# ysbbin/Robust-Object-Detection

Hardware: AMD Instinct MI355X
Metric: images/sec FRCNN-R50-FPN train @1333x800 bs=2/GPU (higher is better)
Workload: dtype f32; 1 GPU; configs[1]: FRCNN R50-FPN v2 baseline train step; global_batch=2, per_gpu_batch=2, image=1333x800 (padded 1344x800), parallelism=dp1, trainable_backbone_layers=3, conv_tuner=bench_tune.json (91 shapes pinned)

## Files before the change

### include/mx_det.h

```cpp
#ifndef MX_DET_H
#define MX_DET_H
#include <stddef.h>
#include <stdint.h>
#ifdef __cplusplus
extern "C" {
#endif

#define MX_OK 0
#define MX_EINVAL -1
#define MX_EUNSUPPORTED -2
#define MX_EHIP -3

#define MX_F32 0
#define MX_BF16 1

typedef void* mx_stream_t;

int mx_version(void);
const char* mx_last_error(void);
int mx_trace_marker(int id, mx_stream_t stream);
int mx_stream_create(int device, mx_stream_t* out);

size_t mx_match_workspace(int64_t G, int64_t A);
int mx_match_assign(const float* gt, const int64_t* gt_labels, int64_t G, const float* boxes, int64_t A,
// ... 190 lines not shown
int mx_conv2d_fwd(const mx_conv_shape* s, const uint16_t* x, const uint16_t* w, const float* bias, void* y,
                  int ydtype, float* stats, mx_stream_t stream);
int mx_conv2d_dgrad(const mx_conv_shape* s, const uint16_t* dy, const uint16_t* w, uint16_t* dx,
                    mx_stream_t stream);
int mx_conv2d_fwd_ex(const mx_conv_shape* s, const uint16_t* x, const uint16_t* w, const float* bias,
                     const uint16_t* residual, int act, void* y, int ydtype, float* stats, void* ws, size_t ws_bytes,
                     mx_stream_t stream, const mx_conv_cfg* cfg);
size_t mx_conv_workspace(const mx_conv_shape* s, int pass, const mx_conv_cfg* cfg);
int mx_conv_set_variant(int variant);
int mx_conv_get_variant(void);
int mx_conv_set_wgrad_variant(int variant);
int mx_conv_get_wgrad_variant(void);
int mx_conv_pack_weight(const mx_conv_shape* s, const float* w, int64_t Cin, int64_t Kout, uint16_t* wk, uint16_t* wt,
                        int split, mx_stream_t stream);
size_t mx_conv_dgrad_weight_elems(const mx_conv_shape* s, int64_t Cpad, int64_t Kpad);
typedef struct {
  const float* w;
  uint16_t* wk;
  uint16_t* wt;
  int64_t Cin, Kout, Cpad, Kpad;
  int32_t R, S, stride_h, stride_w, pad_h, pad_w;
  int32_t flags;
} mx_pack_desc;
size_t mx_conv_pack_plan_bytes(int64_t njobs);
int mx_conv_pack_batched(const mx_pack_desc* jobs, int64_t njobs, void* plan, size_t plan_bytes, int upload,
                         mx_stream_t stream);
typedef struct {
  float* p;
  float* buf;
  int64_t n;
  int32_t first;
  int32_t pack;
} mx_sgd_param;
size_t mx_sgd_pack_plan_bytes(int64_t nparams);
int mx_sgd_pack_build(const mx_sgd_param* params, int64_t nparams, const mx_pack_desc* packs, void* host_plan,
                      size_t plan_bytes, int64_t* blocks, size_t* lds_bytes);
int mx_sgd_pack_step(const void* plan, const float* const* grads, int64_t nparams, int64_t blocks, size_t lds_bytes,
                     float lr, float momentum, float dampening, float weight_decay, int nesterov, mx_stream_t stream);
typedef struct {
  float* p;
  float* exp_avg;
  float* exp_avg_sq;
  int64_t n;
  int32_t pack;
  int32_t reserved;
} mx_adamw_param;
size_t mx_adamw_pack_plan_bytes(int64_t nparams);
int mx_adamw_pack_build(const mx_adamw_param* params, int64_t nparams, const mx_pack_desc* packs, void* host_plan,
                        size_t plan_bytes, int64_t* blocks, size_t* lds_bytes);
int mx_adamw_pack_step(const void* plan, const float* const* grads, int64_t nparams, int64_t blocks, size_t lds_bytes,
                       int64_t step, double lr, double beta1, double beta2, double eps, double weight_decay,
                       mx_stream_t stream);
int mx_conv_transpose_weight(const uint16_t* w, int64_t K, int64_t RS, int64_t C, uint16_t* wt, mx_stream_t stream);
int mx_conv2d_dgrad_t(const mx_conv_shape* s, const uint16_t* dy, const uint16_t* wt, uint16_t* dx, void* ws,
                      size_t ws_bytes, mx_stream_t stream);
int mx_conv2d_dgrad_ex(const mx_conv_shape* s, const uint16_t* dy, const uint16_t* wt, const uint16_t* residual,
                       uint16_t* dx, void* ws, size_t ws_bytes, mx_stream_t stream, const mx_conv_cfg* cfg);
int mx_conv2d_dgrad_bnb(const mx_conv_shape* s, const uint16_t* dy, const uint16_t* wt, const uint16_t* residual,
                        uint16_t* dx, const uint16_t* y, const uint16_t* z, const float* mean, const float* invstd,
                        int act, float* part, int64_t part_mb, void* ws, size_t ws_bytes, mx_stream_t stream,
                        const mx_conv_cfg* cfg);
int mx_conv2d_wgrad(const mx_conv_shape* s, const uint16_t* dy, const uint16_t* x, float* dw, mx_stream_t stream);
int mx_conv2d_wgrad_ex(const mx_conv_shape* s, const uint16_t* dy, const uint16_t* x, float* dw, int64_t Kout,
                       int64_t Cin, int layout, void* ws, size_t ws_bytes, mx_stream_t stream, const mx_conv_cfg* cfg);
int mx_conv_set_loader(int loader);
int mx_conv_set_tile(int block_rows, int block_cols);
int mx_conv_set_max_splits(int max_splits);
int mx_conv_set_stages(int stages);
int mx_conv_set_korder(int order);
int mx_conv_set_wgrad_target(int64_t blocks);
int mx_conv_last_launch(int32_t out[8]);

size_t mx_conv_workspace_x3(const mx_conv_shape* s, int pass, const mx_conv_cfg* cfg);
int mx_conv2d_fwd_x3(const mx_conv_shape* s, const float* x, const uint16_t* w, const float* bias, const float* residual,
                     int act, float* y, float* stats, void* ws, size_t ws_bytes, mx_stream_t stream,
                     const mx_conv_cfg* cfg);
int mx_conv2d_stem_x3(const mx_conv_shape* s, const float* x, const uint16_t* w, const float* bias, int act, float* y,
                      float* stats, mx_stream_t stream);
int mx_conv2d_dgrad_x3(const mx_conv_shape* s, const float* dy, const uint16_t* wt, const float* residual, float* dx,
                       const float* y, const float* z, const float* mean, const float* invstd, int act, float* part,
                       int64_t part_mb, void* ws, size_t ws_bytes, mx_stream_t stream, const mx_conv_cfg* cfg);
int mx_conv2d_wgrad_x3(const mx_conv_shape* s, const float* dy, const float* x, float* dw, int64_t Kout, int64_t Cin,
                       int layout, void* ws, size_t ws_bytes, mx_stream_t stream, const mx_conv_cfg* cfg);

int64_t mx_rpn_rows_capacity(int64_t P, int64_t NB, int level);
size_t mx_rpn_rows_workspace(int64_t P);
int mx_rpn_rows_build(const float* g, int64_t N, int64_t H, int64_t W, int64_t C, int levels, int32_t* rows0,
                      int64_t cap0, int32_t* rows1, int64_t cap1, int32_t* rows2, int64_t cap2, int32_t* counts,
                      int32_t* flag, void* ws, size_t ws_bytes, mx_stream_t stream);
int64_t mx_rpn_tiles_capacity(int64_t P, int64_t NB, int level);
int mx_rpn_tiles_build(const float* g, int64_t N, int64_t H, int64_t W, int64_t C, int levels, int32_t* tiles0,
                       int64_t cap0, int32_t* tiles1, int64_t cap1, int32_t* tiles2, int64_t cap2, int32_t* counts,
                       int32_t* flag, void* ws, size_t ws_bytes, mx_stream_t stream);
int mx_conv2d_wgrad_x3_rows(const mx_conv_shape* s, const float* dy, const float* x, float* dw, int64_t Kout,
                            int64_t Cin, int layout, const int32_t* tiles, const int32_t* ntiles, int64_t cap, void* ws,
                            size_t ws_bytes, mx_stream_t stream, const mx_conv_cfg* cfg);
int mx_rpn_lists_build(const float* g, int64_t N, int64_t H, int64_t W, int64_t C, int32_t* rows0, int64_t cap0,
                       int32_t* rows1, int64_t cap1, int32_t* rows2, int64_t cap2, int32_t* counts, int32_t* tiles0,
                       int64_t tcap0, int32_t* tiles1, int64_t tcap1, int32_t* tcounts, int32_t* flag, void* ws,
                       size_t ws_bytes, mx_stream_t stream);
int mx_conv2d_dgrad_x3_rows_supported(const mx_conv_shape* s, const mx_conv_cfg* cfg);
int mx_conv2d_dgrad_x3_rows(const mx_conv_shape* s, const float* dy, const uint16_t* wt, const float* residual, float* dx,
                            const int32_t* rows, const int32_t* nrows, int64_t cap, mx_stream_t stream,
                            const mx_conv_cfg* cfg);
int mx_act_bias_bwd_rows(const float* gy, const float* y, const float* mask, int64_t mask_period, int64_t M, int64_t K,
                         const int32_t* rows, const int32_t* nrows, int64_t cap, float* g, float* db, void* ws,
                         size_t ws_bytes, mx_stream_t stream);

int mx_maxpool_fwd(const void* x, int dtype, int64_t N, int64_t H, int64_t W, int64_t C, int k, int stride, int pad,
                   void* y, int32_t* argmax, mx_stream_t stream);
int mx_maxpool_bwd(const void* gy, int dtype, const int32_t* argmax, int64_t N, int64_t H, int64_t W, int64_t C, int k,
                   int stride, int pad, void* gx, mx_stream_t stream);
int mx_upsample_nearest_fwd(const void* x, int dtype, int64_t N, int64_t H, int64_t W, int64_t C, int64_t Ho, int64_t Wo,
                            const void* add, void* y, mx_stream_t stream);
int mx_upsample_nearest_bwd(const void* gy, int dtype, int64_t N, int64_t H, int64_t W, int64_t C, int64_t Ho, int64_t Wo,
                            void* gx, mx_stream_t stream);

int mx_bn_finalize(const float* stats, int64_t mblocks, int64_t K, int64_t count, const float* gamma,
                   const float* beta, float eps, float momentum, float* running_mean, float* running_var,
                   float* mean_out, float* invstd_out, float* scale_out, float* shift_out, mx_stream_t stream);
int mx_bn_bwd_finalize(const float* part, int64_t mb, int64_t K, int64_t M, const float* mean, const float* invstd,
                       const float* gamma, float* sums, float* coef, void* ws, size_t ws_bytes, mx_stream_t stream);
size_t mx_rpn_loss_workspace(int64_t n);
int mx_rpn_loss_fwd(const float* objectness, const float* deltas, const float* labels, const float* targets,
                    const uint8_t* pos, const uint8_t* neg, int64_t n, float beta, float* out, void* ws,
                    size_t ws_bytes, mx_stream_t stream);
int mx_rpn_loss_bwd(const float* objectness, const float* deltas, const float* labels, const float* targets,
                    const uint8_t* pos, const uint8_t* neg, int64_t n, float beta, const float* out, const float* grad,
                    float* grad_objectness, float* grad_deltas, mx_stream_t stream);
int mx_roi_loss_fwd(const float* logits, int64_t ldl, int C, const float* reg, int64_t ldr, const int64_t* labels,
                    const float* targets, int64_t R, float beta, float* out, void* ws, size_t ws_bytes,
                    mx_stream_t stream);
int mx_roi_loss_bwd(const float* logits, int64_t ldl, int C, const float* reg, int64_t ldr, const int64_t* labels,
                    const float* targets, int64_t R, float beta, const float* grad, float* grad_logits,
                    float* grad_reg, mx_stream_t stream);
size_t mx_bn_finalize_workspace(int64_t mblocks, int64_t K);
int mx_bn_finalize_ex(const float* stats, int64_t mblocks, int64_t K, int64_t count, const float* gamma,
                      const float* beta, float eps, float momentum, float* running_mean, float* running_var,
                      float* mean_out, float* invstd_out, float* scale_out, float* shift_out, void* ws,
                      size_t ws_bytes, mx_stream_t stream);
int mx_bn_finalize_adapt(const float* stats, int64_t mblocks, int64_t K, int64_t count, const float* gamma,
                         const float* beta, float eps, const float* src_mean, const float* src_var, double prior,
                         double n_images, double* state ,
                         float* mean_out, float* var_out, float* scale_out, float* shift_out, void* ws, size_t ws_bytes,
                         mx_stream_t stream);
int mx_bn_apply(const void* x, int xdtype, int64_t M, int64_t K, const float* scale, const float* shift,
                const void* residual, int act, void* y, int ydtype, mx_stream_t stream);
int mx_bn_act_maxpool(const float* z, int64_t N, int64_t H, int64_t W, int64_t C, const float* scale, const float* shift,
                      int act, int k, int stride, int pad, float* y, mx_stream_t stream);
size_t mx_bn_bwd_workspace(int64_t M, int64_t K);
int mx_bn_bwd_reduce_ex(const void* dy, const void* y, const void* x, int dtype, int64_t M, int64_t K, int act,
                        const float* mean, const float* invstd, const float* gamma, void* ws, size_t ws_bytes,
                        float* sums, float* coef, mx_stream_t stream);
int mx_bn_bwd_apply_ex(const void* dy, const void* y, const void* x, int dtype, int64_t M, int64_t K, int act,
                       const float* coef, void* dx, void* dres, mx_stream_t stream);
size_t mx_act_bias_bwd_workspace(int64_t M, int64_t K);
int mx_act_bias_bwd(const void* gy, const void* y, int dtype, int64_t M, int64_t K, int64_t K8, int act,
                    void* g, int gdtype, float* db, void* ws, size_t ws_bytes, mx_stream_t stream);
int mx_bn_bwd_reduce(const uint16_t* dy, const uint16_t* y, const uint16_t* x, int64_t M, int64_t K, int act,
                     const float* mean, const float* invstd, float* sums, mx_stream_t stream);
int mx_bn_bwd_apply(const uint16_t* dy, const uint16_t* y, const uint16_t* x, int64_t M, int64_t K, int act,
                    const float* mean, const float* invstd, const float* gamma, const float* sums,
                    uint16_t* dx, uint16_t* dres ,
                    mx_stream_t stream);

int mx_sgd_step(float* const* params, const float* const* grads, float* const* momentum_bufs,
                const int64_t* numels, const uint8_t* first, int64_t count, float lr, float momentum,
                float dampening, float weight_decay, int nesterov, mx_stream_t stream);
int mx_adamw_step(float* const* params, const float* const* grads, float* const* exp_avgs, float* const* exp_avg_sqs,
                  const int64_t* numels, const int64_t* steps, int64_t count, double lr, double beta1, double beta2,
                  double eps, double weight_decay, mx_stream_t stream);

int mx_reflect_pad_u8(const uint8_t* src, int64_t B, int64_t H, int64_t W, int64_t C, int64_t Hp, int64_t Wp,
                      uint8_t* dst, mx_stream_t stream);
int mx_up_concat(const void* up, const void* skip, int dtype, int64_t N, int64_t H, int64_t W, int64_t Cu, int64_t Cs,
                 void* out, mx_stream_t stream);
int mx_up_concat_bwd(const void* gcat, int dtype, int64_t N, int64_t H, int64_t W, int64_t Cu, int64_t Cs, void* gup,
                     void* gskip, mx_stream_t stream);
int mx_restore_finish(const uint8_t* img_padded, int64_t B, int64_t Hp, int64_t Wp, const float* residual, int64_t H,
                      int64_t W, uint8_t* out, mx_stream_t stream);
int mx_restore_finish_gated(const uint8_t* img_padded, int64_t B, int64_t Hp, int64_t Wp, const float* residual, int64_t H,
                            int64_t W, const int32_t* verdict, uint8_t* out, mx_stream_t stream);

size_t mx_ssim_workspace(int64_t N, int64_t H, int64_t W, int64_t C);
int mx_ssim_l1_fwd(const float* pred, const float* target, int64_t N, int64_t H, int64_t W, int64_t C, int window,
                   float sigma, float c1, float c2, float weight, float* out3, double* dmaps, void* ws, size_t ws_bytes,
                   mx_stream_t stream);
int mx_ssim_l1_bwd(const float* pred, const float* target, const double* dmaps, int64_t N, int64_t H, int64_t W,
                   int64_t C, int window, float sigma, const float* gout, float cs, float cl, float* grad,
                   mx_stream_t stream);

typedef struct {
  int32_t width, height, ncomp;
  int32_t h[3], v[3], tq[3];
  int32_t hmax, vmax, mcux, mcuy;
  int32_t bw[3], bh[3];
  int32_t dw[3], dh[3];
  int64_t coef_off[3], coef_total;
  int32_t restart_interval;
  int32_t scan_off;
  uint16_t qt[4][64];
  uint8_t cid[3], td[3], ta[3];
  uint8_t hbits[8][17], hval[8][256];
  uint8_t hdef[8];
} mx_jpeg_info;
int mx_jpeg_parse(const uint8_t* data, int64_t n, mx_jpeg_info* info);
int mx_jpeg_decode_coefs(const uint8_t* data, int64_t n, const mx_jpeg_info* info, int16_t* coefs_host);
size_t mx_jpeg_workspace(const mx_jpeg_info* info);
int mx_jpeg_reconstruct(const int16_t* coefs, const mx_jpeg_info* info, void* ws, size_t ws_bytes, uint8_t* out,
                        int bgr, mx_stream_t stream);

int mx_jpeg_reconstruct_window(const int16_t* coefs, const mx_jpeg_info* info, int x0, int y0, int w, int h, int hflip,
                               int bgr, uint8_t* out, int64_t out_row_bytes, mx_stream_t stream);
int mx_jpeg_window_cover(const mx_jpeg_info* info, int x0, int y0, int w, int h, int32_t cover[3][4]);

#define MX_JPEG_ST_CODE 1
#define MX_JPEG_ST_DC 2
#define MX_JPEG_ST_RUN 4
#define MX_JPEG_ST_SHORT 8
#define MX_JPEG_ST_RESTART 16
size_t mx_jpeg_entropy_decode_workspace(const mx_jpeg_info* info, int64_t nbytes);
int mx_jpeg_entropy_decode(const uint8_t* scan_dev, int64_t nbytes, const mx_jpeg_info* info, void* ws, size_t ws_bytes,
                           int16_t* coefs_dev, int32_t* status_dev, mx_stream_t stream);
int mx_jpeg_entropy_decode_set_subseq(int bits);
int mx_jpeg_decode_coefs_chunked(const uint8_t* data, int64_t n, const mx_jpeg_info* info, int subseq_bits,
                                 int16_t* coefs_host, int32_t* status);

int mx_jpeg_encode_info(int width, int height, int quality, int subsampling, mx_jpeg_info* out);
int mx_jpeg_write_header(const mx_jpeg_info* info, uint8_t* out, int64_t cap, int64_t* n);
int64_t mx_jpeg_scan_bound(const mx_jpeg_info* info);
int mx_jpeg_encode_coefs(const mx_jpeg_info* info, const int16_t* coefs_host, uint8_t* out, int64_t cap, int64_t* n);
int mx_jpeg_forward(const uint8_t* img, int bgr, const mx_jpeg_info* info, int16_t* coefs_dev, mx_stream_t stream);
size_t mx_jpeg_entropy_workspace(const mx_jpeg_info* info);
int mx_jpeg_entropy(const int16_t* coefs_dev, const mx_jpeg_info* info, void* ws, size_t ws_bytes, uint8_t* out_dev,
                    int64_t out_cap, int64_t* nbytes_dev, mx_stream_t stream);

size_t mx_corrupt_jpeg_workspace(int64_t B, int64_t H, int64_t W, int subsampling);
int mx_corrupt_jpeg_u8(const uint8_t* img, int64_t B, int64_t H, int64_t W, const int32_t* quality_host,
// ... 19 lines not shown
```

### robust-object-detection_amd/csrc/mx_bn.hip

```cpp
#include "mx_common.h"
#include "mx_rpn_rows.h"

namespace mx {

__device__ __forceinline__ float actf(float v, int act) {
  if (act == 1) return v > 0.f ? v : 0.f;
  if (act == 2) return v > 0.f ? v : 0.2f * v;
  return v;
}
__device__ __forceinline__ float actd(float y, int act) {
  if (act == 1) return y > 0.f ? 1.f : 0.f;
  if (act == 2) return y > 0.f ? 1.f : 0.2f;
  return 1.f;
}

static constexpr int CTR_BYTES = 256, MAX_CHUNKS = CTR_BYTES / 4;

template <typename T>
__device__ __forceinline__ void st_sc1(T* p, T v) { __hip_atomic_store(p, v, __ATOMIC_RELAXED, __HIP_MEMORY_SCOPE_AGENT); }
template <typename T>
__device__ __forceinline__ T ld_sc1(const T* p) { return __hip_atomic_load((T*)p, __ATOMIC_RELAXED, __HIP_MEMORY_SCOPE_AGENT); }

__device__ __forceinline__ bool arrive_last(unsigned* ctr, unsigned nblocks) {
  __shared__ int last;
// ... 305 lines not shown
        }
      }
#pragma unroll
      for (int t = 0; t < 8; ++t) s[t] += v[t];
      st8(g + r * K8 + c0, v);
    }
  }
  if (!db) return;
#pragma unroll
  for (int t = 0; t < 8; ++t) red[rl][cl * 8 + t] = s[t];
  __syncthreads();
  const int col = threadIdx.x & 63;
  const int k = blockIdx.y * 64 + col;
  if (threadIdx.x < 64) {
    float a = 0.f;
#pragma unroll 8
    for (int r = 0; r < 32; ++r) a += red[r][col];
    if (k < K) st_sc1(part + (int64_t)blockIdx.x * K + k, a);
  }
  if (!arrive_last(ctr + blockIdx.y, (unsigned)RB)) return;
  __shared__ double fin[1][64], scr[256];
  last_sums<1>((const float*)part, RB, (int64_t)K, (int64_t)blockIdx.y * 64, fin, scr);
  if (threadIdx.x < 64 && k < K) db[k] = (float)fin[0][col];
}

__global__ void __launch_bounds__(256) act_bias_bwd_rows_kernel(const float* __restrict__ gy, const float* __restrict__ y,
                                                                const float* __restrict__ mask, int64_t mask_period,
                                                                int64_t M, int K, int64_t rows_per_block,
                                                                const int32_t* __restrict__ rows,
                                                                const int32_t* __restrict__ nrows, int64_t cap,
                                                                float* __restrict__ g, float* __restrict__ db,
                                                                unsigned* __restrict__ ctr, float* __restrict__ part) {
  __shared__ float red[32][65];
  __shared__ int64_t range[2];
  const int cl = threadIdx.x & 7, rl = threadIdx.x >> 3;
  const int c0 = blockIdx.y * 64 + cl * 8;
  const int64_t RB = gridDim.x;
  const int64_t r0 = (int64_t)blockIdx.x * rows_per_block;
  const int64_t r1 = min<int64_t>(M, r0 + rows_per_block);
  if (threadIdx.x < 2) {
    const int64_t n = min<int64_t>(max<int64_t>((int64_t)*nrows, 0), cap);
    range[threadIdx.x] = rpn_rows_lower_bound(rows, n, threadIdx.x ? r1 : r0);
  }
  __syncthreads();
  float s[8] = {0, 0, 0, 0, 0, 0, 0, 0};
  if (c0 < K) {
    const int64_t j1 = range[1];
    for (int64_t j = range[0]; j < j1; ++j) {
      const int64_t r = rows[j];
      if (r < r0 || r >= r1 || (int)((r - r0) & 31) != rl) continue;
      float v[8], vg[8], vy[8];
      ld8(gy + r * K + c0, vg);
      ld8(y + r * K + c0, vy);
      if (mask) {
        const float mk = mask[r % mask_period];
#pragma unroll
        for (int t = 0; t < 8; ++t) vg[t] = vg[t] * mk;
      }
#pragma unroll
      for (int t = 0; t < 8; ++t) v[t] = vg[t] * act_grad<1>(vy[t]);
#pragma unroll
      for (int t = 0; t < 8; ++t) s[t] += v[t];
      st8(g + r * K + c0, v);
    }
  }
  if (!db) return;
#pragma unroll
  for (int t = 0; t < 8; ++t) red[rl][cl * 8 + t] = s[t];
  __syncthreads();
  const int col = threadIdx.x & 63;
  const int k = blockIdx.y * 64 + col;
  if (threadIdx.x < 64) {
    float a = 0.f;
#pragma unroll 8
    for (int r = 0; r < 32; ++r) a += red[r][col];
    if (k < K) st_sc1(part + (int64_t)blockIdx.x * K + k, a);
  }
  if (!arrive_last(ctr + blockIdx.y, (unsigned)RB)) return;
  __shared__ double fin[1][64], scr[256];
  last_sums<1>((const float*)part, RB, (int64_t)K, (int64_t)blockIdx.y * 64, fin, scr);
  if (threadIdx.x < 64 && k < K) db[k] = (float)fin[0][col];
}

template <int ACT, typename T>
__global__ void __launch_bounds__(256) bn_bwd_apply2_kernel(const T* __restrict__ dy, const T* __restrict__ y,
                                                            const T* __restrict__ x, int64_t n8, int K8,
                                                            const float* __restrict__ coef, T* __restrict__ dx,
                                                            T* __restrict__ dres) {
  const int64_t e = (int64_t)blockIdx.x * 256 + threadIdx.x;
  if (e >= n8) return;
  const int K = K8 * 8;
  const int c0 = (int)(e % K8) * 8;
  float vd[8], vx[8], vy[8] = {0, 0, 0, 0, 0, 0, 0, 0};
  ld8(dy + e * 8, vd);
  ld8(x + e * 8, vx);
  if (ACT) ld8(y + e * 8, vy);
  const float4 a0 = *(const float4*)(coef + c0), a1 = *(const float4*)(coef + c0 + 4);
  const float4 b0 = *(const float4*)(coef + K + c0), b1 = *(const float4*)(coef + K + c0 + 4);
  const float4 d0 = *(const float4*)(coef + 2 * K + c0), d1 = *(const float4*)(coef + 2 * K + c0 + 4);
  const float A[8] = {a0.x, a0.y, a0.z, a0.w, a1.x, a1.y, a1.z, a1.w};
  const float B[8] = {b0.x, b0.y, b0.z, b0.w, b1.x, b1.y, b1.z, b1.w};
  const float C[8] = {d0.x, d0.y, d0.z, d0.w, d1.x, d1.y, d1.z, d1.w};
  float o[8], og[8];
#pragma unroll
  for (int q = 0; q < 8; ++q) {
    og[q] = vd[q] * act_grad<ACT>(vy[q]);
    o[q] = A[q] * og[q] + B[q] * vx[q] + C[q];
  }
  st8(dx + e * 8, o);
  if (dres) st8(dres + e * 8, og);
}

__global__ void bn_coef_from_sums_kernel(const float* __restrict__ sums, int64_t K, int64_t M, const float* __restrict__ mean,
                                         const float* __restrict__ invstd, const float* __restrict__ gamma,
                                         float* __restrict__ coef) {
  const int64_t k = (int64_t)blockIdx.x * blockDim.x + threadIdx.x;
  if (k >= K) return;
  const float is = invstd[k], a = (gamma ? gamma[k] : 1.f) * is;
  const float invM = 1.0f / (float)M;
  const float mg = sums[k] * invM, mgx = sums[K + k] * invM;
  coef[k] = a;
  coef[K + k] = -a * is * mgx;
  coef[2 * K + k] = -a * (mg - mean[k] * is * mgx);
}

static unsigned grid_rows(int64_t M, int64_t K8) {
  int64_t want = std::min<int64_t>(cdiv(M * K8, 256), 2048);
  return (unsigned)std::max<int64_t>(want, cdiv(K8, 256));
}

struct BwdGeo {
  int64_t RB, rows_per_block, gy;
};
static BwdGeo bwd_geo(int64_t M, int64_t K) {
  BwdGeo g;
  g.gy = cdiv(K, 64);
  g.RB = std::max<int64_t>(1, std::min<int64_t>(std::min<int64_t>(128, cdiv(M, 64)), std::max<int64_t>(1, 1024 / g.gy)));
  g.rows_per_block = cdiv(M, g.RB);
  g.RB = cdiv(M, g.rows_per_block);
  return g;
}

static int64_t fin_slices(int64_t mb) { return std::max<int64_t>(1, std::min<int64_t>(64, cdiv(mb, 32))); }

__device__ __forceinline__ float smooth_l1(float u, float beta) {
  const float a = fabsf(u);
  return a < beta ? 0.5f * u * u / beta : a - 0.5f * beta;
}

__global__ void __launch_bounds__(256) rpn_loss_fwd_kernel(const float* __restrict__ x, const float4* __restrict__ d,
                                                           const float* __restrict__ y, const float4* __restrict__ t,
                                                           const uint8_t* __restrict__ pm, const uint8_t* __restrict__ nm,
                                                           int64_t n, float beta, unsigned* __restrict__ ctr,
                                                           double* __restrict__ part, float* __restrict__ out) {
  double a0 = 0.0, a1 = 0.0, a2 = 0.0;
  for (int64_t i = (int64_t)blockIdx.x * 256 + threadIdx.x; i < n; i += (int64_t)gridDim.x * 256) {
    const bool p = pm[i], s = p || nm[i];
    if (!s) continue;
    const float xi = x[i], yi = y[i] > 0.f ? 1.f : 0.f;
    const float m = fmaxf(-xi, 0.f);
    a0 += (double)((1.f - yi) * xi + m + logf(expf(-m) + expf(-xi - m)));
    a2 += 1.0;
    if (p) {
      const float4 di = d[i], ti = t[i];
      a1 += (double)(smooth_l1(di.x - ti.x, beta) + smooth_l1(di.y - ti.y, beta) + smooth_l1(di.z - ti.z, beta) +
                     smooth_l1(di.w - ti.w, beta));
    }
  }
  __shared__ double red[3][256];
  red[0][threadIdx.x] = a0;
  red[1][threadIdx.x] = a1;
  red[2][threadIdx.x] = a2;
  __syncthreads();
  for (int o = 128; o > 0; o >>= 1) {
    if (threadIdx.x < o)
      for (int w = 0; w < 3; ++w) red[w][threadIdx.x] += red[w][threadIdx.x + o];
    __syncthreads();
  }
  const int64_t RB = gridDim.x;
  if (threadIdx.x < 3) st_sc1(part + threadIdx.x * RB + blockIdx.x, red[threadIdx.x][0]);
  if (!arrive_last(ctr, (unsigned)RB)) return;
  __shared__ double fin[3][64], scr[256];
  last_sums<3>(part, RB, 1, 0, fin, scr);
  if (threadIdx.x == 0) {
    const double cnt = fin[2][0];
    out[0] = (float)(fin[0][0] / cnt);
    out[1] = (float)(fin[1][0] / cnt);
    out[2] = (float)cnt;
  }
}

__global__ void __launch_bounds__(256) rpn_loss_bwd_kernel(const float* __restrict__ x, const float4* __restrict__ d,
// ... 215 lines not shown
                           const void* residual, int act, void* y, int ydtype, mx_stream_t stream) {
  MX_CHECK_ARG(K % 8 == 0, "bn_apply: K %% 8 != 0");
  MX_CHECK_ARG((xdtype == MX_BF16 || xdtype == MX_F32) && (ydtype == MX_BF16 || ydtype == MX_F32), "bn_apply: bad dtype");
  MX_CHECK_ARG(!(xdtype == MX_BF16 && ydtype == MX_F32),
               "bn_apply: bf16 input with f32 output is not a supported combination");
  if (M == 0) return MX_OK;
  const unsigned grid = grid_rows(M, K / 8);
  hipStream_t st = (hipStream_t)stream;
  if (xdtype == MX_BF16 && ydtype == MX_BF16)
    bn_apply_kernel<uint16_t, uint16_t><<<grid, 256, 0, st>>>((const uint16_t*)x, M, K, scale, shift,
                                                             (const uint16_t*)residual, act, (uint16_t*)y);
  else if (xdtype == MX_F32 && ydtype == MX_BF16)
    bn_apply_kernel<float, uint16_t><<<grid, 256, 0, st>>>((const float*)x, M, K, scale, shift, (const uint16_t*)residual,
                                                          act, (uint16_t*)y);
  else if (xdtype == MX_F32 && ydtype == MX_F32)
    bn_apply_kernel<float, float><<<grid, 256, 0, st>>>((const float*)x, M, K, scale, shift, (const float*)residual, act,
                                                       (float*)y);
  else
    MX_CHECK_ARG(false, "bn_apply: bf16 input with f32 output is not a supported combination");
  MX_LAUNCH_CHECK();
  return MX_OK;
}

extern "C" size_t mx_bn_bwd_workspace(int64_t M, int64_t K) {
  if (M <= 0 || K <= 0 || K % 8) return 0;
  BwdGeo g = bwd_geo(M, K);
  return CTR_BYTES + sizeof(float) * 2 * (size_t)g.RB * K;
}

template <typename T>
static void bn_bwd_reduce_launch(const void* dy, const void* y, const void* x, int64_t M, int64_t K, int act,
                                 const BwdGeo& g, const float* mean, const float* invstd, const float* gamma, unsigned* ctr,
                                 float* part, float* sums, float* coef, hipStream_t st) {
  dim3 grid((unsigned)g.RB, (unsigned)g.gy);
  const T *d = (const T*)dy, *yy = (const T*)y, *xx = (const T*)x;
  if (act == 1)
    bn_bwd_reduce_kernel<1, T><<<grid, 256, 0, st>>>(d, yy, xx, M, K, g.rows_per_block, mean, invstd, gamma, ctr, part, sums, coef);
  else if (act == 2)
    bn_bwd_reduce_kernel<2, T><<<grid, 256, 0, st>>>(d, yy, xx, M, K, g.rows_per_block, mean, invstd, gamma, ctr, part, sums, coef);
  else
    bn_bwd_reduce_kernel<0, T><<<grid, 256, 0, st>>>(d, yy, xx, M, K, g.rows_per_block, mean, invstd, gamma, ctr, part, sums, coef);
}

extern "C" int mx_bn_bwd_reduce_ex(const void* dy, const void* y, const void* x, int dtype, int64_t M, int64_t K, int act,
                                   const float* mean, const float* invstd, const float* gamma, void* ws, size_t ws_bytes,
                                   float* sums, float* coef, mx_stream_t stream) {
  MX_CHECK_ARG(K % 8 == 0 && K > 0 && M > 0, "bn_bwd_reduce: K must be a positive multiple of 8, M > 0");
  MX_CHECK_ARG(act >= 0 && act <= 2, "bn_bwd_reduce: act 0/1/2");
  MX_CHECK_ARG(act == 0 || y, "bn_bwd_reduce: y required for an activation");
  BwdGeo g = bwd_geo(M, K);
  MX_CHECK_ARG(g.gy <= MAX_CHUNKS && g.RB < 65536, "bn_bwd_reduce: K > %d", MAX_CHUNKS * 64);
  const size_t need = mx_bn_bwd_workspace(M, K);
  MX_CHECK_ARG(ws && ws_bytes >= need, "bn_bwd_reduce: workspace of %zu bytes required (mx_bn_bwd_workspace)", need);
  unsigned* ctr = (unsigned*)ws;
  float* part = (float*)((char*)ws + CTR_BYTES);
  MX_DT_DISPATCH(dtype, bn_bwd_reduce_launch, dy, y, x, M, K, act, g, mean, invstd, gamma, ctr, part, sums, coef,
                 (hipStream_t)stream);
  MX_LAUNCH_CHECK();
  return MX_OK;
}

template <typename T>
static void bn_bwd_apply_launch(const void* dy, const void* y, const void* x, int64_t n8, int K8, int act, const float* coef,
                                void* dx, void* dres, hipStream_t st) {
  const unsigned blocks = (unsigned)cdiv(n8, 256);
  const T *d = (const T*)dy, *yy = (const T*)y, *xx = (const T*)x;
  if (act == 1) bn_bwd_apply2_kernel<1, T><<<blocks, 256, 0, st>>>(d, yy, xx, n8, K8, coef, (T*)dx, (T*)dres);
  else if (act == 2) bn_bwd_apply2_kernel<2, T><<<blocks, 256, 0, st>>>(d, yy, xx, n8, K8, coef, (T*)dx, (T*)dres);
  else bn_bwd_apply2_kernel<0, T><<<blocks, 256, 0, st>>>(d, yy, xx, n8, K8, coef, (T*)dx, (T*)dres);
}

extern "C" int mx_bn_bwd_apply_ex(const void* dy, const void* y, const void* x, int dtype, int64_t M, int64_t K, int act,
                                  const float* coef, void* dx, void* dres, mx_stream_t stream) {
  MX_CHECK_ARG(K % 8 == 0 && K > 0 && K < (1 << 24), "bn_bwd_apply: K must be a positive multiple of 8");
  MX_CHECK_ARG(act >= 0 && act <= 2, "bn_bwd_apply: act 0/1/2");
  MX_CHECK_ARG(act == 0 || y, "bn_bwd_apply: y required for an activation");
  if (M == 0) return MX_OK;
  const int64_t n8 = M * (K / 8);
  MX_DT_DISPATCH(dtype, bn_bwd_apply_launch, dy, y, x, n8, (int)(K / 8), act, coef, dx, dres, (hipStream_t)stream);
  MX_LAUNCH_CHECK();
  return MX_OK;
}

extern "C" int mx_bn_bwd_reduce(const uint16_t* dy, const uint16_t* y, const uint16_t* x, int64_t M, int64_t K, int act,
                                const float* mean, const float* invstd, float* sums, mx_stream_t stream) {
  MX_CHECK_ARG(K % 8 == 0 && K > 0, "bn_bwd_reduce: K must be a positive multiple of 8");
  if (M == 0) return MX_OK;
  hipStream_t st = (hipStream_t)stream;
  const size_t wsb = mx_bn_bwd_workspace(M, K);
  void* ws = nullptr;
  float* coef = nullptr;
  MX_HIP(hipMallocAsync(&ws, wsb, st));
  MX_HIP(hipMemsetAsync(ws, 0, CTR_BYTES, st));
  MX_HIP(hipMallocAsync((void**)&coef, sizeof(float) * 3 * K, st));
  int rc = mx_bn_bwd_reduce_ex(dy, y, x, MX_BF16, M, K, act, mean, invstd, nullptr, ws, wsb, sums, coef, stream);
  MX_HIP(hipFreeAsync(ws, st));
  MX_HIP(hipFreeAsync(coef, st));
  return rc;
}

extern "C" int mx_bn_bwd_apply(const uint16_t* dy, const uint16_t* y, const uint16_t* x, int64_t M, int64_t K, int act,
                               const float* mean, const float* invstd, const float* gamma, const float* sums,
                               uint16_t* dx, uint16_t* dres, mx_stream_t stream) {
  MX_CHECK_ARG(K % 8 == 0 && K > 0, "bn_bwd_apply: K %% 8 != 0");
  if (M == 0) return MX_OK;
  hipStream_t st = (hipStream_t)stream;
  float* coef = nullptr;
  MX_HIP(hipMallocAsync((void**)&coef, sizeof(float) * 3 * K, st));
  bn_coef_from_sums_kernel<<<(unsigned)cdiv(K, 256), 256, 0, st>>>(sums, K, M, mean, invstd, gamma, coef);
  int rc = MX_OK;
  if (hipGetLastError() != hipSuccess) rc = MX_EHIP;
  if (!rc) rc = mx_bn_bwd_apply_ex(dy, y, x, MX_BF16, M, K, act, coef, dx, dres, stream);
  MX_HIP(hipFreeAsync(coef, st));
  return rc;
}

static BwdGeo act_geo(int64_t M, int64_t K8) {
  BwdGeo g;
  g.gy = cdiv(K8, 64);
  g.RB = std::max<int64_t>(1, std::min<int64_t>(std::min<int64_t>(128, cdiv(M, 64)), std::max<int64_t>(1, 1024 / g.gy)));
  g.rows_per_block = cdiv(M, g.RB);
  g.RB = cdiv(M, g.rows_per_block);
  return g;
}

extern "C" size_t mx_act_bias_bwd_workspace(int64_t M, int64_t K) {
  if (M <= 0 || K <= 0) return 0;
  BwdGeo g = act_geo(M, (K + 7) / 8 * 8);
  return CTR_BYTES + sizeof(float) * (size_t)g.RB * K;
}

template <typename T, typename TG>
static void launch_act_bias(const void* gy, const void* y, int64_t M, int K, int K8, int act, const BwdGeo& g,
                            void* out_, float* db, unsigned* ctr, float* part, hipStream_t st) {
  dim3 grid((unsigned)g.RB, (unsigned)g.gy);
  TG* out = (TG*)out_;
  if (act == 1)
    act_bias_bwd_kernel<T, 1, TG><<<grid, 256, 0, st>>>((const T*)gy, (const T*)y, M, K, K8, g.rows_per_block, out, db, ctr, part);
  else if (act == 2)
    act_bias_bwd_kernel<T, 2, TG><<<grid, 256, 0, st>>>((const T*)gy, (const T*)y, M, K, K8, g.rows_per_block, out, db, ctr, part);
  else
    act_bias_bwd_kernel<T, 0, TG><<<grid, 256, 0, st>>>((const T*)gy, (const T*)y, M, K, K8, g.rows_per_block, out, db, ctr, part);
}

extern "C" int mx_act_bias_bwd(const void* gy, const void* y, int dtype, int64_t M, int64_t K, int64_t K8, int act,
                               void* g, int gdtype, float* db, void* ws, size_t ws_bytes, mx_stream_t stream) {
  MX_CHECK_ARG(M >= 0 && K > 0 && K8 >= K && K8 % 8 == 0 && K8 < (1 << 24), "act_bias_bwd: need 0 < K <= K8, K8 %% 8 == 0");
  MX_CHECK_ARG(act >= 0 && act <= 2 && (act == 0 || y), "act_bias_bwd: act 0/1/2 (y required for 1/2)");
  MX_CHECK_ARG(dtype == MX_BF16 || dtype == MX_F32, "act_bias_bwd: dtype bf16 or f32");
  MX_CHECK_ARG(gdtype == MX_BF16 || gdtype == MX_F32, "act_bias_bwd: gdtype bf16 or f32");
  if (M == 0) {
    if (db) MX_HIP(hipMemsetAsync(db, 0, sizeof(float) * K, (hipStream_t)stream));
    return MX_OK;
  }
  BwdGeo g_ = act_geo(M, K8);
  MX_CHECK_ARG(g_.gy <= MAX_CHUNKS, "act_bias_bwd: K8 > %d", MAX_CHUNKS * 64);
  unsigned* ctr = nullptr;
  float* part = nullptr;
  if (db) {
    const size_t need = mx_act_bias_bwd_workspace(M, K);
    MX_CHECK_ARG(ws && ws_bytes >= need, "act_bias_bwd: workspace of %zu bytes required (mx_act_bias_bwd_workspace)", need);
    ctr = (unsigned*)ws;
    part = (float*)((char*)ws + CTR_BYTES);
  }
  hipStream_t st = (hipStream_t)stream;
  if (dtype == MX_BF16 && gdtype == MX_BF16)
// ... 103 lines not shown
```

### robust-object-detection_amd/csrc/mx_conv.hip

```cpp
#include "mx_common.h"
#include "mx_conv_layout.h"
#include "mx_dma.h"
#include "mx_rpn_rows.h"

#include <vector>

namespace mx {

typedef __bf16 bf16x8 __attribute__((ext_vector_type(8)));
typedef short s16x4 __attribute__((ext_vector_type(4)));
typedef float f32x4 __attribute__((ext_vector_type(4)));

static constexpr int BM = 128, BK = 64, NT = 256;

struct ConvP {
  const uint16_t* src;
  const uint16_t* wt;
  int64_t M, Ncol, Kdim;
  int64_t OH, OW;
  int64_t IH, IW, IC;
  int R, S, st_h, st_w, pad_h, pad_w;
  const float* bias;
  const void* residual;
  int act;
// ... 1457 lines not shown
    for (int i = 0; i < BCH; ++i) {
      if (kin && b_row[i] < p.Ncol) {
        rbh[i] = *(const uint4*)(whi + b_row[i] * p.Kdim + k);
        rbl[i] = *(const uint4*)(wlo + b_row[i] * p.Kdim + k);
      } else {
        rbh[i] = rbl[i] = make_uint4(0, 0, 0, 0);
      }
    }
  };
  auto store = [&](int buf) {
    char* Ah = smem + buf * STAGE;
    char* Al = Ah + APL;
    char* Bh = Al + APL;
    char* Bl = Bh + BPL;
#pragma unroll
    for (int i = 0; i < ACH; ++i) {
      const int row = (tid >> 2) + RPS * i;
      const int off = row * RB + ((kc ^ tile_swz<4>(row)) << 4);
      uint4 h, l;
      split8(ra[i][0], ra[i][1], h, l);
      *(uint4*)(Ah + off) = h;
      *(uint4*)(Al + off) = l;
    }
#pragma unroll
    for (int i = 0; i < BCH; ++i) {
      const int row = (tid >> 2) + RPS * i;
      const int off = row * RB + ((kc ^ tile_swz<4>(row)) << 4);
      *(uint4*)(Bh + off) = rbh[i];
      *(uint4*)(Bl + off) = rbl[i];
    }
  };
  f32x4 acc[TI][TJ];
#pragma unroll
  for (int i = 0; i < TI; ++i)
#pragma unroll
    for (int j = 0; j < TJ; ++j) acc[i][j] = f32x4{0.f, 0.f, 0.f, 0.f};
  if (ntk > 0) {
    load();
    store(0);
  }
  __syncthreads();
  for (int64_t t = 0; t < ntk; ++t) {
    const int buf = (int)(t & 1);
    if (t + 1 < ntk) load();
    const char* Ah = smem + buf * STAGE;
    const char* Al = Ah + APL;
    const char* Bh = Al + APL;
    const char* Bl = Bh + BPL;
    const int ch = lane >> 4;
    bf16x8 ah[TI], al[TI], bh[TJ], bl[TJ];
#pragma unroll
    for (int i = 0; i < TI; ++i) {
      const int row = wm * WM + i * 16 + (lane & 15);
      const int off = row * RB + ((ch ^ tile_swz<4>(row)) << 4);
      ah[i] = *(const bf16x8*)(Ah + off);
      al[i] = *(const bf16x8*)(Al + off);
    }
#pragma unroll
    for (int j = 0; j < TJ; ++j) {
      const int row = wn * WN + j * 16 + (lane & 15);
      const int off = row * RB + ((ch ^ tile_swz<4>(row)) << 4);
      bh[j] = *(const bf16x8*)(Bh + off);
      bl[j] = *(const bf16x8*)(Bl + off);
    }
#pragma unroll
    for (int i = 0; i < TI; ++i)
#pragma unroll
      for (int j = 0; j < TJ; ++j) {
        acc[i][j] = __builtin_amdgcn_mfma_f32_16x16x32_bf16(al[i], bh[j], acc[i][j], 0, 0, 0);
        acc[i][j] = __builtin_amdgcn_mfma_f32_16x16x32_bf16(ah[i], bl[j], acc[i][j], 0, 0, 0);
        acc[i][j] = __builtin_amdgcn_mfma_f32_16x16x32_bf16(ah[i], bh[j], acc[i][j], 0, 0, 0);
      }
    if (t + 1 < ntk) store(buf ^ 1);
    __syncthreads();
  }
  conv_epilogue<BN, 2, BMT, float, 2, 2, MODE == 1>(p, acc, smem, m0, n0, mt, wm, wn, lane, tid, split);
}

__device__ __forceinline__ int x3_swz(int row) {
  const int g = (row >> 2) & 3;
  return g ^ (g >> 1);
}

template <int BN, int MODE, int STAGES, int OCC, int BMT, int WR = 2, int WC = 2, bool ROWS = false>
__global__ void __launch_bounds__(64 * WR * WC, OCC) conv_x3_buf_kernel(ConvP p) {
#if defined(__HIP_DEVICE_COMPILE__)
  extern __shared__ __attribute__((aligned(16))) char smem[];
  constexpr int RB = 64, RPI = 16;
  constexpr int NW = WC * WR;
  constexpr int AR = BMT / NW, AI = AR / RPI, BR = BN / NW, BI = BR / RPI;
  constexpr int LOADS = 2 * AI + 2 * BI;
  constexpr int AH = BMT * RB, BP = BN * RB, STAGE = 2 * AH + 2 * BP;
  constexpr int WN = BN / WC, TJ = WN / 16, WM = BMT / WR, TI = WM / 16;
  static_assert(AI >= 1 && BI >= 1 && STAGES >= 2, "tile shape");
  const int tid = threadIdx.x, lane = tid & 63, wave = tid >> 6;
  const int wm = wave / WC, wn = wave % WC;
  const int64_t ntiles_n = (p.Ncol + BN - 1) / BN;
  const int64_t gid = xcd_remap(blockIdx.x, (int64_t)gridDim.x);
  const int split = (int)(gid % p.splits);
  const int64_t bid = gid / p.splits;
  const int64_t mt = bid / ntiles_n, nt = bid % ntiles_n;
  const int64_t m0 = mt * BMT, n0 = nt * BN;
  int64_t nrows = p.M;
  if constexpr (ROWS) {
    static_assert(MODE == 1, "rows form: dgrad only");
    nrows = min<int64_t>(max<int64_t>((int64_t)*p.rows_count, 0), p.rows_cap);
    if (m0 >= nrows) return;
  }
  const int lrow = lane >> 2, pc = lane & 3;
  const int qa = pc ^ x3_swz(lrow), qb = pc ^ tile_swz<4>(lrow);
  const int IH = (int)p.IH, IW = (int)p.IW, IC = (int)p.IC, R = p.R, S = p.S;
  uint32_t a_voff[AI];
  uint64_t a_mask[AI];
#pragma unroll
  for (int i = 0; i < AI; ++i) {
    int64_t m = m0 + wave * AR + i * RPI + lrow;
    uint64_t mask = 0;
    int32_t off = 0;
    bool mok = m < nrows;
    if constexpr (ROWS) {
      m = mok ? (int64_t)p.rows[m] : -1;
      mok = (uint64_t)m < (uint64_t)p.M;
    }
    if (mok) {
      const int ow = (int)(m % p.OW);
      const int64_t t = m / p.OW;
      const int oh = (int)(t % p.OH);
      const int n = (int)(t / p.OH);
      const int h0 = MODE == 0 ? oh * p.st_h - p.pad_h : oh + p.pad_h - (R - 1);
      const int w0 = MODE == 0 ? ow * p.st_w - p.pad_w : ow + p.pad_w - (S - 1);
      off = ((n * IH + h0) * IW + w0) * IC + qa * 4;
      for (int r = 0; r < R; ++r)
        for (int q = 0; q < S; ++q) {
          const int rr = MODE == 0 ? r : R - 1 - r, qq = MODE == 0 ? q : S - 1 - q;
          if ((unsigned)(h0 + rr) < (unsigned)IH && (unsigned)(w0 + qq) < (unsigned)IW) mask |= 1ull << (r * S + q);
        }
    }
    a_voff[i] = (uint32_t)off * 4u;
    a_mask[i] = mask;
  }
  uint32_t b_voff[BI];
#pragma unroll
  for (int i = 0; i < BI; ++i) {
    const int64_t n = n0 + wave * BR + i * RPI + lrow;
    b_voff[i] = n < p.Ncol ? (uint32_t)((n * p.Kdim + qb * 8) * 2) : kOOB;
  }
  const i32x4 arsrc = dma_rsrc(p.src, (uint32_t)(p.src_elems * 4));
  const i32x4 bhrsrc = dma_rsrc(p.wt, (uint32_t)(p.wt_elems * 2));
  const i32x4 blrsrc = dma_rsrc(p.wt + p.wt_plane, (uint32_t)(p.wt_elems * 2));
  const uint32_t lds0 = lds_addr(smem);
  const int64_t nk = p.Kdim / 32;
  const int64_t kbeg = (int64_t)split * p.kt_per_split;
  const int64_t ntk = min<int64_t>(nk, kbeg + p.kt_per_split) - kbeg;
  const int korder = __builtin_amdgcn_readfirstlane(p.korder);
  KPos kp;
  kp.init(korder, (int)kbeg, R, S, IC, 32);
  constexpr int dbg = 0;
  auto issue = [&](int buf) {
    const uint32_t A = lds0 + buf * STAGE;
    const uint32_t B = A + 2 * AH;
    const int cr = kp.cr, cq = kp.cq, cc = kp.cc;
    const int rr = MODE == 0 ? cr : R - 1 - cr, qq = MODE == 0 ? cq : S - 1 - cq;
    const uint32_t a_soff = (uint32_t)(((rr * IW + qq) * IC + cc) * 4);
    const int tap = cr * S + cq;
    const uint32_t b_soff = (uint32_t)__builtin_amdgcn_readfirstlane((int)((tap * IC + cc) * 2));
    if (!(dbg & 8)) {
#pragma unroll
    for (int i = 0; i < AI; ++i) {
      const bool ok = (a_mask[i] >> tap) & 1ull;
      const uint32_t v = a_voff[i] + a_soff;
      const uint32_t dst = A + (wave * AR + i * RPI) * RB;
      lds_dma16(arsrc, dst, ok ? v : kOOB, 0u);
      lds_dma16(arsrc, dst + AH, ok ? v + 64u : kOOB, 0u);
    }
    }
    if (!(dbg & 4)) {
#pragma unroll
    for (int i = 0; i < BI; ++i) {
      const uint32_t dst = B + (wave * BR + i * RPI) * RB;
      lds_dma16(bhrsrc, dst, b_voff[i], b_soff);
      lds_dma16(blrsrc, dst + BP, b_voff[i], b_soff);
    }
    }
    kp.advance(korder, R, S, IC, 32);
  };
  f32x4 acc[TI][TJ];
#pragma unroll
  for (int i = 0; i < TI; ++i)
#pragma unroll
    for (int j = 0; j < TJ; ++j) acc[i][j] = f32x4{0.f, 0.f, 0.f, 0.f};
#pragma unroll
  for (int st = 0; st < STAGES - 1; ++st)
    if (st < ntk) issue(st);
  const int g = lane >> 4, q0 = (g & 1) * 2;
  for (int64_t t = 0; t < ntk; ++t) {
    if (t + STAGES - 2 < ntk) wait_vmcnt<LOADS * (STAGES - 2)>();
    else wait_vmcnt<0>();
    block_barrier();
    if (t + STAGES - 1 < ntk) issue((int)((t + STAGES - 1) % STAGES));
    const char* A = smem + (int)(t % STAGES) * STAGE;
    const char* Ag = A + (g >> 1) * AH;
    const char* Bh = A + 2 * AH;
    const char* Bl = Bh + BP;
    constexpr int TJB = (TJ > 4 && WC == 2) ? 1 : TJ;
    bf16x8 ah[TI], al[TI], bh[TJB], bl[TJB];
    auto loadb = [&](int j, int slot) {
      const int row = wn * WN + j * 16 + (lane & 15);
      const int off = row * RB + ((g ^ tile_swz<4>(row)) << 4);
      bh[slot] = *(const bf16x8*)(Bh + off);
      bl[slot] = *(const bf16x8*)(Bl + off);
    };
    if constexpr (TJB == TJ) {
#pragma unroll
      for (int j = 0; j < TJ; ++j) loadb(j, j);
    }
#pragma unroll
    for (int i = 0; i < TI; ++i) {
      const int row = wm * WM + i * 16 + (lane & 15);
      const int f = x3_swz(row);
      const float4 u = *(const float4*)(Ag + row * RB + ((q0 ^ f) << 4));
      const float4 w = *(const float4*)(Ag + row * RB + (((q0 + 1) ^ f) << 4));
      uint4 h, l;
      if (dbg & 2) {
        h = __builtin_bit_cast(uint4, u);
        l = __builtin_bit_cast(uint4, w);
      } else {
        split8(u, w, h, l);
      }
      ah[i] = __builtin_bit_cast(bf16x8, h);
      al[i] = __builtin_bit_cast(bf16x8, l);
    }
    if constexpr (TJB == TJ) {
#pragma unroll
      for (int i = 0; i < TI; ++i)
#pragma unroll
        for (int j = 0; j < TJ; ++j) {
          acc[i][j] = __builtin_amdgcn_mfma_f32_16x16x32_bf16(al[i], bh[j], acc[i][j], 0, 0, 0);
          acc[i][j] = __builtin_amdgcn_mfma_f32_16x16x32_bf16(ah[i], bl[j], acc[i][j], 0, 0, 0);
          acc[i][j] = __builtin_amdgcn_mfma_f32_16x16x32_bf16(ah[i], bh[j], acc[i][j], 0, 0, 0);
        }
    } else {
#pragma unroll
      for (int j = 0; j < TJ; ++j) {
        loadb(j, 0);
#pragma unroll
        for (int i = 0; i < TI; ++i) {
          acc[i][j] = __builtin_amdgcn_mfma_f32_16x16x32_bf16(al[i], bh[0], acc[i][j], 0, 0, 0);
          acc[i][j] = __builtin_amdgcn_mfma_f32_16x16x32_bf16(ah[i], bl[0], acc[i][j], 0, 0, 0);
          acc[i][j] = __builtin_amdgcn_mfma_f32_16x16x32_bf16(ah[i], bh[0], acc[i][j], 0, 0, 0);
        }
      }
    }
  }
  if (dbg & 1) {
    float sum = 0.f;
#pragma unroll
    for (int i = 0; i < TI; ++i)
#pragma unroll
      for (int j = 0; j < TJ; ++j) sum += acc[i][j][0] + acc[i][j][1] + acc[i][j][2] + acc[i][j][3];
    if (sum == 1.2345e-30f) ((float*)p.out)[0] = sum;
    return;
  }
  __syncthreads();
  conv_epilogue<BN, (WC == 1 ? 1 : WR), BMT, float, WR, WC, MODE == 1, ROWS>(p, acc, smem, m0, n0, mt, wm, wn, lane,
                                                                             tid, split, nrows);
#endif
}

#if defined(__HIP_DEVICE_COMPILE__)
template <bool ROWS>
__device__ __forceinline__ void wgrad_x3_body(const WgP& p) {
  extern __shared__ __attribute__((aligned(16))) char smem[];
  constexpr int PXT = 32, OPB = PXT * 256, STAGE = 4 * OPB;
  const int tid = threadIdx.x, lane = tid & 63, wave = tid >> 6;
  const int wm = wave >> 1, wn = wave & 1;
  const int64_t ntn = (p.Ncol + 127) / 128;
  const int64_t ntiles = ((p.K + 127) / 128) * ntn;
  const int64_t work = xcd_remap(blockIdx.x, (int64_t)gridDim.x);
  const int64_t split = work / ntiles, tile = work % ntiles;
  const int64_t mt = tile / ntn, nt = tile % ntn;
  const int64_t k0 = mt * 128, c0 = nt * 128;
  const int64_t pbeg = split * p.kchunk;
  const int64_t pend = min<int64_t>(p.P, pbeg + p.kchunk);
  if (pbeg >= pend) return;
  int li = 0, lend = 0;
  if constexpr (ROWS) {
    const int n = (int)wgrad_rows(p);
    const int tb = (int)(pbeg / PXT), te = (int)((pend + PXT - 1) / PXT);
    auto lower = [&](int v) {
      int lo = 0, hi = n;
      while (lo < hi) {
        const int mid = (lo + hi) >> 1;
        if (p.rows[mid] < v) lo = mid + 1;
        else hi = mid;
      }
      return lo;
    };
    li = lower(tb);
    lend = lower(te);
  }
  const float* __restrict__ dy = (const float*)p.dy;
  const float* __restrict__ x = (const float*)p.x;
  const int ch = tid & 15;
  const int64_t col = c0 + ch * 8;
  const bool col_ok = col < p.Ncol;
  const int tap = col_ok ? (int)(col / p.C) : 0;
  const int cc = col_ok ? (int)(col - (int64_t)tap * p.C) : 0;
  const int r = tap / p.S, s = tap - (tap / p.S) * p.S;
  const bool k_ok = (k0 + ch * 8) < p.K;
  const int OW = (int)p.OW, OH = (int)p.OH, H = (int)p.H, W = (int)p.W, C = (int)p.C;
  const __amdgpu_buffer_rsrc_t dyr = __builtin_amdgcn_make_buffer_rsrc((void*)dy, (short)0, (int)(p.P * p.K * 4), 0x00020000);
  const __amdgpu_buffer_rsrc_t xr =
      __builtin_amdgcn_make_buffer_rsrc((void*)x, (short)0, (int)(p.N * p.H * p.W * p.C * 4), 0x00020000);
  const int dw = PXT % OW, dh = (PXT / OW) % OH, dn = PXT / (OW * OH);
  const int ihb = -p.pad_h + r, iwb = -p.pad_w + s;
  int px_n[2], px_oh[2], px_ow[2], px_i[2];
#pragma unroll
  for (int i = 0; i < 2; ++i) {
    const int64_t pi = pbeg + (tid >> 4) + 16 * i;
    px_i[i] = (int)pi;
    const int64_t t = pi / OW;
    px_ow[i] = (int)(pi - t * OW);
    px_oh[i] = (int)(t % OH);
    px_n[i] = (int)(t / OH);
  }
  const int pend32 = (int)pend;
  const uint32_t dy_col = (uint32_t)(k0 + ch * 8) * 4u;
  float4 rd[2][2], rx[2][2];
  auto load = [&]() {
#pragma unroll
    for (int i = 0; i < 2; ++i) {
      if constexpr (ROWS) {
        px_i[i] = p.rows[li] * PXT + (tid >> 4) + 16 * i;
        const int t = px_i[i] / OW;
        px_ow[i] = px_i[i] - t * OW;
        px_n[i] = t / OH;
        px_oh[i] = t - px_n[i] * OH;
      }
      const bool pok = px_i[i] < pend32;
      const int pix = px_i[i];
      const uint32_t od = (pok && k_ok) ? __umul24((uint32_t)pix, (uint32_t)(p.K * 4)) + dy_col : kOOB;
      const int ih = __mul24(px_oh[i], p.st_h) + ihb, iw = __mul24(px_ow[i], p.st_w) + iwb;
      const bool xok = pok && col_ok && (unsigned)ih < (unsigned)H && (unsigned)iw < (unsigned)W;
      const uint32_t ox = xok ? (uint32_t)__mul24(__mul24(px_n[i], H) + ih, W) + (uint32_t)iw : 0u;
      const uint32_t oxb = xok ? __umul24(ox, (uint32_t)(C * 4)) + (uint32_t)cc * 4u : kOOB;
      rd[i][0] = __builtin_bit_cast(float4, __builtin_amdgcn_raw_buffer_load_b128(dyr, od, 0, 0));
      rd[i][1] = __builtin_bit_cast(float4, __builtin_amdgcn_raw_buffer_load_b128(dyr, od + 16u, 0, 0));
      rx[i][0] = __builtin_bit_cast(float4, __builtin_amdgcn_raw_buffer_load_b128(xr, oxb, 0, 0));
      rx[i][1] = __builtin_bit_cast(float4, __builtin_amdgcn_raw_buffer_load_b128(xr, oxb + 16u, 0, 0));
      px_i[i] += PXT;
      if constexpr (ROWS) continue;
      int ow = px_ow[i] + dw;
      const int c1 = ow >= OW ? 1 : 0;
      ow -= c1 * OW;
      int oh = px_oh[i] + dh + c1;
      const int c2 = oh >= OH ? 1 : 0;
      oh -= c2 * OH;
      px_ow[i] = ow;
      px_oh[i] = oh;
      px_n[i] += dn + c2;
    }
    if constexpr (ROWS) ++li;
  };
  auto store = [&](int buf) {
    char* Dh = smem + buf * STAGE;
#pragma unroll
    for (int i = 0; i < 2; ++i) {
      const int row = (tid >> 4) + 16 * i;
      const int off = row * 256 + (swz_w(row, ch) << 4);
      uint4 h, l;
      split8(rd[i][0], rd[i][1], h, l);
      *(uint4*)(Dh + off) = h;
      *(uint4*)(Dh + OPB + off) = l;
      split8(rx[i][0], rx[i][1], h, l);
      *(uint4*)(Dh + 2 * OPB + off) = h;
      *(uint4*)(Dh + 3 * OPB + off) = l;
    }
  };
  auto tr_read = [&](const char* T, int prow0, int colbase) -> s16x4 {
    const int g = lane >> 4, q = (lane & 15) >> 2, pp = lane & 3;
    const int row = prow0 + 8 * g + q;
    const int colx = colbase + 4 * pp;
    const int chunk = colx >> 3, within = (colx & 7) * 2;
    return __builtin_amdgcn_ds_read_tr16_b64_v4i16((LDS_AS s16x4*)(T + row * 256 + (swz_w(row, chunk) << 4) + within));
  };
  auto frag = [&](const char* T, int colbase) -> bf16x8 {
    const s16x4 lo = tr_read(T, 0, colbase), hi = tr_read(T, 4, colbase);
    return __builtin_bit_cast(bf16x8, __builtin_shufflevector(lo, hi, 0, 1, 2, 3, 4, 5, 6, 7));
  };
  f32x4 acc[4][4];
#pragma unroll
  for (int i = 0; i < 4; ++i)
#pragma unroll
    for (int j = 0; j < 4; ++j) acc[i][j] = f32x4{0.f, 0.f, 0.f, 0.f};
  const int64_t nk = ROWS ? (int64_t)(lend - li) : (pend - pbeg + PXT - 1) / PXT;
  if (ROWS && nk == 0) {
    wgrad_store(p, acc, k0, c0, wm, wn, lane, split);
    return;
  }
  load();
  store(0);
  __syncthreads();
  for (int64_t it = 0; it < nk; ++it) {
    const int buf = (int)(it & 1);
    if (it + 1 < nk) load();
    const char* Dh = smem + buf * STAGE;
    bf16x8 ah[4], al[4], bh[4], bl[4];
#pragma unroll
    for (int i = 0; i < 4; ++i) {
      ah[i] = frag(Dh, wm * 64 + i * 16);
      al[i] = frag(Dh + OPB, wm * 64 + i * 16);
    }
#pragma unroll
    for (int j = 0; j < 4; ++j) {
      bh[j] = frag(Dh + 2 * OPB, wn * 64 + j * 16);
      bl[j] = frag(Dh + 3 * OPB, wn * 64 + j * 16);
    }
#pragma unroll
    for (int i = 0; i < 4; ++i)
#pragma unroll
      for (int j = 0; j < 4; ++j) {
        acc[i][j] = __builtin_amdgcn_mfma_f32_16x16x32_bf16(al[i], bh[j], acc[i][j], 0, 0, 0);
        acc[i][j] = __builtin_amdgcn_mfma_f32_16x16x32_bf16(ah[i], bl[j], acc[i][j], 0, 0, 0);
        acc[i][j] = __builtin_amdgcn_mfma_f32_16x16x32_bf16(ah[i], bh[j], acc[i][j], 0, 0, 0);
      }
    if (it + 1 < nk) store(buf ^ 1);
    __syncthreads();
  }
  wgrad_store(p, acc, k0, c0, wm, wn, lane, split);
}
#endif
__global__ void __launch_bounds__(NT, 2) conv_wgrad_x3_kernel(WgP p) {
#if defined(__HIP_DEVICE_COMPILE__)
  wgrad_x3_body<false>(p);
#endif
}
__global__ void __launch_bounds__(NT, 2) conv_wgrad_x3_rows_kernel(WgP p) {
#if defined(__HIP_DEVICE_COMPILE__)
  wgrad_x3_body<true>(p);
#endif
}

__global__ void __launch_bounds__(512, 1) conv_wgrad_x3w_kernel(WgP p) {
#if defined(__HIP_DEVICE_COMPILE__)
  extern __shared__ __attribute__((aligned(16))) char smem[];
  constexpr int PXT = 32, OPB = PXT * 256, STAGE = 6 * OPB;
  const int tid = threadIdx.x, lane = tid & 63, wave = tid >> 6;
  const int wm = wave >> 2, wn = wave & 3;
  const int64_t ntn = (p.Ncol + 255) / 256;
  const int64_t ntiles = ((p.K + 127) / 128) * ntn;
  const int64_t work = xcd_remap(blockIdx.x, (int64_t)gridDim.x);
  const int64_t split = work / ntiles, tile = work % ntiles;
  const int64_t mt = tile / ntn, nt = tile % ntn;
  const int64_t k0 = mt * 128, c0 = nt * 256;
  const int64_t pbeg = split * p.kchunk;
  const int64_t pend = min<int64_t>(p.P, pbeg + p.kchunk);
  if (pbeg >= pend) return;
  const float* __restrict__ dy = (const float*)p.dy;
  const float* __restrict__ x = (const float*)p.x;
  const int chd = tid & 15, rowd = tid >> 4;
  const int chx = tid & 31, rowx = tid >> 5;
  const bool k_ok = (k0 + chd * 8) < p.K;
  const int64_t col = c0 + chx * 8;
  const bool col_ok = col < p.Ncol;
  const int tap = col_ok ? (int)(col / p.C) : 0;
  const int cc = col_ok ? (int)(col - (int64_t)tap * p.C) : 0;
  const int r = tap / p.S, s = tap - (tap / p.S) * p.S;
  const int OW = (int)p.OW, OH = (int)p.OH, H = (int)p.H, W = (int)p.W, C = (int)p.C;
  const __amdgpu_buffer_rsrc_t dyr = __builtin_amdgcn_make_buffer_rsrc((void*)dy, (short)0, (int)(p.P * p.K * 4), 0x00020000);
  const __amdgpu_buffer_rsrc_t xr =
      __builtin_amdgcn_make_buffer_rsrc((void*)x, (short)0, (int)(p.N * p.H * p.W * p.C * 4), 0x00020000);
  const int dw = PXT % OW, dh = (PXT / OW) % OH, dn = PXT / (OW * OH);
  const int ihb = -p.pad_h + r, iwb = -p.pad_w + s;
  int pxd = (int)(pbeg + rowd);
  int px_n[2], px_oh[2], px_ow[2], px_i[2];
#pragma unroll
  for (int i = 0; i < 2; ++i) {
    const int64_t pi = pbeg + rowx + 16 * i;
    px_i[i] = (int)pi;
    const int64_t t = pi / OW;
    px_ow[i] = (int)(pi - t * OW);
    px_oh[i] = (int)(t % OH);
    px_n[i] = (int)(t / OH);
  }
  const int pend32 = (int)pend;
  const uint32_t dy_col = (uint32_t)(k0 + chd * 8) * 4u;
  float4 rd[2], rx[2][2];
  auto load = [&]() {
    {
      const uint32_t od = (pxd < pend32 && k_ok) ? __umul24((uint32_t)pxd, (uint32_t)(p.K * 4)) + dy_col : kOOB;
      rd[0] = __builtin_bit_cast(float4, __builtin_amdgcn_raw_buffer_load_b128(dyr, od, 0, 0));
      rd[1] = __builtin_bit_cast(float4, __builtin_amdgcn_raw_buffer_load_b128(dyr, od + 16u, 0, 0));
      pxd += PXT;
    }
#pragma unroll
    for (int i = 0; i < 2; ++i) {
      const bool pok = px_i[i] < pend32;
      const int ih = __mul24(px_oh[i], p.st_h) + ihb, iw = __mul24(px_ow[i], p.st_w) + iwb;
      const bool xok = pok && col_ok && (unsigned)ih < (unsigned)H && (unsigned)iw < (unsigned)W;
      const uint32_t ox = xok ? (uint32_t)__mul24(__mul24(px_n[i], H) + ih, W) + (uint32_t)iw : 0u;
      const uint32_t oxb = xok ? __umul24(ox, (uint32_t)(C * 4)) + (uint32_t)cc * 4u : kOOB;
      rx[i][0] = __builtin_bit_cast(float4, __builtin_amdgcn_raw_buffer_load_b128(xr, oxb, 0, 0));
      rx[i][1] = __builtin_bit_cast(float4, __builtin_amdgcn_raw_buffer_load_b128(xr, oxb + 16u, 0, 0));
      px_i[i] += PXT;
      int ow = px_ow[i] + dw;
      const int c1 = ow >= OW ? 1 : 0;
      ow -= c1 * OW;
      int oh = px_oh[i] + dh + c1;
      const int c2 = oh >= OH ? 1 : 0;
      oh -= c2 * OH;
      px_ow[i] = ow;
      px_oh[i] = oh;
      px_n[i] += dn + c2;
    }
  };
  const int xh = chx >> 4, xc = chx & 15;
  auto store = [&](int buf) {
    char* D = smem + buf * STAGE;
    uint4 h, l;
    {
      const int off = rowd * 256 + (swz_w(rowd, chd) << 4);
      split8(rd[0], rd[1], h, l);
      *(uint4*)(D + off) = h;
      *(uint4*)(D + OPB + off) = l;
    }
#pragma unroll
    for (int i = 0; i < 2; ++i) {
      const int row = rowx + 16 * i;
      const int off = row * 256 + (swz_w(row, xc) << 4);
      split8(rx[i][0], rx[i][1], h, l);
      *(uint4*)(D + (2 + xh) * OPB + off) = h;
      *(uint4*)(D + (4 + xh) * OPB + off) = l;
    }
  };
  auto tr_read = [&](const char* T, int prow0, int colbase) -> s16x4 {
    const int g = lane >> 4, q = (lane & 15) >> 2, pp = lane & 3;
    const int row = prow0 + 8 * g + q;
    const int colx = colbase + 4 * pp;
    const int chunk = colx >> 3, within = (colx & 7) * 2;
    return __builtin_amdgcn_ds_read_tr16_b64_v4i16((LDS_AS s16x4*)(T + row * 256 + (swz_w(row, chunk) << 4) + within));
  };
  auto frag = [&](const char* T, int colbase) -> bf16x8 {
    const s16x4 lo = tr_read(T, 0, colbase), hi = tr_read(T, 4, colbase);
    return __builtin_bit_cast(bf16x8, __builtin_shufflevector(lo, hi, 0, 1, 2, 3, 4, 5, 6, 7));
  };
  f32x4 acc[4][4];
#pragma unroll
  for (int i = 0; i < 4; ++i)
#pragma unroll
    for (int j = 0; j < 4; ++j) acc[i][j] = f32x4{0.f, 0.f, 0.f, 0.f};
  const int64_t nk = (pend - pbeg + PXT - 1) / PXT;
  load();
  store(0);
  __syncthreads();
  const int xplane = wn >> 1, xcol = (wn & 1) * 64;
  for (int64_t it = 0; it < nk; ++it) {
    const int buf = (int)(it & 1);
    if (it + 1 < nk) load();
    const char* D = smem + buf * STAGE;
    bf16x8 ah[4], al[4], bh[4], bl[4];
#pragma unroll
    for (int i = 0; i < 4; ++i) {
      ah[i] = frag(D, wm * 64 + i * 16);
      al[i] = frag(D + OPB, wm * 64 + i * 16);
    }
#pragma unroll
    for (int j = 0; j < 4; ++j) {
      bh[j] = frag(D + (2 + xplane) * OPB, xcol + j * 16);
      bl[j] = frag(D + (4 + xplane) * OPB, xcol + j * 16);
    }
#pragma unroll
    for (int i = 0; i < 4; ++i)
#pragma unroll
      for (int j = 0; j < 4; ++j) {
        acc[i][j] = __builtin_amdgcn_mfma_f32_16x16x32_bf16(al[i], bh[j], acc[i][j], 0, 0, 0);
        acc[i][j] = __builtin_amdgcn_mfma_f32_16x16x32_bf16(ah[i], bl[j], acc[i][j], 0, 0, 0);
        acc[i][j] = __builtin_amdgcn_mfma_f32_16x16x32_bf16(ah[i], bh[j], acc[i][j], 0, 0, 0);
      }
    if (it + 1 < nk) store(buf ^ 1);
    __syncthreads();
  }
  wgrad_store(p, acc, k0, c0, wm, wn, lane, split);
#endif
}

__device__ __forceinline__ void wgrad_store8(const WgP& p, f32x4 (&acc)[8][8], int64_t k0, int64_t c0, int wm, int wn,
                                             int lane, int64_t split) {
  float* slab = p.slab ? p.slab + split * p.K * p.Ncol : nullptr;
#pragma unroll
  for (int i = 0; i < 8; ++i)
#pragma unroll
    for (int j = 0; j < 8; ++j)
#pragma unroll
      for (int rr = 0; rr < 4; ++rr) {
        const int64_t k = k0 + wm * 128 + i * 16 + (lane >> 4) * 4 + rr;
        const int64_t cl = c0 + wn * 128 + j * 16 + (lane & 15);
        if (k >= p.K || cl >= p.Ncol) continue;
        if (slab) {
          slab[k * p.Ncol + cl] = acc[i][j][rr];
        } else {
          const int64_t o = wgrad_dst(p, k, (int)cl);
          if (o >= 0) p.dw[o] = acc[i][j][rr];
        }
      }
}

__global__ void __launch_bounds__(256, 1) conv_wgrad_x3ww_kernel(WgP p) {
#if defined(__HIP_DEVICE_COMPILE__)
  extern __shared__ __attribute__((aligned(16))) char smem[];
  constexpr int PXT = 32, SUB = PXT * 256, STAGE = 8 * SUB;
  const int tid = threadIdx.x, lane = tid & 63, wave = tid >> 6;
  const int wm = wave >> 1, wn = wave & 1;
  const int64_t ntn = (p.Ncol + 255) / 256;
  const int64_t ntiles = ((p.K + 255) / 256) * ntn;
  const int64_t work = xcd_remap(blockIdx.x, (int64_t)gridDim.x);
  const int64_t split = work / ntiles, tile = work % ntiles;
  const int64_t mt = tile / ntn, nt = tile % ntn;
  const int64_t k0 = mt * 256, c0 = nt * 256;
  const int64_t pbeg = split * p.kchunk;
  const int64_t pend = min<int64_t>(p.P, pbeg + p.kchunk);
  if (pbeg >= pend) return;
  const float* __restrict__ dy = (const float*)p.dy;
  const float* __restrict__ x = (const float*)p.x;
  const int ch = tid & 31, row0 = tid >> 5;
  const bool k_ok = (k0 + ch * 8) < p.K;
  const int64_t col = c0 + ch * 8;
  const bool col_ok = col < p.Ncol;
  const int tap = col_ok ? (int)(col / p.C) : 0;
  const int cc = col_ok ? (int)(col - (int64_t)tap * p.C) : 0;
  const int r = tap / p.S, s = tap - (tap / p.S) * p.S;
  const int OW = (int)p.OW, OH = (int)p.OH, H = (int)p.H, W = (int)p.W, C = (int)p.C;
  const __amdgpu_buffer_rsrc_t dyr = __builtin_amdgcn_make_buffer_rsrc((void*)dy, (short)0, (int)(p.P * p.K * 4), 0x00020000);
  const __amdgpu_buffer_rsrc_t xr =
      __builtin_amdgcn_make_buffer_rsrc((void*)x, (short)0, (int)(p.N * p.H * p.W * p.C * 4), 0x00020000);
  const int dw = PXT % OW, dh = (PXT / OW) % OH, dn = PXT / (OW * OH);
  const int ihb = -p.pad_h + r, iwb = -p.pad_w + s;
  int px_n[4], px_oh[4], px_ow[4], px_i[4];
#pragma unroll
  for (int i = 0; i < 4; ++i) {
    const int64_t pi = pbeg + row0 + 8 * i;
    px_i[i] = (int)pi;
    const int64_t t = pi / OW;
    px_ow[i] = (int)(pi - t * OW);
    px_oh[i] = (int)(t % OH);
    px_n[i] = (int)(t / OH);
  }
  const int pend32 = (int)pend;
  const uint32_t dy_col = (uint32_t)(k0 + ch * 8) * 4u;
  float4 rd[4][2], rx[4][2];
  auto load = [&]() {
#pragma unroll
    for (int i = 0; i < 4; ++i) {
      const bool pok = px_i[i] < pend32;
      const uint32_t od = (pok && k_ok) ? __umul24((uint32_t)px_i[i], (uint32_t)(p.K * 4)) + dy_col : kOOB;
      const int ih = __mul24(px_oh[i], p.st_h) + ihb, iw = __mul24(px_ow[i], p.st_w) + iwb;
      const bool xok = pok && col_ok && (unsigned)ih < (unsigned)H && (unsigned)iw < (unsigned)W;
      const uint32_t ox = xok ? (uint32_t)__mul24(__mul24(px_n[i], H) + ih, W) + (uint32_t)iw : 0u;
      const uint32_t oxb = xok ? __umul24(ox, (uint32_t)(C * 4)) + (uint32_t)cc * 4u : kOOB;
      rd[i][0] = __builtin_bit_cast(float4, __builtin_amdgcn_raw_buffer_load_b128(dyr, od, 0, 0));
      rd[i][1] = __builtin_bit_cast(float4, __builtin_amdgcn_raw_buffer_load_b128(dyr, od + 16u, 0, 0));
      rx[i][0] = __builtin_bit_cast(float4, __builtin_amdgcn_raw_buffer_load_b128(xr, oxb, 0, 0));
      rx[i][1] = __builtin_bit_cast(float4, __builtin_amdgcn_raw_buffer_load_b128(xr, oxb + 16u, 0, 0));
      px_i[i] += PXT;
      int ow = px_ow[i] + dw;
      const int c1 = ow >= OW ? 1 : 0;
      ow -= c1 * OW;
      int oh = px_oh[i] + dh + c1;
      const int c2 = oh >= OH ? 1 : 0;
      oh -= c2 * OH;
      px_ow[i] = ow;
      px_oh[i] = oh;
      px_n[i] += dn + c2;
    }
  };
  const int sub = ch >> 4, c16 = ch & 15;
  auto store = [&](int buf) {
    char* D = smem + buf * STAGE;
#pragma unroll
    for (int i = 0; i < 4; ++i) {
      const int row = row0 + 8 * i;
      const int off = row * 256 + (swz_w(row, c16) << 4);
      uint4 h, l;
      split8(rd[i][0], rd[i][1], h, l);
      *(uint4*)(D + (0 + sub) * SUB + off) = h;
      *(uint4*)(D + (2 + sub) * SUB + off) = l;
      split8(rx[i][0], rx[i][1], h, l);
      *(uint4*)(D + (4 + sub) * SUB + off) = h;
      *(uint4*)(D + (6 + sub) * SUB + off) = l;
    }
  };
  auto tr_read = [&](const char* T, int prow0, int colbase) -> s16x4 {
    const int g = lane >> 4, q = (lane & 15) >> 2, pp = lane & 3;
    const int row = prow0 + 8 * g + q;
    const int colx = colbase + 4 * pp;
    const int chunk = colx >> 3, within = (colx & 7) * 2;
    return __builtin_amdgcn_ds_read_tr16_b64_v4i16((LDS_AS s16x4*)(T + row * 256 + (swz_w(row, chunk) << 4) + within));
  };
  auto frag = [&](const char* T, int colbase) -> bf16x8 {
    const s16x4 lo = tr_read(T, 0, colbase), hi = tr_read(T, 4, colbase);
    return __builtin_bit_cast(bf16x8, __builtin_shufflevector(lo, hi, 0, 1, 2, 3, 4, 5, 6, 7));
  };
  f32x4 acc[8][8];
#pragma unroll
  for (int i = 0; i < 8; ++i)
#pragma unroll
    for (int j = 0; j < 8; ++j) acc[i][j] = f32x4{0.f, 0.f, 0.f, 0.f};
  const int64_t nk = (pend - pbeg + PXT - 1) / PXT;
  load();
  store(0);
  __syncthreads();
  for (int64_t it = 0; it < nk; ++it) {
    const int buf = (int)(it & 1);
    if (it + 1 < nk) load();
    const char* D = smem + buf * STAGE;
    const char* Ah = D + (0 + wm) * SUB;
    const char* Al = D + (2 + wm) * SUB;
    const char* Bh = D + (4 + wn) * SUB;
    const char* Bl = D + (6 + wn) * SUB;
    bf16x8 ah[8], al[8], bh[8], bl[8];
#pragma unroll
    for (int i = 0; i < 8; ++i) {
      ah[i] = frag(Ah, i * 16);
      al[i] = frag(Al, i * 16);
    }
#pragma unroll
    for (int j = 0; j < 8; ++j) {
      bh[j] = frag(Bh, j * 16);
      bl[j] = frag(Bl, j * 16);
    }
#pragma unroll
    for (int i = 0; i < 8; ++i)
#pragma unroll
      for (int j = 0; j < 8; ++j) {
        acc[i][j] = __builtin_amdgcn_mfma_f32_16x16x32_bf16(al[i], bh[j], acc[i][j], 0, 0, 0);
        acc[i][j] = __builtin_amdgcn_mfma_f32_16x16x32_bf16(ah[i], bl[j], acc[i][j], 0, 0, 0);
        acc[i][j] = __builtin_amdgcn_mfma_f32_16x16x32_bf16(ah[i], bh[j], acc[i][j], 0, 0, 0);
      }
    if (it + 1 < nk) store(buf ^ 1);
    __syncthreads();
  }
  wgrad_store8(p, acc, k0, c0, wm, wn, lane, split);
#endif
}

__global__ void transpose_w_kernel(const uint16_t* __restrict__ w, int64_t K, int64_t RS, int64_t C, uint16_t* __restrict__ wt) {
  int64_t i = (int64_t)blockIdx.x * blockDim.x + threadIdx.x;
  if (i >= K * RS * C) return;
  int64_t c = i % C, rs = (i / C) % RS, k = i / (C * RS);
  wt[(c * RS + rs) * K + k] = w[i];
}

__global__ void krsc_to_dgrad_kernel(const uint16_t* __restrict__ w, PackP p) {
  const int64_t i = (int64_t)blockIdx.x * blockDim.x + threadIdx.x;
  if (i >= p.K * p.R * p.S * p.C) return;
  const int64_t c = i % p.C, t = i / p.C;
  const int sx = (int)(t % p.S), r = (int)((t / p.S) % p.R);
  const int64_t k = t / ((int64_t)p.S * p.R);
  const int q = (r % p.st_h) * p.st_w + sx % p.st_w;
  p.wt[p.off[q] + ((c * p.Rc[q] + r / p.st_h) * p.Sc[q] + sx / p.st_w) * p.Kpad + k] = w[i];
}


static constexpr int STEM_T = 4, STEM_K = 64, STEM_R = 7;
struct StemP {
  const float* x;
  const uint16_t* w;
// ... 687 lines not shown
               "%s: dy / x must each stay below 2 GiB and 8M pixels (32-bit / 24-bit offset math)", name);
  return MX_OK;
}

static int wgrad_finish(const WgP& p, const WGeo& g, int64_t Kout, hipStream_t st, const char* name) {
  if (g.splits <= 1) return MX_OK;
  MX_CHECK_ARG(Kout < 65536, "%s: too many output channels for the split reduce", name);
  wgrad_reduce_kernel<<<dim3((unsigned)cdiv(p.Ncol / 4, 64), (unsigned)Kout), 256, 0, st>>>(p, (int)g.splits);
  MX_LAUNCH_CHECK();
  return MX_OK;
}

extern "C" int mx_conv2d_wgrad_ex(const mx_conv_shape* s, const uint16_t* dy, const uint16_t* x, float* dw,
                                  int64_t Kout, int64_t Cin, int layout, void* ws, size_t ws_bytes,
                                  mx_stream_t stream, const mx_conv_cfg* cfg) {
  const char* name = "conv wgrad";
  Cfg cf;
  int rc = resolve_cfg(cfg, cf);
  if (!rc) rc = wgrad_check(s, Kout, Cin, layout, name);
  if (rc) return rc;
  hipStream_t st = (hipStream_t)stream;
  WgP p{};
  WGeo g;
  rc = fill_wgrad(p, g, cf, wgrad_geo, s, dy, x, dw, Kout, Cin, layout, ws, ws_bytes, name, "mx_conv_workspace");
  if (rc) return rc;
  MX_CHECK_ARG(g.tiles < (1ll << 31) && g.splits < 65536, "conv wgrad: grid too large");
  dim3 grid((unsigned)g.tiles, (unsigned)g.splits);
  int v = cf.k.wgrad_variant >= 4 ? 3 : cf.k.wgrad_variant;
  if (v == 3 && !(p.P * p.K * 2 < (1ll << 31) && p.N * p.H * p.W * p.C * 2 < (1ll << 31) &&
                 (p.OH * p.OW >= 32 || (p.OH == 1 && p.OW == 1))))
    v = 0;
  if (v == 3) conv_wgrad_buf_kernel<<<(unsigned)(g.tiles * g.splits), NT, 3 * 2 * 32 * 256, st>>>(p);
  else if (v == 2) conv_wgrad_glds_kernel<<<grid, NT, 2 * 2 * BKG * 256, st>>>(p);
  else if (v == 1) conv_wgrad_kernel<64><<<grid, NT, 0, st>>>(p);
  else conv_wgrad_kernel<32><<<grid, NT, 0, st>>>(p);
  MX_LAUNCH_CHECK();
  g_launch_count = 0;
  record_launch(2, 128, 128, g.splits, g.tiles, v == 3, v);
  return wgrad_finish(p, g, Kout, st, name);
}

extern "C" int mx_conv2d_wgrad(const mx_conv_shape* s, const uint16_t* dy, const uint16_t* x, float* dw, mx_stream_t stream) {
  int rc = conv_check(s);
  if (rc) return rc;
  size_t wsb = mx_conv_workspace(s, 2, nullptr);
  void* ws = nullptr;
  if (wsb) MX_HIP(hipMallocAsync(&ws, wsb, (hipStream_t)stream));
  rc = mx_conv2d_wgrad_ex(s, dy, x, dw, s->K, s->C, 0, ws, wsb, stream, nullptr);
  if (ws) MX_HIP(hipFreeAsync(ws, (hipStream_t)stream));
  return rc;
}

static Geo make_geo_x3(const Cfg& cf, int64_t M, int64_t Ncol, int64_t Kdim) {
  Geo g;
  g.M = M; g.Ncol = Ncol; g.Kdim = Kdim;
  g.narrow = Ncol <= 64;
  g.bn = g.narrow ? 64 : 128;
  const int64_t cus = num_cus();
  g.bmt = 128;
  g.tiles = cdiv(M, 128) * cdiv(Ncol, g.bn);
  if (g.tiles < 2 * cus) {
    g.bmt = 64;
    g.tiles = cdiv(M, 64) * cdiv(Ncol, g.bn);
  }
  if (cf.k.tile_rows) {
    g.bmt = cf.k.tile_rows;
    g.bn = g.bmt == 256 ? 128 : std::min(cf.k.tile_cols, 128);
    g.narrow = g.bn == 64;
    g.tiles = cdiv(M, g.bmt) * cdiv(Ncol, g.bn);
  }
  g.nk = cdiv(Kdim, 32);
  g.splits = geo_splits(cf, g);
  if (g.splits > 1) g.splits = (int)cdiv(g.nk, cdiv(g.nk, (int64_t)g.splits));
  return g;
}

template <int BN, int MODE, int BMT>
static void launch_x3(const ConvP& p, int64_t blocks, hipStream_t st) {
  const size_t ring = (size_t)2 * 2 * (BMT + BN) * 64;
  const size_t epi = (size_t)(BMT / 2) * (BN + 4) * 4;
  conv_x3_kernel<BN, MODE, BMT><<<(unsigned)blocks, NT, std::max(ring, epi), st>>>(p);
}

template <int BN, int MODE, int STAGES, int OCC, int BMT, int WR = 2, int WC = 2>
static void launch_x3_buf(const ConvP& p, int64_t blocks, hipStream_t st) {
  const size_t ring = (size_t)STAGES * 2 * (BMT + BN) * 64;
  const size_t epi = (size_t)(WC == 1 ? BMT : BMT / WR) * (BN + 4) * 4;
  conv_x3_buf_kernel<BN, MODE, STAGES, OCC, BMT, WR, WC><<<(unsigned)blocks, 64 * WR * WC, std::max(ring, epi), st>>>(p);
}

template <int MODE>
static int launch_igemm_x3(const Cfg& cf, ConvP& p, const Geo& g0, void* ws, size_t ws_bytes, hipStream_t st) {
  const bool buf = cf.loader >= 1 && p.IC % 32 == 0 && p.R * p.S <= 64 && p.Kdim % 32 == 0 && p.src_elems > 0 &&
                   p.src_elems * 4 < (1ll << 31) && p.wt_elems > 0 && p.wt_plane + p.wt_elems < (1ll << 30);
  Geo g = g0;
  if (g.bmt == 256 && !buf) {
    g.bmt = 128;
    g.tiles = cdiv(g.M, 128) * cdiv(g.Ncol, g.bn);
  }
  int64_t blocks = g.tiles;
  MX_CHECK_ARG(g.Kdim < (1ll << 30) && p.IH < (1ll << 26) && p.IW < (1ll << 26) && p.IC < (1ll << 30),
               "conv: GEMM K or spatial size too large");
  MX_CHECK_ARG(p.IC % 8 == 0 && p.Kdim % 8 == 0, "conv x3: channel counts must be multiples of 8");
  const int splits = plan_splitk(p, g, cdiv(g.Kdim, 32), ws, ws_bytes, "mx_conv_workspace_x3");
  if (!splits) return MX_EINVAL;
  blocks *= splits;
  MX_CHECK_ARG(blocks < (1ll << 31), "conv: grid too large");
  if (buf) {
    const bool alt = cf.k.stages == 3;
    const bool wide = cf.k.stages == 0, wide64 = wide;
    const bool altw = cf.k.stages == 5;
    p.korder = cf.korder;
    if (cf.loader == 2) p.src_elems = 0;
    if (cf.loader == 3) p.wt_elems = 0;
    if (g.bmt == 256) {
      alt ? launch_x3_buf<128, MODE, 2, 1, 256, 4>(p, blocks, st) : launch_x3_buf<128, MODE, 3, 1, 256, 4>(p, blocks, st);
    } else if (g.bmt == 64) {
      if (g.bn == 64) {
        if (altw) launch_x3_buf<64, MODE, 3, 3, 64, 4, 1>(p, blocks, st);
        else alt ? launch_x3_buf<64, MODE, 4, 2, 64>(p, blocks, st) : launch_x3_buf<64, MODE, 3, 3, 64>(p, blocks, st);
      } else if (altw) launch_x3_buf<128, MODE, 2, 3, 64, 4, 1>(p, blocks, st);
      else if (wide64) launch_x3_buf<128, MODE, 3, 2, 64, 4, 1>(p, blocks, st);
      else alt ? launch_x3_buf<128, MODE, 2, 3, 64>(p, blocks, st) : launch_x3_buf<128, MODE, 3, 2, 64>(p, blocks, st);
    } else {
      if (g.bn == 64) alt ? launch_x3_buf<64, MODE, 2, 3, 128>(p, blocks, st) : launch_x3_buf<64, MODE, 3, 2, 128>(p, blocks, st);
      else if (altw) launch_x3_buf<128, MODE, 3, 1, 128, 4, 1>(p, blocks, st);
      else if (wide) launch_x3_buf<128, MODE, 2, 2, 128, 4, 1>(p, blocks, st);
      else alt ? launch_x3_buf<128, MODE, 3, 1, 128>(p, blocks, st) : launch_x3_buf<128, MODE, 2, 2, 128>(p, blocks, st);
    }
  } else if (g.bmt == 64) {
    if (g.bn == 64) launch_x3<64, MODE, 64>(p, blocks, st);
    else launch_x3<128, MODE, 64>(p, blocks, st);
  } else {
    if (g.bn == 64) launch_x3<64, MODE, 128>(p, blocks, st);
    else launch_x3<128, MODE, 128>(p, blocks, st);
  }
  MX_LAUNCH_CHECK();
  record_launch(MODE, g.bmt, g.bn, p.splits, g.tiles, buf, 100 + (buf ? cf.k.stages : 0));
  return launch_splitk_reduce<float>(p, g, st);
}

static size_t conv_workspace(const mx_conv_shape* s, int pass, const mx_conv_cfg* cfg,
                             Geo (*geo)(const Cfg&, int64_t, int64_t, int64_t),
                             WGeo (*wgeo)(const Cfg&, const mx_conv_shape*)) {
  Cfg cf;
  if (!s || pass < 0 || pass > 2 || resolve_cfg(cfg, cf)) return 0;
  if (pass == 2) {
    bool dense;
    const mx_conv_shape sd = wgrad_shape(s, &dense);
    return split_ws_bytes(wgeo(cf, &sd).splits, sd.K, sd.R * sd.S * sd.C);
  }
  if (pass == 0) {
    const Geo g = geo(cf, s->N * s->Ho * s->Wo, s->K, s->R * s->S * s->C);
    return split_ws_bytes(g.splits, g.M, g.Ncol);
  }
  if (s->stride_h < 1 || s->stride_h > 2 || s->stride_w < 1 || s->stride_w > 2) return 0;
  DClass cl[4];
  const int n = dgrad_launch_classes(s, cl);
  size_t mx = 0;
  for (int i = 0; i < n; ++i) {
    const Geo g = geo(cf, s->N * cl[i].Hc * cl[i].Wc, s->C, (int64_t)cl[i].Rc * cl[i].Sc * s->K);
    mx = std::max(mx, split_ws_bytes(g.splits, g.M, g.Ncol));
  }
  return mx;
}
extern "C" size_t mx_conv_workspace(const mx_conv_shape* s, int pass, const mx_conv_cfg* cfg) {
  return conv_workspace(s, pass, cfg, make_geo, wgrad_geo);
}
extern "C" size_t mx_conv_workspace_x3(const mx_conv_shape* s, int pass, const mx_conv_cfg* cfg) {
  return conv_workspace(s, pass, cfg, make_geo_x3, wgrad_geo_x3);
}

extern "C" int mx_conv2d_fwd_x3(const mx_conv_shape* s, const float* x, const uint16_t* w, const float* bias,
                                const float* residual, int act, float* y, float* stats, void* ws, size_t ws_bytes,
                                mx_stream_t stream, const mx_conv_cfg* cfg) {
  Cfg cf;
  int rc = resolve_cfg(cfg, cf);
  if (rc) return rc;
  rc = conv_check(s);
  if (rc) return rc;
  MX_CHECK_ARG(s->C % 8 == 0, "conv fwd x3: C=%lld must be a multiple of 8 (pad the input channels)", (long long)s->C);
  MX_CHECK_ARG(s->K % 8 == 0 || !residual, "conv fwd x3: residual needs K %% 8 == 0");
  MX_CHECK_ARG(x && w && y, "conv fwd x3: null operand");
  ConvP p{};
  fill_fwd(p, s, x, w);
  p.bias = bias; p.residual = residual; p.act = act; p.out = y; p.out_f32 = 1; p.stats = stats;
  p.wt_plane = p.Ncol * p.Kdim;
  g_launch_count = 0;
  return launch_igemm_x3<0>(cf, p, make_geo_x3(cf, p.M, p.Ncol, p.Kdim), ws, ws_bytes, (hipStream_t)stream);
}

extern "C" int mx_conv2d_dgrad_x3(const mx_conv_shape* s, const float* dy, const uint16_t* wt, const float* residual,
                                  float* dx, const float* y, const float* z, const float* mean, const float* invstd,
                                  int act, float* part, int64_t part_mb, void* ws, size_t ws_bytes, mx_stream_t stream,
                                  const mx_conv_cfg* cfg) {
  Cfg cf;
  int rc = resolve_cfg(cfg, cf);
  if (rc) return rc;
  rc = conv_check(s);
  if (rc) return rc;
  MX_CHECK_ARG(s->K % 8 == 0 && s->C % 8 == 0, "conv dgrad x3: K and C must be multiples of 8");
  MX_CHECK_ARG(s->stride_h <= 2 && s->stride_w <= 2, "conv dgrad x3: strides 1 and 2 are supported");
  const BnbArgs b{y, z, mean, invstd, act, part, part_mb};
  const bool bnb = part != nullptr;
  if (bnb) {
    MX_CHECK_ARG(s->stride_h == 1 && s->stride_w == 1, "conv dgrad x3 bnb: stride 1 only");
    MX_CHECK_ARG(y && z && mean && invstd && act >= 0 && act <= 2, "conv dgrad x3 bnb: bad BN arguments");
    MX_CHECK_ARG(part_mb == cdiv(s->N * s->H * s->W, 64), "conv dgrad x3 bnb: part rows must be cdiv(N*H*W, 64)");
  }
  DClass cl[4];
  const int n = dgrad_launch_classes(s, cl);
  g_launch_count = 0;
  for (int i = 0; i < n; ++i) {
    ConvP p{};
    fill_dgrad_class(p, s, cl[i], dy, wt, residual, dx, bnb ? &b : nullptr);
    p.out_f32 = 1; p.wt_plane = s->C * s->R * s->S * s->K;
    rc = launch_igemm_x3<1>(cf, p, make_geo_x3(cf, p.M, p.Ncol, p.Kdim), ws, ws_bytes, (hipStream_t)stream);
    if (rc) return rc;
  }
  return MX_OK;
}

static bool dgrad_x3_rows_pick(const Cfg& cf, const mx_conv_shape* s, Geo* out) {
  if (s->stride_h != 1 || s->stride_w != 1 || s->K % 32 || s->C % 8 || s->R * s->S > 64 || s->R * s->S < 1) return false;
  if (s->H != s->Ho || s->W != s->Wo) return false;
  const int64_t M = s->N * s->H * s->W, Kdim = s->R * s->S * s->K;
  const bool buf = cf.loader >= 1 && cf.loader != 2 && cf.loader != 3 && M * s->K * 4 < (1ll << 31) && M > 0 &&
                   2 * s->C * Kdim < (1ll << 30);
  const Geo g = make_geo_x3(cf, M, s->C, Kdim);
  if (!buf || g.splits != 1 || cf.k.stages != 0 || g.bn != 128 || (g.bmt != 128 && g.bmt != 64)) return false;
  if (out) *out = g;
  return true;
}

extern "C" int mx_conv2d_dgrad_x3_rows_supported(const mx_conv_shape* s, const mx_conv_cfg* cfg) {
  Cfg cf;
  if (!s || resolve_cfg(cfg, cf) || conv_check(s)) return 0;
  return dgrad_x3_rows_pick(cf, s, nullptr) ? 1 : 0;
}

extern "C" int mx_conv2d_dgrad_x3_rows(const mx_conv_shape* s, const float* dy, const uint16_t* wt, const float* residual,
                                       float* dx, const int32_t* rows, const int32_t* nrows, int64_t cap,
                                       mx_stream_t stream, const mx_conv_cfg* cfg) {
  Cfg cf;
  int rc = resolve_cfg(cfg, cf);
  if (rc) return rc;
  rc = conv_check(s);
  if (rc) return rc;
  MX_CHECK_ARG(dy && wt && dx && rows && nrows, "conv dgrad x3 rows: null operand");
  Geo g;
  if (!dgrad_x3_rows_pick(cf, s, &g)) {
    set_error("conv dgrad x3 rows: the dense launch of this shape and cfg has no rows form");
    return MX_EUNSUPPORTED;
  }
  DClass cl[4];
  const int n = dgrad_launch_classes(s, cl);
  MX_CHECK_ARG(n == 1 && cl[0].Hc == s->H && cl[0].Wc == s->W, "conv dgrad x3 rows: one stride-1 class expected");
  ConvP p{};
  fill_dgrad_class(p, s, cl[0], dy, wt, residual, dx, nullptr);
  p.out_f32 = 1; p.wt_plane = s->C * s->R * s->S * s->K;
  MX_CHECK_ARG(cap >= 0 && cap <= p.M, "conv dgrad x3 rows: capacity %lld outside [0, %lld]", (long long)cap, (long long)p.M);
  MX_CHECK_ARG(p.Kdim == s->R * s->S * s->K && p.M < (1ll << 31), "conv dgrad x3 rows: unexpected class geometry");
  p.rows = rows; p.rows_count = nrows; p.rows_cap = cap;
  p.splits = 1; p.kt_per_split = p.Kdim / 32; p.slab = nullptr; p.korder = cf.korder;
  g_launch_count = 0;
  if (cap == 0) return MX_OK;
  const int64_t blocks = rpn_rows_grid(cap, g.bmt) * cdiv(p.Ncol, (int64_t)g.bn);
  hipStream_t st = (hipStream_t)stream;
  if (g.bmt == 128) {
    constexpr size_t lds = std::max<size_t>((size_t)2 * 2 * (128 + 128) * 64, (size_t)128 * (128 + 4) * 4);
    conv_x3_buf_kernel<128, 1, 2, 2, 128, 4, 1, true><<<(unsigned)blocks, 256, lds, st>>>(p);
  } else {
    constexpr size_t lds = std::max<size_t>((size_t)3 * 2 * (64 + 128) * 64, (size_t)64 * (128 + 4) * 4);
    conv_x3_buf_kernel<128, 1, 3, 2, 64, 4, 1, true><<<(unsigned)blocks, 256, lds, st>>>(p);
  }
  MX_LAUNCH_CHECK();
  record_launch(1, g.bmt, g.bn, 1, blocks, true, 107);
  return MX_OK;
}

extern "C" int mx_conv2d_wgrad_x3(const mx_conv_shape* s, const float* dy, const float* x, float* dw, int64_t Kout,
                                  int64_t Cin, int layout, void* ws, size_t ws_bytes, mx_stream_t stream,
                                  const mx_conv_cfg* cfg) {
  const char* name = "conv wgrad x3";
  Cfg cf;
  int rc = resolve_cfg(cfg, cf);
  if (!rc) rc = wgrad_check(s, Kout, Cin, layout, name);
  if (rc) return rc;
  hipStream_t st = (hipStream_t)stream;
  WgP p{};
  WGeo g;
  rc = fill_wgrad(p, g, cf, wgrad_geo_x3, s, dy, x, dw, Kout, Cin, layout, ws, ws_bytes, name, "mx_conv_workspace_x3");
  if (!rc) rc = wgrad_x3_ranges(p, g, name);
  if (rc) return rc;
  const bool wide = wgrad_x3_wide(cf), ww = wgrad_x3_ww(cf);
  if (ww)
    conv_wgrad_x3ww_kernel<<<(unsigned)(g.tiles * g.splits), 256, 2 * 8 * 32 * 256, st>>>(p);
  else if (wide)
    conv_wgrad_x3w_kernel<<<(unsigned)(g.tiles * g.splits), 512, 2 * 6 * 32 * 256, st>>>(p);
  else
    conv_wgrad_x3_kernel<<<(unsigned)(g.tiles * g.splits), NT, 2 * 4 * 32 * 256, st>>>(p);
  MX_LAUNCH_CHECK();
  g_launch_count = 0;
  record_launch(2, ww ? 256 : 128, (ww || wide) ? 256 : 128, g.splits, g.tiles, true, 100 + (ww ? 5 : wide ? 4 : 3));
  return wgrad_finish(p, g, Kout, st, name);
}

extern "C" int mx_conv2d_wgrad_x3_rows(const mx_conv_shape* s, const float* dy, const float* x, float* dw, int64_t Kout,
                                       int64_t Cin, int layout, const int32_t* tiles, const int32_t* ntiles, int64_t cap,
                                       void* ws, size_t ws_bytes, mx_stream_t stream, const mx_conv_cfg* cfg) {
  const char* name = "conv wgrad x3 rows";
  Cfg cf;
  int rc = resolve_cfg(cfg, cf);
  if (!rc) rc = wgrad_check(s, Kout, Cin, layout, name);
  if (rc) return rc;
  MX_CHECK_ARG(dy && x && dw && tiles && ntiles, "conv wgrad x3 rows: null operand");
  MX_CHECK_ARG(!wgrad_x3_wide(cf) && !wgrad_x3_ww(cf),
               "conv wgrad x3 rows: only the 128 x 128 kernel (wgrad_variant 3) has a tile-list form");
  bool dense;
  wgrad_shape(s, &dense);
  MX_CHECK_ARG(!dense, "conv wgrad x3 rows: a dense (FC-style) conv has no pixel axis to list");
  const int64_t ksteps = cdiv(s->N * s->Ho * s->Wo, 32);
  MX_CHECK_ARG(cap >= 0 && cap <= ksteps, "conv wgrad x3 rows: capacity %lld outside [0, %lld]", (long long)cap,
               (long long)ksteps);
  WgP p{};
  WGeo g;
  rc = fill_wgrad(p, g, cf, wgrad_geo_x3, s, dy, x, dw, Kout, Cin, layout, ws, ws_bytes, name, "mx_conv_workspace_x3");
  if (!rc) rc = wgrad_x3_ranges(p, g, name);
  if (rc) return rc;
  p.rows = tiles; p.nrows = ntiles; p.rows_cap = cap;
  hipStream_t st = (hipStream_t)stream;
  conv_wgrad_x3_rows_kernel<<<(unsigned)(g.tiles * g.splits), NT, 2 * 4 * 32 * 256, st>>>(p);
  MX_LAUNCH_CHECK();
  g_launch_count = 0;
  record_launch(2, 128, 128, g.splits, g.tiles, true, 106);
  return wgrad_finish(p, g, Kout, st, name);
}

extern "C" int mx_conv2d_stem_x3(const mx_conv_shape* s, const float* x, const uint16_t* w, const float* bias,
                                 int act, float* y, float* stats, mx_stream_t stream) {
  int rc = conv_check(s);
  if (rc) return rc;
  MX_CHECK_ARG(s->R == 7 && s->S == 7 && s->K == STEM_K, "conv stem x3: a 7x7 conv to 64 channels is required");
  MX_CHECK_ARG(s->C >= 4 && s->C % 4 == 0, "conv stem x3: input channel stride C=%lld must be a multiple of 4",
               (long long)s->C);
  MX_CHECK_ARG(act == 0 || act == 1, "conv stem x3: act 0 (none) or 1 (relu)");
  MX_CHECK_ARG(x && w && y, "conv stem x3: null operand");
  MX_CHECK_ARG(s->N * s->H * s->W * s->C * 4 < (1ll << 31), "conv stem x3: input must stay below 2 GiB");
  StemP p{};
  p.x = x; p.w = w; p.bias = bias; p.y = y; p.stats = stats;
  p.M = s->N * s->Ho * s->Wo;
  p.mblocks = cdiv(p.M, SROWS);
  p.H = (int)s->H; p.W = (int)s->W; p.C = (int)s->C; p.Ho = (int)s->Ho; p.Wo = (int)s->Wo;
  p.st_h = s->stride_h; p.st_w = s->stride_w; p.pad_h = s->pad_h; p.pad_w = s->pad_w; p.act = act;
  p.xbytes = (int)(s->N * s->H * s->W * s->C * 4);
  const int64_t ntiles = cdiv(p.M, 16 * STEM_T);
  const int64_t slots = 2 * (int64_t)num_cus();
  p.tiles_per_block = std::max<int64_t>(4, cdiv(ntiles, slots));
  const int64_t blocks = cdiv(ntiles, p.tiles_per_block);
  conv_stem_x3_kernel<<<(unsigned)blocks, 256, 0, (hipStream_t)stream>>>(p);
  MX_LAUNCH_CHECK();
  return MX_OK;
}
```

### robust-object-detection_amd/mx_det/_lib.py

```python
import ctypes
import os

_HERE = os.path.dirname(os.path.abspath(__file__))
LIB_PATH = os.environ.get("MX_DET_LIB") or os.path.join(_HERE, "libmx_det.so")

c_i64 = ctypes.c_int64
c_int = ctypes.c_int
c_f = ctypes.c_float
c_d = ctypes.c_double
c_vp = ctypes.c_void_p
c_sz = ctypes.c_size_t
c_u64 = ctypes.c_uint64
F4 = ctypes.c_float * 4


class ConvShape(ctypes.Structure):
    _fields_ = [("N", c_i64), ("H", c_i64), ("W", c_i64), ("C", c_i64), ("K", c_i64), ("R", c_i64), ("S", c_i64),
                ("Ho", c_i64), ("Wo", c_i64), ("stride_h", ctypes.c_int32), ("stride_w", ctypes.c_int32),
                ("pad_h", ctypes.c_int32), ("pad_w", ctypes.c_int32)]


class ConvCfg(ctypes.Structure):
    _fields_ = [("tile_rows", ctypes.c_int32), ("tile_cols", ctypes.c_int32), ("max_splits", ctypes.c_int32),
                ("stages", ctypes.c_int32), ("wgrad_variant", ctypes.c_int32), ("reserved", ctypes.c_int32),
# ... 148 lines not shown
    "mx_jpeg_reconstruct_window": (c_int, [c_vp, c_vp, c_int, c_int, c_int, c_int, c_int, c_int, c_vp, c_i64, c_vp]),
    "mx_jpeg_window_cover": (c_int, [c_vp, c_int, c_int, c_int, c_int, c_vp]),
    "mx_jpeg_entropy_decode_workspace": (c_sz, [c_vp, c_i64]),
    "mx_jpeg_entropy_decode": (c_int, [c_vp, c_i64, c_vp, c_vp, c_sz, c_vp, c_vp, c_vp]),
    "mx_jpeg_entropy_decode_set_subseq": (c_int, [c_int]),
    "mx_jpeg_decode_coefs_chunked": (c_int, [c_vp, c_i64, c_vp, c_int, c_vp, c_vp]),
    "mx_jpeg_encode_info": (c_int, [c_int, c_int, c_int, c_int, c_vp]),
    "mx_jpeg_write_header": (c_int, [c_vp, c_vp, c_i64, c_vp]),
    "mx_jpeg_scan_bound": (c_i64, [c_vp]),
    "mx_jpeg_encode_coefs": (c_int, [c_vp, c_vp, c_vp, c_i64, c_vp]),
    "mx_jpeg_forward": (c_int, [c_vp, c_int, c_vp, c_vp, c_vp]),
    "mx_jpeg_entropy_workspace": (c_sz, [c_vp]),
    "mx_jpeg_entropy": (c_int, [c_vp, c_vp, c_vp, c_sz, c_vp, c_i64, c_vp, c_vp]),
    "mx_corrupt_jpeg_workspace": (c_sz, [c_i64, c_i64, c_i64, c_int]),
    "mx_corrupt_jpeg_u8": (c_int, [c_vp, c_i64, c_i64, c_i64, c_vp, c_int, c_int, c_vp, c_sz, c_vp, c_vp]),
    "mx_conv_set_wgrad_variant": (c_int, [c_int]),
    "mx_conv_get_wgrad_variant": (c_int, []),
    "mx_conv_set_wgrad_target": (c_int, [c_i64]),
    "mx_conv_last_launch": (c_int, [c_vp]),
    "mx_conv2d_wgrad_ex": (c_int, [ctypes.POINTER(ConvShape), c_vp, c_vp, c_vp, c_i64, c_i64, c_int, c_vp,
                                   ctypes.c_size_t, c_vp, c_cfg]),
    "mx_conv_transpose_weight": (c_int, [c_vp, c_i64, c_i64, c_i64, c_vp, c_vp]),
    "mx_conv_pack_weight": (c_int, [c_vp, c_vp, c_i64, c_i64, c_vp, c_vp, c_int, c_vp]),
    "mx_conv_dgrad_weight_elems": (ctypes.c_size_t, [c_vp, c_i64, c_i64]),
    "mx_conv_pack_plan_bytes": (ctypes.c_size_t, [c_i64]),
    "mx_conv_pack_batched": (c_int, [c_vp, c_i64, c_vp, ctypes.c_size_t, c_int, c_vp]),
    "mx_conv2d_dgrad_bnb": (c_int, [ctypes.POINTER(ConvShape), c_vp, c_vp, c_vp, c_vp, c_vp, c_vp, c_vp, c_vp, c_int,
                                    c_vp, c_i64, c_vp, c_sz, c_vp, c_cfg]),
    "mx_rpn_loss_workspace": (c_sz, [c_i64]),
    "mx_rpn_loss_fwd": (c_int, [c_vp, c_vp, c_vp, c_vp, c_vp, c_vp, c_i64, c_f, c_vp, c_vp, c_sz, c_vp]),
    "mx_rpn_loss_bwd": (c_int, [c_vp, c_vp, c_vp, c_vp, c_vp, c_vp, c_i64, c_f, c_vp, c_vp, c_vp, c_vp, c_vp]),
    "mx_roi_loss_fwd": (c_int, [c_vp, c_i64, c_int, c_vp, c_i64, c_vp, c_vp, c_i64, c_f, c_vp, c_vp, c_sz, c_vp]),
    "mx_roi_loss_bwd": (c_int, [c_vp, c_i64, c_int, c_vp, c_i64, c_vp, c_vp, c_i64, c_f, c_vp, c_vp, c_vp, c_vp]),
    "mx_bn_bwd_finalize": (c_int, [c_vp, c_i64, c_i64, c_i64, c_vp, c_vp, c_vp, c_vp, c_vp, c_vp, c_sz, c_vp]),
    "mx_conv2d_dgrad_ex": (c_int, [ctypes.POINTER(ConvShape), c_vp, c_vp, c_vp, c_vp, c_vp, c_sz, c_vp, c_cfg]),
    "mx_conv2d_dgrad_t": (c_int, [ctypes.POINTER(ConvShape), c_vp, c_vp, c_vp, c_vp, c_sz, c_vp]),
    "mx_maxpool_fwd": (c_int, [c_vp, c_int, c_i64, c_i64, c_i64, c_i64, c_int, c_int, c_int, c_vp, c_vp, c_vp]),
    "mx_maxpool_bwd": (c_int, [c_vp, c_int, c_vp, c_i64, c_i64, c_i64, c_i64, c_int, c_int, c_int, c_vp, c_vp]),
    "mx_upsample_nearest_fwd": (c_int, [c_vp, c_int, c_i64, c_i64, c_i64, c_i64, c_i64, c_i64, c_vp, c_vp, c_vp]),
    "mx_upsample_nearest_bwd": (c_int, [c_vp, c_int, c_i64, c_i64, c_i64, c_i64, c_i64, c_i64, c_vp, c_vp]),
    "mx_reflect_pad_u8": (c_int, [c_vp, c_i64, c_i64, c_i64, c_i64, c_i64, c_i64, c_vp, c_vp]),
    "mx_up_concat": (c_int, [c_vp, c_vp, c_int, c_i64, c_i64, c_i64, c_i64, c_i64, c_vp, c_vp]),
    "mx_up_concat_bwd": (c_int, [c_vp, c_int, c_i64, c_i64, c_i64, c_i64, c_i64, c_vp, c_vp, c_vp]),
    "mx_restore_finish": (c_int, [c_vp, c_i64, c_i64, c_i64, c_vp, c_i64, c_i64, c_vp, c_vp]),
    "mx_ssim_workspace": (c_sz, [c_i64, c_i64, c_i64, c_i64]),
    "mx_ssim_l1_fwd": (c_int, [c_vp, c_vp, c_i64, c_i64, c_i64, c_i64, c_int, c_f, c_f, c_f, c_f, c_vp, c_vp, c_vp,
                               c_sz, c_vp]),
    "mx_ssim_l1_bwd": (c_int, [c_vp, c_vp, c_vp, c_i64, c_i64, c_i64, c_i64, c_int, c_f, c_vp, c_f, c_f, c_vp, c_vp]),
    "mx_bn_finalize": (c_int, [c_vp, c_i64, c_i64, c_i64, c_vp, c_vp, c_f, c_f, c_vp, c_vp, c_vp, c_vp, c_vp, c_vp,
                               c_vp]),
    "mx_bn_finalize_workspace": (ctypes.c_size_t, [c_i64, c_i64]),
    "mx_bn_finalize_ex": (c_int, [c_vp, c_i64, c_i64, c_i64, c_vp, c_vp, c_f, c_f, c_vp, c_vp, c_vp, c_vp, c_vp, c_vp,
                                  c_vp, ctypes.c_size_t, c_vp]),
    "mx_bn_finalize_adapt": (c_int, [c_vp, c_i64, c_i64, c_i64, c_vp, c_vp, c_f, c_vp, c_vp, c_d, c_d, c_vp, c_vp, c_vp,
                                     c_vp, c_vp, c_vp, ctypes.c_size_t, c_vp]),
    "mx_act_bias_bwd_workspace": (ctypes.c_size_t, [c_i64, c_i64]),
    "mx_act_bias_bwd": (c_int, [c_vp, c_vp, c_int, c_i64, c_i64, c_i64, c_int, c_vp, c_int, c_vp, c_vp,
                                ctypes.c_size_t, c_vp]),
    "mx_sgd_step": (c_int, [c_vp, c_vp, c_vp, c_vp, c_vp, c_i64, c_f, c_f, c_f, c_f, c_int, c_vp]),
    "mx_sgd_pack_plan_bytes": (ctypes.c_size_t, [c_i64]),
    "mx_sgd_pack_build": (c_int, [c_vp, c_i64, c_vp, c_vp, ctypes.c_size_t, c_vp, c_vp]),
    "mx_sgd_pack_step": (c_int, [c_vp, c_vp, c_i64, c_i64, ctypes.c_size_t, c_f, c_f, c_f, c_f, c_int, c_vp]),
    "mx_adamw_step": (c_int, [c_vp, c_vp, c_vp, c_vp, c_vp, c_vp, c_i64, c_d, c_d, c_d, c_d, c_d, c_vp]),
    "mx_adamw_pack_plan_bytes": (ctypes.c_size_t, [c_i64]),
    "mx_adamw_pack_build": (c_int, [c_vp, c_i64, c_vp, c_vp, ctypes.c_size_t, c_vp, c_vp]),
    "mx_adamw_pack_step": (c_int, [c_vp, c_vp, c_i64, c_i64, ctypes.c_size_t, c_i64, c_d, c_d, c_d, c_d, c_d, c_vp]),
    "mx_bn_apply": (c_int, [c_vp, c_int, c_i64, c_i64, c_vp, c_vp, c_vp, c_int, c_vp, c_int, c_vp]),
    "mx_bn_act_maxpool": (c_int, [c_vp, c_i64, c_i64, c_i64, c_i64, c_vp, c_vp, c_int, c_int, c_int, c_int, c_vp,
                                  c_vp]),
    "mx_bn_bwd_reduce": (c_int, [c_vp, c_vp, c_vp, c_i64, c_i64, c_int, c_vp, c_vp, c_vp, c_vp]),
    "mx_bn_bwd_apply": (c_int, [c_vp, c_vp, c_vp, c_i64, c_i64, c_int, c_vp, c_vp, c_vp, c_vp, c_vp, c_vp, c_vp]),
    "mx_bn_bwd_workspace": (ctypes.c_size_t, [c_i64, c_i64]),
    "mx_bn_bwd_reduce_ex": (c_int, [c_vp, c_vp, c_vp, c_int, c_i64, c_i64, c_int, c_vp, c_vp, c_vp, c_vp,
                                    ctypes.c_size_t, c_vp, c_vp, c_vp]),
    "mx_bn_bwd_apply_ex": (c_int, [c_vp, c_vp, c_vp, c_int, c_i64, c_i64, c_int, c_vp, c_vp, c_vp, c_vp]),
    "mx_conv_workspace_x3": (c_sz, [ctypes.POINTER(ConvShape), c_int, c_cfg]),
    "mx_conv2d_stem_x3": (c_int, [ctypes.POINTER(ConvShape), c_vp, c_vp, c_vp, c_int, c_vp, c_vp, c_vp]),
    "mx_conv2d_fwd_x3": (c_int, [ctypes.POINTER(ConvShape), c_vp, c_vp, c_vp, c_vp, c_int, c_vp, c_vp, c_vp, c_sz,
                                 c_vp, c_cfg]),
    "mx_conv2d_dgrad_x3": (c_int, [ctypes.POINTER(ConvShape), c_vp, c_vp, c_vp, c_vp, c_vp, c_vp, c_vp, c_vp, c_int,
                                   c_vp, c_i64, c_vp, c_sz, c_vp, c_cfg]),
    "mx_conv2d_wgrad_x3": (c_int, [ctypes.POINTER(ConvShape), c_vp, c_vp, c_vp, c_i64, c_i64, c_int, c_vp, c_sz,
                                   c_vp, c_cfg]),
    "mx_rpn_rows_capacity": (c_i64, [c_i64, c_i64, c_int]),
    "mx_rpn_rows_workspace": (c_sz, [c_i64]),
    "mx_rpn_rows_build": (c_int, [c_vp, c_i64, c_i64, c_i64, c_i64, c_int, c_vp, c_i64, c_vp, c_i64, c_vp, c_i64, c_vp,
                                  c_vp, c_vp, c_sz, c_vp]),
    "mx_rpn_tiles_capacity": (c_i64, [c_i64, c_i64, c_int]),
    "mx_rpn_tiles_build": (c_int, [c_vp, c_i64, c_i64, c_i64, c_i64, c_int, c_vp, c_i64, c_vp, c_i64, c_vp, c_i64, c_vp,
                                   c_vp, c_vp, c_sz, c_vp]),
    "mx_conv2d_wgrad_x3_rows": (c_int, [ctypes.POINTER(ConvShape), c_vp, c_vp, c_vp, c_i64, c_i64, c_int, c_vp, c_vp,
                                        c_i64, c_vp, c_sz, c_vp, c_cfg]),
    "mx_rpn_lists_build": (c_int, [c_vp, c_i64, c_i64, c_i64, c_i64, c_vp, c_i64, c_vp, c_i64, c_vp, c_i64, c_vp, c_vp,
                                   c_i64, c_vp, c_i64, c_vp, c_vp, c_vp, c_sz, c_vp]),
    "mx_conv2d_dgrad_x3_rows_supported": (c_int, [ctypes.POINTER(ConvShape), c_cfg]),
    "mx_conv2d_dgrad_x3_rows": (c_int, [ctypes.POINTER(ConvShape), c_vp, c_vp, c_vp, c_vp, c_vp, c_vp, c_i64, c_vp,
                                        c_cfg]),
    "mx_act_bias_bwd_rows": (c_int, [c_vp, c_vp, c_vp, c_i64, c_i64, c_i64, c_vp, c_vp, c_i64, c_vp, c_vp, c_vp, c_sz,
                                     c_vp]),
    "mx_coco_match": (c_int, [c_vp, c_vp, c_vp, c_i64, c_vp, c_vp, c_vp, c_vp, c_vp, c_i64, c_i64, c_vp, c_i64, c_vp,
                              c_i64, c_i64, c_i64, c_vp, c_vp, c_vp, c_vp]),
    "mx_coco_accumulate_workspace": (c_sz, [c_i64]),
    "mx_coco_accumulate": (c_int, [c_vp, c_vp, c_vp, c_vp, c_vp, c_vp, c_i64, c_i64, c_i64, c_vp, c_vp, c_i64, c_i64,
                                   c_i64, c_vp, c_i64, c_vp, c_i64, c_vp, c_vp, c_vp, c_vp, c_sz, c_vp]),
}

_lib = None


class MxError(RuntimeError):
    pass


def _cfg_optional(fn, nargs):
    def entry(*a):
        return fn(*a) if len(a) == nargs else fn(*a, None)
    return entry


def load():
    global _lib
    if _lib is None:
        import torch
        if not os.path.exists(LIB_PATH):
            raise MxError(f"libmx_det.so not built at {LIB_PATH}; run `python -c 'import __graft_entry__ as g; g.build()'`")
        lib = ctypes.CDLL(LIB_PATH, mode=ctypes.RTLD_GLOBAL)
        for name, (res, args) in _SIGS.items():
            if not hasattr(lib, name):
                continue
            fn = getattr(lib, name)
            fn.restype = res
            fn.argtypes = args
            if args and args[-1] is c_cfg:
                setattr(lib, name, _cfg_optional(fn, len(args)))
        _lib = lib
    return _lib


def declared_symbols():
    return list(_SIGS)


_fns = {}


def call(name, *args):
    fn = _fns.get(name)
    if fn is None:
        lib = load()
        if not hasattr(lib, name):
            raise MxError(f"libmx_det.so does not export {name}")
        fn = _fns[name] = getattr(lib, name)
    rc = fn(*args)
    if rc != 0:
        msg = load().mx_last_error().decode(errors="replace")
        raise MxError(f"{name} failed ({rc}): {msg}")
    return rc


def ptr(t):
    return t.data_ptr() if t is not None else None


def stream():
    import torch
    return torch._C._cuda_getCurrentRawStream(torch._C._cuda_getDevice())
# ... 5 lines not shown
```

### robust-object-detection_amd/mx_det/conv.py

```python
import contextlib
import ctypes
import gc
import os
import threading
import weakref

import torch

from . import _lib
from ._lib import call

ACT_NONE, ACT_RELU, ACT_LEAKY = 0, 1, 2
MX_F32, MX_BF16 = 0, 1


def dcode(t):
    if t.dtype == torch.float32:
        return MX_F32
    if t.dtype == torch.bfloat16:
        return MX_BF16
    raise RuntimeError(f"unsupported activation dtype {t.dtype}")


def is_x3(t):
# ... 261 lines not shown
        K, C, R, S = e.w.shape
        return PackDesc(e.w.data_ptr(), e.wk.data_ptr(), e.wt.data_ptr() if e.wt is not None else None,
                        C, K, e.cp, e.kp, R, S, e.stride[0], e.stride[1], e.pad[0], e.pad[1],
                        (1 if e.dense else 0) | (2 if e.split else 0))

    def fusable(self, params):
        by_ptr = {}
        for k in self.order:
            e = self.entries[k]
            by_ptr.setdefault(e.w.data_ptr(), []).append(e)
        out = []
        for p in params:
            es = by_ptr.get(p.data_ptr(), ())
            e = es[0] if len(es) == 1 else None
            if e is not None and not (e.w.numel() == p.numel() and e.w.is_contiguous() and p.is_contiguous()
                                      and e.w.shape[2] * e.w.shape[3] <= 49):
                e = None
            out.append(e)
        return out

    @staticmethod
    def mark_packed(entries):
        for e in entries:
            if e is not None:
                e.version = e.w._version

    def refresh(self):
        dirty = [k for k in self.order if self.entries[k].version != self.entries[k].w._version]
        if not dirty:
            return
        upload = tuple(dirty) != self._plan_key
        if upload:
            descs = (PackDesc * len(dirty))()
            for i, k in enumerate(dirty):
                descs[i] = self.desc(self.entries[k])
            nb = _lib.load().mx_conv_pack_plan_bytes(len(dirty))
            self._plan = torch.empty(nb, dtype=torch.uint8, device=self.entries[dirty[0]].w.device)
            self._descs = descs
            self._plan_key = tuple(dirty)
        call("mx_conv_pack_batched", ctypes.cast(self._descs, ctypes.c_void_p), len(dirty), _p(self._plan),
             self._plan.numel(), int(upload), _s())
        for k in dirty:
            e = self.entries[k]
            e.version = e.w._version

    def lookup(self, w, cp, kp, stride, pad, dgrad, dense=False, split=False):
        e = self.entries.get(self.key(w, cp, kp, stride, pad, split))
        if e is None or e.version != w._version or (dgrad and (e.wt is None or e.dense != dense)):
            return None
        return e.wk, e.wt


_packer = None


def set_packer(p):
    global _packer
    _packer = p


def get_packer():
    return _packer


def operands(w, cin_pad, stride, pad, kpad, dgrad, dense=False, split=False):
    if _packer is not None:
        r = _packer.lookup(w, cin_pad, kpad, stride, pad, dgrad, dense, split)
        if r is not None:
            return r
    if dense and dgrad:
        wk, _ = pack_weight(w, cin_pad, stride, pad, split=split)
        K = w.shape[0]
        planes = wk.view(2 if split else 1, K, -1)
        wt = torch.nn.functional.pad(planes.transpose(1, 2), (0, kpad - K)).contiguous().view(-1)
        return wk, wt
    return pack_weight(w, cin_pad, stride, pad, kpad=kpad, dgrad=dgrad, split=split)


def _is_dense(x_shape, R, S, stride, pad):
    return (x_shape[1], x_shape[2]) == (R, S) and tuple(pad) == (0, 0) and R * S > 1


def conv_dgrad(dy, wt, x_shape, R, S, stride, pad, residual=None, bnb=None, rows=None, rows_fill=True,
               rows_inplace=False):
    N, H, W, C = x_shape
    K = dy.shape[3]
    x3 = is_x3(dy)
    assert wt.numel() == (2 if x3 else 1) * C * R * S * K, (wt.numel(), C, R, S, K)
    Ho, Wo = out_hw(H, W, R, S, stride, pad)
    sh = _lib.ConvShape(N, H, W, C, K, R, S, Ho, Wo, stride[0], stride[1], pad[0], pad[1])
    dyc = dy.contiguous()
    if rows is not None and x3 and bnb is None:
        if residual is not None:
            assert residual.dtype == dy.dtype and residual.shape == (N, H, W, C) and residual.is_contiguous()
        key = ("dgrad", dy.dtype, N, H, W, C, K, R, S, tuple(stride), tuple(pad), residual is not None, False)
        c = None
        if _tune_on():
            def trial(c_):
                cfg_ = _fd_cfg(c_)
                wsb_ = _lib.load().mx_conv_workspace_x3(ctypes.byref(sh), 1, cfg_)
                ws_ = torch.empty(wsb_, dtype=torch.uint8, device=dy.device) if wsb_ else None
                tmp = torch.empty((N, H, W, C), dtype=dy.dtype, device=dy.device)
                call("mx_conv2d_dgrad_x3", ctypes.byref(sh), _p(dyc), _p(wt), _p(residual), _p(tmp), None, None, None,
                     None, 0, None, 0, _p(ws_), wsb_, _s(), cfg_)
            c = _pick(key, _FD_CANDS_X3, trial)
        cfg = _fd_cfg(c)
        if _lib.load().mx_conv2d_dgrad_x3_rows_supported(ctypes.byref(sh), cfg):
            t0 = _timer.start() if _timer else None
            if residual is not None:
                dx = residual if rows_inplace else residual.clone()
            elif rows_fill:
                dx = torch.zeros((N, H, W, C), dtype=dy.dtype, device=dy.device)
            else:
                dx = torch.empty((N, H, W, C), dtype=dy.dtype, device=dy.device)
            call("mx_conv2d_dgrad_x3_rows", ctypes.byref(sh), _p(dyc), _p(wt), _p(dx) if residual is not None else None,
                 _p(dx), _p(rows[0]), _p(rows[1]), rows[2], _s(), cfg)
            if _timer:
                _timer.stop("x3_dgrad", 2.0 * rows[2] * K * R * S * C, t0, _tag(N, H, W, C, K, R, S, stride),
                            dy.numel() * dy.element_size() + wt.numel() * 2 + rows[2] * C * 4)
            return dx
    dx = torch.empty((N, H, W, C), dtype=dy.dtype, device=dy.device)
    t0 = _timer.start() if _timer else None
    if residual is not None:
        assert residual.dtype == dy.dtype and residual.shape == dx.shape and residual.is_contiguous()
    part, mb = None, (N * H * W + 63) // 64
    if bnb is not None:
        part = torch.empty((2, mb, C), dtype=torch.float32, device=dy.device)

    def run(c):
        cfg = _fd_cfg(c)
        if x3:
            wsb = _lib.load().mx_conv_workspace_x3(ctypes.byref(sh), 1, cfg)
            ws = torch.empty(wsb, dtype=torch.uint8, device=dy.device) if wsb else None
            b = bnb if part is not None else None
            call("mx_conv2d_dgrad_x3", ctypes.byref(sh), _p(dyc), _p(wt), _p(residual), _p(dx),
                 _p(b.y) if b else None, _p(b.z) if b else None, _p(b.mean) if b else None,
                 _p(b.invstd) if b else None, int(b.act) if b else 0, _p(part), mb, _p(ws), wsb, _s(), cfg)
            return
        wsb = _lib.load().mx_conv_workspace(ctypes.byref(sh), 1, cfg)
        ws = torch.empty(wsb, dtype=torch.uint8, device=dy.device) if wsb else None
        if part is not None:
            call("mx_conv2d_dgrad_bnb", ctypes.byref(sh), _p(dyc), _p(wt), _p(residual), _p(dx), _p(bnb.y),
                 _p(bnb.z), _p(bnb.mean), _p(bnb.invstd), int(bnb.act), _p(part), mb, _p(ws), wsb, _s(), cfg)
        else:
            call("mx_conv2d_dgrad_ex", ctypes.byref(sh), _p(dyc), _p(wt), _p(residual), _p(dx), _p(ws), wsb, _s(), cfg)

    key = ("dgrad", dy.dtype, N, H, W, C, K, R, S, tuple(stride), tuple(pad), residual is not None, part is not None)
    _tuned(key, _FD_CANDS_X3 if x3 else _FD_CANDS, run)
    if part is not None:
        bnb.part = part
    if _timer:
        _timer.stop(("x3_" if x3 else "") + "dgrad", 2.0 * N * Ho * Wo * K * R * S * C, t0,
                    _tag(N, H, W, C, K, R, S, stride),
                    dy.numel() * dy.element_size() + wt.numel() * 2 + dx.numel() * dx.element_size())
    return dx


_pending = []
if hasattr(torch.autograd.graph, "set_warn_on_accumulate_grad_stream_mismatch"):
    torch.autograd.graph.set_warn_on_accumulate_grad_stream_mismatch(False)
_dp = False


def set_data_parallel(flag):
    global _dp
    _dp = bool(flag)


class _Uses:
    __slots__ = ("n", "__weakref__")

    def __init__(self):
        self.n = 0


_uses = weakref.WeakValueDictionary()


def _count_use(w):
    c = _uses.get(id(w))
    if c is None:
        c = _uses[id(w)] = _Uses()
    c.n += 1
    return c


def side_wgrad_enabled(ctx):
    uses, ctx.uses = ctx.uses, None
    if os.environ.get("MX_SIDE_WGRAD", "1") == "0" or _timer is not None:
        return False
    w = ctx.wref()
    if w is None or not w.is_leaf or w.grad is not None or uses is None or uses.n != 1:
        return False
    import torch.distributed as dist
    return _dp or not (dist.is_available() and dist.is_initialized() and dist.get_world_size() > 1)


def grad_dest(ctx):
    uses = ctx.uses
    if uses is None or uses.n != 1:
        return None
    w = ctx.wref()
    if w is None:
        return None
    p = w if w.is_leaf else w._base
    slot = getattr(p, "_mx_grad_slot", None) if p is not None else None
    if slot is None or not p.is_leaf or p.grad is not None or not w.is_contiguous() or w.numel() != p.numel():
        return None
    flat, off = slot
    return flat.narrow(0, off, p.numel()).view(w.shape)


def wgrad_stream(device):
    return dedicated_stream(device, "wgrad")


def _wgrad_plan(ctx, dy, x, K, R, S, stride, pad, kout=None, cin=None, rows=None):
    if not ctx.needs_input_grad[1]:
        return None
    dst = grad_dest(ctx)
    side = side_wgrad_enabled(ctx)
    if side and os.environ.get("MX_WGRAD_FORK", "early") != "late":
        job = wgrad_prepare(dy, x, K, R, S, stride, pad, kout, cin, dst, rows)
        fork = torch.cuda.Event()
        fork.record()
        return job, side, fork
    return (dy, x, K, R, S, stride, pad, kout, cin, dst, rows), side, None


def _wgrad_run(plan):
    job, side, fork = plan
    if not isinstance(job, _WgradJob):
        job = wgrad_prepare(*job)
    return wgrad_launch(job, side, fork)


def _join_side():
    cur = torch.cuda.current_stream()
    for ev, _keep in _pending:
        cur.wait_event(ev)
    _pending.clear()


class _WgradJob:
    __slots__ = ("sh", "x3", "entry", "dw", "dyc", "x", "ws", "wsb", "cfg", "kout", "cin", "K", "R", "S", "stride",
                 "t0", "rows")


def wgrad_prepare(dy, x, K, R, S, stride, pad, kout=None, cin=None, out=None, rows=None):
    j = _WgradJob()
    sh = j.sh = shape(x, K, R, S, stride, pad)
    j.kout = kout = kout or K
    j.cin = cin = cin or x.shape[3]
    j.K, j.R, j.S, j.stride = K, R, S, stride
    j.x3 = x3 = is_x3(x)
    assert dy.dtype == x.dtype, (dy.dtype, x.dtype)
    wsfn = "mx_conv_workspace_x3" if x3 else "mx_conv_workspace"
    j.entry = entry = "mx_conv2d_wgrad_x3" if x3 else "mx_conv2d_wgrad_ex"
    if out is not None:
        assert out.shape == (kout, cin, R, S) and out.dtype == torch.float32 and out.is_contiguous(), out.shape
        dw = out
    else:
        dw = torch.empty((kout, cin, R, S), dtype=torch.float32, device=x.device)
    j.dw = dw
    j.x = x
    j.dyc = dyc = dy.contiguous()
    j.t0 = _timer.start() if _timer else None
    j.rows = None
    key = ("wgrad", x.dtype, sh.N, sh.H, sh.W, x.shape[3], K, R, S, tuple(stride), tuple(pad))
    def trial(c):
        cfg_ = _wg_cfg(c)
        wsb_ = getattr(_lib.load(), wsfn)(ctypes.byref(sh), 2, cfg_)
        ws_ = torch.empty(wsb_, dtype=torch.uint8, device=x.device) if wsb_ else None
        call(entry, ctypes.byref(sh), _p(dyc), _p(x), _p(dw), kout, cin, 1, _p(ws_), wsb_, _s(), cfg_)
    j.cfg = _wg_cfg(_pick(key, _WG_CANDS_X3 if x3 else _WG_CANDS, trial) if _tune_on() else None)
    j.wsb = getattr(_lib.load(), wsfn)(ctypes.byref(sh), 2, j.cfg)
    j.ws = torch.empty(j.wsb, dtype=torch.uint8, device=x.device) if j.wsb else None
    if rows is not None and x3 and (j.cfg is None or j.cfg.wgrad_variant == 3):
        j.rows, j.entry = rows, "mx_conv2d_wgrad_x3_rows"
    return j


def wgrad_launch(j, side=False, fork=None):
    stream = _s()
    if side:
        st = wgrad_stream(j.x.device)
        if fork is not None:
            st.wait_event(fork)
        else:
            st.wait_stream(torch.cuda.current_stream())
        stream = st.cuda_stream
    rows = j.rows
    if rows is not None:
        call(j.entry, ctypes.byref(j.sh), _p(j.dyc), _p(j.x), _p(j.dw), j.kout, j.cin, 1, _p(rows[0]), _p(rows[1]),
             rows[2], _p(j.ws), j.wsb, stream, j.cfg)
    else:
        call(j.entry, ctypes.byref(j.sh), _p(j.dyc), _p(j.x), _p(j.dw), j.kout, j.cin, 1, _p(j.ws), j.wsb, stream,
             j.cfg)
    if side:
        ev = torch.cuda.Event()
        ev.record(st)
        if not _pending:
            torch.autograd.Variable._execution_engine.queue_callback(_join_side)
        _pending.append((ev, (j.dyc, j.x, j.ws, rows)))
    dw, sh, x, dyc, K, R, S, stride, t0 = j.dw, j.sh, j.x, j.dyc, j.K, j.R, j.S, j.stride, j.t0
    x3 = j.x3
    j.dw = None
    if _timer:
        px = min(rows[2] * 32, sh.N * sh.Ho * sh.Wo) if rows is not None else sh.N * sh.Ho * sh.Wo
        _timer.stop(("x3_" if x3 else "") + "wgrad", 2.0 * px * K * R * S * x.shape[3], t0,
                    _tag(sh.N, sh.H, sh.W, x.shape[3], K, R, S, stride),
                    dyc.numel() * dyc.element_size() + x.numel() * x.element_size() + dw.numel() * 4)
    return dw


def conv_wgrad(dy, x, K, R, S, stride, pad, kout=None, cin=None, side=False, out=None, rows=None):
    return wgrad_launch(wgrad_prepare(dy, x, K, R, S, stride, pad, kout, cin, out, rows), side)


def act_bias_bwd(gy, y, act, K8, need_db, g_dtype=torch.bfloat16):
    K = gy.shape[-1]
    gy = gy.contiguous()
    M = gy.numel() // K
    assert gy.dtype in (torch.bfloat16, torch.float32) and y.dtype == gy.dtype and y.shape == gy.shape
    g = torch.empty(gy.shape[:-1] + (K8,), dtype=g_dtype, device=gy.device)
    db = torch.empty(K, dtype=torch.float32, device=gy.device) if need_db else None
    ws = None
    if need_db:
        ws = bn_scratch(_lib.load().mx_act_bias_bwd_workspace(M, K), gy.device)
    call("mx_act_bias_bwd", _p(gy), _p(y.contiguous()) if act else None, dcode(gy), M, K, K8, int(act), _p(g),
         dcode(g), _p(db), _p(ws), ws.numel() if ws is not None else 0, _s())
    return g, db


def act_bias_bwd_rows(gy, y, need_db, rows, mask=None):
    K = gy.shape[-1]
    gy = gy.contiguous()
    M = gy.numel() // K
    assert gy.dtype == torch.float32 and y.dtype == gy.dtype and y.shape == gy.shape and K % 8 == 0
    g = torch.zeros(gy.shape, dtype=gy.dtype, device=gy.device)
    db = torch.empty(K, dtype=torch.float32, device=gy.device) if need_db else None
# ... 370 lines not shown
    t = _scratch.get(key)
    if t is None or t.numel() < nbytes:
        if torch.cuda.is_current_stream_capturing():
            raise RuntimeError("bn_scratch: first use of a stream inside a graph capture (warm the capture "
                               "up on conv.capture_stream(device) first)")
        if t is not None:
            _scratch_kept.append(t)
        t = torch.zeros(max(nbytes, 1 << 20), dtype=torch.uint8, device=device)
        _scratch[key] = t
    return t


def bn_train_finalize(st, K, M, gamma, beta, eps, momentum, rmean, rvar):
    mean = torch.empty(K, dtype=torch.float32, device=st.device)
    invstd, scale, shift = torch.empty_like(mean), torch.empty_like(mean), torch.empty_like(mean)
    fws = bn_scratch(_lib.load().mx_bn_finalize_workspace(st.shape[1], K), st.device)
    call("mx_bn_finalize_ex", _p(st), st.shape[1], K, M, _p(gamma.detach()), _p(beta.detach()), float(eps),
         float(momentum), _p(rmean), _p(rvar), _p(mean), _p(invstd), _p(scale), _p(shift), _p(fws), fws.numel(), _s())
    return mean, invstd, scale, shift


def bn_adapting(bn):
    ad = bn.__dict__.get("_mx_adapt")
    return ad if ad is not None and ad.owner.enabled else None


def bn_adapt_finalize(st, K, M, images, bn, ad):
    scale = torch.empty(K, dtype=torch.float32, device=st.device)
    shift = torch.empty_like(scale)
    ad.prepare(K, st.device)
    n = ad.count(images)
    fws = bn_scratch(_lib.load().mx_bn_finalize_workspace(st.shape[1], K), st.device)
    call("mx_bn_finalize_adapt", _p(st), st.shape[1], K, M, _p(bn.weight.detach()), _p(bn.bias.detach()), float(bn.eps),
         _p(bn.running_mean), _p(bn.running_var), float(ad.owner.prior), float(n), _p(ad.state), _p(ad.mean),
         _p(ad.var), _p(scale), _p(shift), _p(fws), fws.numel(), _s())
    return scale, shift


def _no_grad_inputs(x, conv, bn):
    if torch.is_grad_enabled() and x.requires_grad:
        raise RuntimeError("test-time BatchNorm adaptation has no backward: run it under torch.no_grad() "
                           "(the input of an adapted conv + BatchNorm requires grad)")
    if conv.bias is not None:
        raise ValueError("test-time BatchNorm adaptation: the conv in front of an adapted BatchNorm has no bias")


def adapt_conv_bn(x, conv, bn, act, residual, ad):
    _no_grad_inputs(x, conv, bn)
    if ad.frozen:
        return eval_conv_bn(x, conv, bn, act, residual, ad.mean, ad.var)
    w = conv.weight
    wk, _ = operands(w, x.shape[3], conv.stride, conv.padding, _ceil8(w.shape[0]), False, split=is_x3(x))
    z, st = conv_fwd(x.contiguous(), wk, conv.stride, conv.padding, stats=True, cin=w.shape[1])
    K = w.shape[0]
    M = z.numel() // K
    scale, shift = bn_adapt_finalize(st, K, M, z.shape[0], bn, ad)
    y = torch.empty_like(z)
    res = residual.contiguous() if residual is not None else None
    call("mx_bn_apply", _p(z), dcode(z), M, K, _p(scale), _p(shift), _p(res), int(act), _p(y), dcode(y), _s())
    return y


def conv_bn_act_maxpool(x, conv, bn, act, k, st, pd, adapt=None):
    assert is_x3(x) and (bn.training or adapt is not None)
    if adapt is not None:
        _no_grad_inputs(x, conv, bn)
    elif bn.num_batches_tracked is not None and not batch_counted(bn):
        bn.num_batches_tracked.add_(1)
    w = conv.weight
    wk, _ = operands(w, x.shape[3], conv.stride, conv.padding, _ceil8(w.shape[0]), False, split=True)
    z, stt = conv_fwd(x.contiguous(), wk, conv.stride, conv.padding, stats=True, cin=w.shape[1])
    N, H, W, K = z.shape
    if adapt is not None:
        scale, shift = bn_adapt_finalize(stt, K, N * H * W, N, bn, adapt)
    else:
        _, _, scale, shift = bn_train_finalize(stt, K, N * H * W, bn.weight, bn.bias, bn.eps, bn.momentum,
                                               bn.running_mean, bn.running_var)
    Ho, Wo = (H + 2 * pd - k) // st + 1, (W + 2 * pd - k) // st + 1
    y = torch.empty((N, Ho, Wo, K), dtype=torch.float32, device=z.device)
    call("mx_bn_act_maxpool", _p(z), N, H, W, K, _p(scale), _p(shift), int(act), k, st, pd, _p(y), _s())
    return y


class ConvBNAct(torch.autograd.Function):

    @staticmethod
    def forward(ctx, x, w, gamma, beta, residual, rmean, rvar, stride, pad, act, eps, momentum, link=None,
                bnb_own=None, bnb_feed=None):
        need_dx = ctx.needs_input_grad[0]
        ctx.link, ctx.role = link if link is not None else (None, None)
        ctx.bnb_own, ctx.bnb_feed = bnb_own, bnb_feed
        wk, wt = operands(w, x.shape[3], stride, pad, _ceil8(w.shape[0]), need_dx, split=is_x3(x))
        z, st = conv_fwd(x, wk, stride, pad, stats=True, cin=w.shape[1])
        K = w.shape[0]
        M = z.numel() // K
        mean, invstd, scale, shift = bn_train_finalize(st, K, M, gamma, beta, eps, momentum, rmean, rvar)
        y = torch.empty_like(z)
        res = residual.contiguous() if residual is not None else None
        t0 = _timer.start() if _timer else None
        call("mx_bn_apply", _p(z), dcode(z), M, K, _p(scale), _p(shift), _p(res), int(act), _p(y), dcode(y), _s())
        if _timer:
            _timer.stop("bn_apply", M * K * z.element_size() * (2 + (1 if res is not None else 0)), t0, f"{M}x{K}")
        ctx.save_for_backward(x, wt if need_dx else None, z, y, mean, invstd, gamma)
        ctx.cfg = (stride, pad, act, w.shape, residual is not None)
        if bnb_own is not None:
            bnb_own.y, bnb_own.z, bnb_own.mean, bnb_own.invstd, bnb_own.act = y, z, mean, invstd, act
        ctx.wref, ctx.uses = weakref.ref(w), _count_use(w)
        ctx.chain = _chain_join(x) if _chains and need_dx else None
        return y

    @staticmethod
    def backward(ctx, gy):
        x, wt, z, y, mean, invstd, gamma = ctx.saved_tensors
        stride, pad, act, wshape, has_res = ctx.cfg
        K, _, R, S = wshape
        M = z.numel() // K
        gy = gy.to(z.dtype).contiguous()
        sums = torch.empty((2, K), dtype=torch.float32, device=z.device)
        coef = torch.empty((3, K), dtype=torch.float32, device=z.device)
        own = ctx.bnb_own
        if own is not None and own.part is not None:
            part, own.part = own.part, None
            mb = part.shape[1]
            ws = bn_scratch(_lib.load().mx_bn_finalize_workspace(mb, K), z.device)
            call("mx_bn_bwd_finalize", _p(part), mb, K, M, _p(mean), _p(invstd), _p(gamma.detach()), _p(sums),
                 _p(coef), _p(ws), ws.numel(), _s())
        else:
            wsb = _lib.load().mx_bn_bwd_workspace(M, K)
            ws = bn_scratch(wsb, z.device)
            t0 = _timer.start() if _timer else None
            call("mx_bn_bwd_reduce_ex", _p(gy), _p(y), _p(z), dcode(z), M, K, int(act), _p(mean), _p(invstd),
                 _p(gamma.detach()), _p(ws), ws.numel(), _p(sums), _p(coef), _s())
            if _timer:
                _timer.stop("bn_bwd_reduce", M * K * z.element_size() * (3 if act else 2), t0, f"{M}x{K}")
        dz = torch.empty_like(z)
        dres = torch.empty_like(z) if has_res else None
        t0 = _timer.start() if _timer else None
        call("mx_bn_bwd_apply_ex", _p(gy), _p(y), _p(z), dcode(z), M, K, int(act), _p(coef), _p(dz), _p(dres), _s())
        if _timer:
            _timer.stop("bn_bwd_apply", M * K * z.element_size() * (4 + (1 if has_res else 0)), t0, f"{M}x{K}")
        dx = dw = None
        wg = _wgrad_plan(ctx, dz, x, K, R, S, stride, pad, cin=wshape[1])
        link = ctx.link
        if ctx.role == "sink" and dres is not None:
            link.dres, dres = dres, None
        if ctx.needs_input_grad[0]:
            res = None
            if ctx.role == "src":
                res, link.dres = link.dres, None
            feed = ctx.bnb_feed
            chain = ctx.chain
            bnb = feed if (feed is not None and feed.y is not None and tuple(stride) == (1, 1)
                           and feed.y.shape == x.shape and (chain is None or chain.last())) else None
            dx = conv_dgrad(dz, wt, x.shape, R, S, stride, pad, residual=_chain_res(chain, res), bnb=bnb)
            if chain is not None:
                dx = chain.hand(dx)
        if wg is not None:
            dw = _wgrad_run(wg)
        dgamma = sums[1] if ctx.needs_input_grad[2] else None
        dbeta = sums[0] if ctx.needs_input_grad[3] else None
        return dx, dw, dgamma, dbeta, dres, None, None, None, None, None, None, None, None, None, None


class Conv2d(torch.nn.Module):

    def __init__(self, cin, cout, k, stride=1, padding=0, bias=True, act=ACT_NONE, out_dtype=None):
        super().__init__()
        k = (k, k) if isinstance(k, int) else tuple(k)
        self.stride = (stride, stride) if isinstance(stride, int) else tuple(stride)
        self.padding = (padding, padding) if isinstance(padding, int) else tuple(padding)
        self.weight = torch.nn.Parameter(torch.empty(cout, cin, *k))
        self.bias = torch.nn.Parameter(torch.zeros(cout)) if bias else None
        self.act = act
        self.out_dtype = out_dtype
        torch.nn.init.kaiming_uniform_(self.weight, a=5 ** 0.5)

    def forward(self, x, be):
        return be.conv(x, self.weight, self.bias, self.stride, self.padding, self.act, self.out_dtype)


class BatchNorm2d(torch.nn.Module):

    def __init__(self, c, eps=1e-5, momentum=0.1):
        super().__init__()
        self.eps, self.momentum = eps, momentum
        self.weight = torch.nn.Parameter(torch.ones(c))
        self.bias = torch.nn.Parameter(torch.zeros(c))
        self.register_buffer("running_mean", torch.zeros(c))
        self.register_buffer("running_var", torch.ones(c))
        self.register_buffer("num_batches_tracked", torch.tensor(0, dtype=torch.long))


_nbt_token = object()


def count_batches(bns):
    global _nbt_token
    t = [b.num_batches_tracked for b in bns if b.num_batches_tracked is not None]
    if t:
        torch._foreach_add_(t, 1)
    _nbt_token = tok = object()
    for b in bns:
        b.__dict__["_mx_nbt"] = tok


def batch_counted(bn):
    return bn.__dict__.get("_mx_nbt") is _nbt_token


class ResLink:

    def __init__(self):
        self.dres = None

    def bind(self, role):
        return (self, role)


class BNBLink:

    def __init__(self):
        self.y = self.z = self.mean = self.invstd = self.part = None
        self.act = 0


def conv_bn(x, conv, bn, act, residual=None, link=None, bnb_own=None, bnb_feed=None):
    if bn.training:
        if bn.num_batches_tracked is not None and not batch_counted(bn):
            bn.num_batches_tracked.add_(1)
        return ConvBNAct.apply(x, conv.weight, bn.weight, bn.bias, residual, bn.running_mean, bn.running_var,
                               conv.stride, conv.padding, act, bn.eps, bn.momentum, link, bnb_own, bnb_feed)
    ad = bn_adapting(bn)
    if ad is not None:
        return adapt_conv_bn(x, conv, bn, act, residual, ad)
    return eval_conv_bn(x, conv, bn, act, residual)


# ... 39 lines not shown
```

Measured before the change: 105.6 images/sec.

## Emit BN-backward gradient as pre-split bf16 hi/lo planes for x3 dgrad and wgrad

The BN backward apply kernel gains a split mode that writes dz directly as two bf16 planes (hi and lo) instead of f32. The x3 dgrad and wgrad conv kernels gain template variants that consume these planes directly, skipping their own per-tile f32-to-bf16x3 splitting and halving the bytes loaded per dy element per plane. A planner enables the path only when tuned configs are known and the shapes are supported. It adds kernel variants and coupling between the BN and conv stages, and if the planner's checks and the kernels' support rules disagree, precision or correctness could suffer.

Measured after the change: 106.5 images/sec (median of 6 runs). About the same (+0.9%).

```diff
diff --git a/include/mx_det.h b/include/mx_det.h
--- a/include/mx_det.h
+++ b/include/mx_det.h
@@ -296,6 +296,15 @@
                        int64_t part_mb, void* ws, size_t ws_bytes, mx_stream_t stream, const mx_conv_cfg* cfg);
 int mx_conv2d_wgrad_x3(const mx_conv_shape* s, const float* dy, const float* x, float* dw, int64_t Kout, int64_t Cin,
                        int layout, void* ws, size_t ws_bytes, mx_stream_t stream, const mx_conv_cfg* cfg);
+int mx_conv2d_dgrad_x3_split(const mx_conv_shape* s, const uint16_t* dy, const uint16_t* wt, const float* residual,
+                             float* dx, const float* y, const float* z, const float* mean, const float* invstd, int act,
+                             float* part, int64_t part_mb, void* ws, size_t ws_bytes, mx_stream_t stream,
+                             const mx_conv_cfg* cfg);
+int mx_conv2d_wgrad_x3_split(const mx_conv_shape* s, const uint16_t* dy, const float* x, float* dw, int64_t Kout,
+                             int64_t Cin, int layout, void* ws, size_t ws_bytes, mx_stream_t stream,
+                             const mx_conv_cfg* cfg);
+int mx_conv2d_x3_split_supported(const mx_conv_shape* s, int passes, const mx_conv_cfg* dgrad_cfg,
+                                 const mx_conv_cfg* wgrad_cfg);
 
 int64_t mx_rpn_rows_capacity(int64_t P, int64_t NB, int level);
 size_t mx_rpn_rows_workspace(int64_t P);
@@ -368,6 +377,8 @@
                         float* sums, float* coef, mx_stream_t stream);
 int mx_bn_bwd_apply_ex(const void* dy, const void* y, const void* x, int dtype, int64_t M, int64_t K, int act,
                        const float* coef, void* dx, void* dres, mx_stream_t stream);
+int mx_bn_bwd_apply_split(const float* dy, const float* y, const float* x, int64_t M, int64_t K, int act,
+                          const float* coef, uint16_t* dz, float* dres, mx_stream_t stream);
 size_t mx_act_bias_bwd_workspace(int64_t M, int64_t K);
 int mx_act_bias_bwd(const void* gy, const void* y, int dtype, int64_t M, int64_t K, int64_t K8, int act,
                     void* g, int gdtype, float* db, void* ws, size_t ws_bytes, mx_stream_t stream);
diff --git a/robust-object-detection_amd/csrc/mx_bn.hip b/robust-object-detection_amd/csrc/mx_bn.hip
--- a/robust-object-detection_amd/csrc/mx_bn.hip
+++ b/robust-object-detection_amd/csrc/mx_bn.hip
@@ -411,7 +411,7 @@
   if (threadIdx.x < 64 && k < K) db[k] = (float)fin[0][col];
 }
 
-template <int ACT, typename T>
+template <int ACT, typename T, bool SPLIT = false>
 __global__ void __launch_bounds__(256) bn_bwd_apply2_kernel(const T* __restrict__ dy, const T* __restrict__ y,
                                                             const T* __restrict__ x, int64_t n8, int K8,
                                                             const float* __restrict__ coef, T* __restrict__ dx,
@@ -436,7 +436,16 @@
     og[q] = vd[q] * act_grad<ACT>(vy[q]);
     o[q] = A[q] * og[q] + B[q] * vx[q] + C[q];
   }
-  st8(dx + e * 8, o);
+  if constexpr (SPLIT) {
+    static_assert(sizeof(T) == 4, "split planes: f32 gradients only");
+    uint4 h, l;
+    split8(make_float4(o[0], o[1], o[2], o[3]), make_float4(o[4], o[5], o[6], o[7]), h, l);
+    uint16_t* hi = (uint16_t*)dx;
+    *(uint4*)(hi + e * 8) = h;
+    *(uint4*)(hi + (n8 + e) * 8) = l;
+  } else {
+    st8(dx + e * 8, o);
+  }
   if (dres) st8(dres + e * 8, og);
 }
 
@@ -818,6 +827,24 @@
   return MX_OK;
 }
 
+extern "C" int mx_bn_bwd_apply_split(const float* dy, const float* y, const float* x, int64_t M, int64_t K, int act,
+                                     const float* coef, uint16_t* dz, float* dres, mx_stream_t stream) {
+  MX_CHECK_ARG(K % 8 == 0 && K > 0 && K < (1 << 24), "bn_bwd_apply_split: K must be a positive multiple of 8");
+  MX_CHECK_ARG(act >= 0 && act <= 2, "bn_bwd_apply_split: act 0/1/2");
+  MX_CHECK_ARG(act == 0 || y, "bn_bwd_apply_split: y required for an activation");
+  if (M == 0) return MX_OK;
+  const int64_t n8 = M * (K / 8);
+  const int K8 = (int)(K / 8);
+  const unsigned blocks = (unsigned)cdiv(n8, 256);
+  hipStream_t st = (hipStream_t)stream;
+  float* out = (float*)dz;
+  if (act == 1) bn_bwd_apply2_kernel<1, float, true><<<blocks, 256, 0, st>>>(dy, y, x, n8, K8, coef, out, dres);
+  else if (act == 2) bn_bwd_apply2_kernel<2, float, true><<<blocks, 256, 0, st>>>(dy, y, x, n8, K8, coef, out, dres);
+  else bn_bwd_apply2_kernel<0, float, true><<<blocks, 256, 0, st>>>(dy, y, x, n8, K8, coef, out, dres);
+  MX_LAUNCH_CHECK();
+  return MX_OK;
+}
+
 extern "C" int mx_bn_bwd_reduce(const uint16_t* dy, const uint16_t* y, const uint16_t* x, int64_t M, int64_t K, int act,
                                 const float* mean, const float* invstd, float* sums, mx_stream_t stream) {
   MX_CHECK_ARG(K % 8 == 0 && K > 0, "bn_bwd_reduce: K must be a positive multiple of 8");
diff --git a/robust-object-detection_amd/csrc/mx_conv.hip b/robust-object-detection_amd/csrc/mx_conv.hip
--- a/robust-object-detection_amd/csrc/mx_conv.hip
+++ b/robust-object-detection_amd/csrc/mx_conv.hip
@@ -1563,7 +1563,7 @@
   return g ^ (g >> 1);
 }
 
-template <int BN, int MODE, int STAGES, int OCC, int BMT, int WR = 2, int WC = 2, bool ROWS = false>
+template <int BN, int MODE, int STAGES, int OCC, int BMT, int WR = 2, int WC = 2, bool ROWS = false, bool ASPLIT = false>
 __global__ void __launch_bounds__(64 * WR * WC, OCC) conv_x3_buf_kernel(ConvP p) {
 #if defined(__HIP_DEVICE_COMPILE__)
   extern __shared__ __attribute__((aligned(16))) char smem[];
@@ -1574,6 +1574,8 @@
   constexpr int AH = BMT * RB, BP = BN * RB, STAGE = 2 * AH + 2 * BP;
   constexpr int WN = BN / WC, TJ = WN / 16, WM = BMT / WR, TI = WM / 16;
   static_assert(AI >= 1 && BI >= 1 && STAGES >= 2, "tile shape");
+  static_assert(!ASPLIT || MODE == 1, "pre-split A operand: dgrad only");
+  constexpr int AEB = ASPLIT ? 2 : 4;
   const int tid = threadIdx.x, lane = tid & 63, wave = tid >> 6;
   const int wm = wave / WC, wn = wave % WC;
   const int64_t ntiles_n = (p.Ncol + BN - 1) / BN;
@@ -1584,12 +1586,12 @@
   const int64_t m0 = mt * BMT, n0 = nt * BN;
   int64_t nrows = p.M;
   if constexpr (ROWS) {
-    static_assert(MODE == 1, "rows form: dgrad only");
+    static_assert(MODE == 1 && !ASPLIT, "rows form: dgrad only, f32 operand");
     nrows = min<int64_t>(max<int64_t>((int64_t)*p.rows_count, 0), p.rows_cap);
     if (m0 >= nrows) return;
   }
   const int lrow = lane >> 2, pc = lane & 3;
-  const int qa = pc ^ x3_swz(lrow), qb = pc ^ tile_swz<4>(lrow);
+  const int qb = pc ^ tile_swz<4>(lrow), qa = ASPLIT ? qb : pc ^ x3_swz(lrow);
   const int IH = (int)p.IH, IW = (int)p.IW, IC = (int)p.IC, R = p.R, S = p.S;
   uint32_t a_voff[AI];
   uint64_t a_mask[AI];
@@ -1610,14 +1612,14 @@
       const int n = (int)(t / p.OH);
       const int h0 = MODE == 0 ? oh * p.st_h - p.pad_h : oh + p.pad_h - (R - 1);
       const int w0 = MODE == 0 ? ow * p.st_w - p.pad_w : ow + p.pad_w - (S - 1);
-      off = ((n * IH + h0) * IW + w0) * IC + qa * 4;
+      off = ((n * IH + h0) * IW + w0) * IC + qa * (16 / AEB);
       for (int r = 0; r < R; ++r)
         for (int q = 0; q < S; ++q) {
           const int rr = MODE == 0 ? r : R - 1 - r, qq = MODE == 0 ? q : S - 1 - q;
           if ((unsigned)(h0 + rr) < (unsigned)IH && (unsigned)(w0 + qq) < (unsigned)IW) mask |= 1ull << (r * S + q);
         }
     }
-    a_voff[i] = (uint32_t)off * 4u;
+    a_voff[i] = (uint32_t)off * (uint32_t)AEB;
     a_mask[i] = mask;
   }
   uint32_t b_voff[BI];
@@ -1626,7 +1628,8 @@
     const int64_t n = n0 + wave * BR + i * RPI + lrow;
     b_voff[i] = n < p.Ncol ? (uint32_t)((n * p.Kdim + qb * 8) * 2) : kOOB;
   }
-  const i32x4 arsrc = dma_rsrc(p.src, (uint32_t)(p.src_elems * 4));
+  const i32x4 arsrc = dma_rsrc(p.src, (uint32_t)(p.src_elems * AEB));
+  const i32x4 alrsrc = dma_rsrc(p.src + (ASPLIT ? p.src_elems : 0), (uint32_t)(p.src_elems * AEB));
   const i32x4 bhrsrc = dma_rsrc(p.wt, (uint32_t)(p.wt_elems * 2));
   const i32x4 blrsrc = dma_rsrc(p.wt + p.wt_plane, (uint32_t)(p.wt_elems * 2));
   const uint32_t lds0 = lds_addr(smem);
@@ -1642,7 +1645,7 @@
     const uint32_t B = A + 2 * AH;
     const int cr = kp.cr, cq = kp.cq, cc = kp.cc;
     const int rr = MODE == 0 ? cr : R - 1 - cr, qq = MODE == 0 ? cq : S - 1 - cq;
-    const uint32_t a_soff = (uint32_t)(((rr * IW + qq) * IC + cc) * 4);
+    const uint32_t a_soff = (uint32_t)(((rr * IW + qq) * IC + cc) * AEB);
     const int tap = cr * S + cq;
     const uint32_t b_soff = (uint32_t)__builtin_amdgcn_readfirstlane((int)((tap * IC + cc) * 2));
     if (!(dbg & 8)) {
@@ -1652,7 +1655,8 @@
       const uint32_t v = a_voff[i] + a_soff;
       const uint32_t dst = A + (wave * AR + i * RPI) * RB;
       lds_dma16(arsrc, dst, ok ? v : kOOB, 0u);
-      lds_dma16(arsrc, dst + AH, ok ? v + 64u : kOOB, 0u);
+      if constexpr (ASPLIT) lds_dma16(alrsrc, dst + AH, ok ? v : kOOB, 0u);
+      else lds_dma16(arsrc, dst + AH, ok ? v + 64u : kOOB, 0u);
     }
     }
     if (!(dbg & 4)) {
@@ -1698,6 +1702,12 @@
 #pragma unroll
     for (int i = 0; i < TI; ++i) {
       const int row = wm * WM + i * 16 + (lane & 15);
+      if constexpr (ASPLIT) {
+        const int off = row * RB + ((g ^ tile_swz<4>(row)) << 4);
+        ah[i] = *(const bf16x8*)(A + off);
+        al[i] = *(const bf16x8*)(A + AH + off);
+        continue;
+      }
       const int f = x3_swz(row);
       const float4 u = *(const float4*)(Ag + row * RB + ((q0 ^ f) << 4));
       const float4 w = *(const float4*)(Ag + row * RB + (((q0 + 1) ^ f) << 4));
@@ -1749,8 +1759,18 @@
 }
 
 #if defined(__HIP_DEVICE_COMPILE__)
-template <bool ROWS>
+template <bool DSPLIT>
+__device__ __forceinline__ void dy_planes(const float4 a, const float4 b, uint4& hi, uint4& lo) {
+  if constexpr (DSPLIT) {
+    hi = __builtin_bit_cast(uint4, a);
+    lo = __builtin_bit_cast(uint4, b);
+  } else {
+    split8(a, b, hi, lo);
+  }
+}
+template <bool ROWS, bool DSPLIT = false>
 __device__ __forceinline__ void wgrad_x3_body(const WgP& p) {
+  static_assert(!(ROWS && DSPLIT), "tile-list form: f32 dy only");
   extern __shared__ __attribute__((aligned(16))) char smem[];
   constexpr int PXT = 32, OPB = PXT * 256, STAGE = 4 * OPB;
   const int tid = threadIdx.x, lane = tid & 63, wave = tid >> 6;
@@ -1790,7 +1810,11 @@
   const int r = tap / p.S, s = tap - (tap / p.S) * p.S;
   const bool k_ok = (k0 + ch * 8) < p.K;
   const int OW = (int)p.OW, OH = (int)p.OH, H = (int)p.H, W = (int)p.W, C = (int)p.C;
-  const __amdgpu_buffer_rsrc_t dyr = __builtin_amdgcn_make_buffer_rsrc((void*)dy, (short)0, (int)(p.P * p.K * 4), 0x00020000);
+  constexpr uint32_t DEB = DSPLIT ? 2u : 4u;
+  const __amdgpu_buffer_rsrc_t dyr =
+      __builtin_amdgcn_make_buffer_rsrc((void*)dy, (short)0, (int)(p.P * p.K * DEB), 0x00020000);
+  const __amdgpu_buffer_rsrc_t dylr = __builtin_amdgcn_make_buffer_rsrc((void*)(p.dy + (DSPLIT ? p.P * p.K : 0)), (short)0,
+                                                                        (int)(p.P * p.K * DEB), 0x00020000);
   const __amdgpu_buffer_rsrc_t xr =
       __builtin_amdgcn_make_buffer_rsrc((void*)x, (short)0, (int)(p.N * p.H * p.W * p.C * 4), 0x00020000);
   const int dw = PXT % OW, dh = (PXT / OW) % OH, dn = PXT / (OW * OH);
@@ -1806,7 +1830,7 @@
     px_n[i] = (int)(t / OH);
   }
   const int pend32 = (int)pend;
-  const uint32_t dy_col = (uint32_t)(k0 + ch * 8) * 4u;
+  const uint32_t dy_col = (uint32_t)(k0 + ch * 8) * DEB;
   float4 rd[2][2], rx[2][2];
   auto load = [&]() {
 #pragma unroll
@@ -1820,13 +1844,14 @@
       }
       const bool pok = px_i[i] < pend32;
       const int pix = px_i[i];
-      const uint32_t od = (pok && k_ok) ? __umul24((uint32_t)pix, (uint32_t)(p.K * 4)) + dy_col : kOOB;
+      const uint32_t od = (pok && k_ok) ? __umul24((uint32_t)pix, (uint32_t)(p.K * DEB)) + dy_col : kOOB;
       const int ih = __mul24(px_oh[i], p.st_h) + ihb, iw = __mul24(px_ow[i], p.st_w) + iwb;
       const bool xok = pok && col_ok && (unsigned)ih < (unsigned)H && (unsigned)iw < (unsigned)W;
       const uint32_t ox = xok ? (uint32_t)__mul24(__mul24(px_n[i], H) + ih, W) + (uint32_t)iw : 0u;
       const uint32_t oxb = xok ? __umul24(ox, (uint32_t)(C * 4)) + (uint32_t)cc * 4u : kOOB;
       rd[i][0] = __builtin_bit_cast(float4, __builtin_amdgcn_raw_buffer_load_b128(dyr, od, 0, 0));
-      rd[i][1] = __builtin_bit_cast(float4, __builtin_amdgcn_raw_buffer_load_b128(dyr, od + 16u, 0, 0));
+      rd[i][1] = DSPLIT ? __builtin_bit_cast(float4, __builtin_amdgcn_raw_buffer_load_b128(dylr, od, 0, 0))
+                        : __builtin_bit_cast(float4, __builtin_amdgcn_raw_buffer_load_b128(dyr, od + 16u, 0, 0));
       rx[i][0] = __builtin_bit_cast(float4, __builtin_amdgcn_raw_buffer_load_b128(xr, oxb, 0, 0));
       rx[i][1] = __builtin_bit_cast(float4, __builtin_amdgcn_raw_buffer_load_b128(xr, oxb + 16u, 0, 0));
       px_i[i] += PXT;
@@ -1850,7 +1875,7 @@
       const int row = (tid >> 4) + 16 * i;
       const int off = row * 256 + (swz_w(row, ch) << 4);
       uint4 h, l;
-      split8(rd[i][0], rd[i][1], h, l);
+      dy_planes<DSPLIT>(rd[i][0], rd[i][1], h, l);
       *(uint4*)(Dh + off) = h;
       *(uint4*)(Dh + OPB + off) = l;
       split8(rx[i][0], rx[i][1], h, l);
@@ -1911,9 +1936,10 @@
   wgrad_store(p, acc, k0, c0, wm, wn, lane, split);
 }
 #endif
+template <bool DSPLIT>
 __global__ void __launch_bounds__(NT, 2) conv_wgrad_x3_kernel(WgP p) {
 #if defined(__HIP_DEVICE_COMPILE__)
-  wgrad_x3_body<false>(p);
+  wgrad_x3_body<false, DSPLIT>(p);
 #endif
 }
 __global__ void __launch_bounds__(NT, 2) conv_wgrad_x3_rows_kernel(WgP p) {
@@ -1922,6 +1948,7 @@
 #endif
 }
 
+template <bool DSPLIT>
 __global__ void __launch_bounds__(512, 1) conv_wgrad_x3w_kernel(WgP p) {
 #if defined(__HIP_DEVICE_COMPILE__)
   extern __shared__ __attribute__((aligned(16))) char smem[];
@@ -1948,7 +1975,11 @@
   const int cc = col_ok ? (int)(col - (int64_t)tap * p.C) : 0;
   const int r = tap / p.S, s = tap - (tap / p.S) * p.S;
   const int OW = (int)p.OW, OH = (int)p.OH, H = (int)p.H, W = (int)p.W, C = (int)p.C;
-  const __amdgpu_buffer_rsrc_t dyr = __builtin_amdgcn_make_buffer_rsrc((void*)dy, (short)0, (int)(p.P * p.K * 4), 0x00020000);
+  constexpr uint32_t DEB = DSPLIT ? 2u : 4u;
+  const __amdgpu_buffer_rsrc_t dyr =
+      __builtin_amdgcn_make_buffer_rsrc((void*)dy, (short)0, (int)(p.P * p.K * DEB), 0x00020000);
+  const __amdgpu_buffer_rsrc_t dylr = __builtin_amdgcn_make_buffer_rsrc((void*)(p.dy + (DSPLIT ? p.P * p.K : 0)), (short)0,
+                                                                        (int)(p.P * p.K * DEB), 0x00020000);
   const __amdgpu_buffer_rsrc_t xr =
       __builtin_amdgcn_make_buffer_rsrc((void*)x, (short)0, (int)(p.N * p.H * p.W * p.C * 4), 0x00020000);
   const int dw = PXT % OW, dh = (PXT / OW) % OH, dn = PXT / (OW * OH);
@@ -1965,13 +1996,14 @@
     px_n[i] = (int)(t / OH);
   }
   const int pend32 = (int)pend;
-  const uint32_t dy_col = (uint32_t)(k0 + chd * 8) * 4u;
+  const uint32_t dy_col = (uint32_t)(k0 + chd * 8) * DEB;
   float4 rd[2], rx[2][2];
   auto load = [&]() {
     {
-      const uint32_t od = (pxd < pend32 && k_ok) ? __umul24((uint32_t)pxd, (uint32_t)(p.K * 4)) + dy_col : kOOB;
+      const uint32_t od = (pxd < pend32 && k_ok) ? __umul24((uint32_t)pxd, (uint32_t)(p.K * DEB)) + dy_col : kOOB;
       rd[0] = __builtin_bit_cast(float4, __builtin_amdgcn_raw_buffer_load_b128(dyr, od, 0, 0));
-      rd[1] = __builtin_bit_cast(float4, __builtin_amdgcn_raw_buffer_load_b128(dyr, od + 16u, 0, 0));
+      rd[1] = DSPLIT ? __builtin_bit_cast(float4, __builtin_amdgcn_raw_buffer_load_b128(dylr, od, 0, 0))
+                     : __builtin_bit_cast(float4, __builtin_amdgcn_raw_buffer_load_b128(dyr, od + 16u, 0, 0));
       pxd += PXT;
     }
 #pragma unroll
@@ -2001,7 +2033,7 @@
     uint4 h, l;
     {
       const int off = rowd * 256 + (swz_w(rowd, chd) << 4);
-      split8(rd[0], rd[1], h, l);
+      dy_planes<DSPLIT>(rd[0], rd[1], h, l);
       *(uint4*)(D + off) = h;
       *(uint4*)(D + OPB + off) = l;
     }
@@ -2086,6 +2118,7 @@
       }
 }
 
+template <bool DSPLIT>
 __global__ void __launch_bounds__(256, 1) conv_wgrad_x3ww_kernel(WgP p) {
 #if defined(__HIP_DEVICE_COMPILE__)
   extern __shared__ __attribute__((aligned(16))) char smem[];
@@ -2111,7 +2144,11 @@
   const int cc = col_ok ? (int)(col - (int64_t)tap * p.C) : 0;
   const int r = tap / p.S, s = tap - (tap / p.S) * p.S;
   const int OW = (int)p.OW, OH = (int)p.OH, H = (int)p.H, W = (int)p.W, C = (int)p.C;
-  const __amdgpu_buffer_rsrc_t dyr = __builtin_amdgcn_make_buffer_rsrc((void*)dy, (short)0, (int)(p.P * p.K * 4), 0x00020000);
+  constexpr uint32_t DEB = DSPLIT ? 2u : 4u;
+  const __amdgpu_buffer_rsrc_t dyr =
+      __builtin_amdgcn_make_buffer_rsrc((void*)dy, (short)0, (int)(p.P * p.K * DEB), 0x00020000);
+  const __amdgpu_buffer_rsrc_t dylr = __builtin_amdgcn_make_buffer_rsrc((void*)(p.dy + (DSPLIT ? p.P * p.K : 0)), (short)0,
+                                                                        (int)(p.P * p.K * DEB), 0x00020000);
   const __amdgpu_buffer_rsrc_t xr =
       __builtin_amdgcn_make_buffer_rsrc((void*)x, (short)0, (int)(p.N * p.H * p.W * p.C * 4), 0x00020000);
   const int dw = PXT % OW, dh = (PXT / OW) % OH, dn = PXT / (OW * OH);
@@ -2127,19 +2164,20 @@
     px_n[i] = (int)(t / OH);
   }
   const int pend32 = (int)pend;
-  const uint32_t dy_col = (uint32_t)(k0 + ch * 8) * 4u;
+  const uint32_t dy_col = (uint32_t)(k0 + ch * 8) * DEB;
   float4 rd[4][2], rx[4][2];
   auto load = [&]() {
 #pragma unroll
     for (int i = 0; i < 4; ++i) {
       const bool pok = px_i[i] < pend32;
-      const uint32_t od = (pok && k_ok) ? __umul24((uint32_t)px_i[i], (uint32_t)(p.K * 4)) + dy_col : kOOB;
+      const uint32_t od = (pok && k_ok) ? __umul24((uint32_t)px_i[i], (uint32_t)(p.K * DEB)) + dy_col : kOOB;
       const int ih = __mul24(px_oh[i], p.st_h) + ihb, iw = __mul24(px_ow[i], p.st_w) + iwb;
       const bool xok = pok && col_ok && (unsigned)ih < (unsigned)H && (unsigned)iw < (unsigned)W;
       const uint32_t ox = xok ? (uint32_t)__mul24(__mul24(px_n[i], H) + ih, W) + (uint32_t)iw : 0u;
       const uint32_t oxb = xok ? __umul24(ox, (uint32_t)(C * 4)) + (uint32_t)cc * 4u : kOOB;
       rd[i][0] = __builtin_bit_cast(float4, __builtin_amdgcn_raw_buffer_load_b128(dyr, od, 0, 0));
-      rd[i][1] = __builtin_bit_cast(float4, __builtin_amdgcn_raw_buffer_load_b128(dyr, od + 16u, 0, 0));
+      rd[i][1] = DSPLIT ? __builtin_bit_cast(float4, __builtin_amdgcn_raw_buffer_load_b128(dylr, od, 0, 0))
+                        : __builtin_bit_cast(float4, __builtin_amdgcn_raw_buffer_load_b128(dyr, od + 16u, 0, 0));
       rx[i][0] = __builtin_bit_cast(float4, __builtin_amdgcn_raw_buffer_load_b128(xr, oxb, 0, 0));
       rx[i][1] = __builtin_bit_cast(float4, __builtin_amdgcn_raw_buffer_load_b128(xr, oxb + 16u, 0, 0));
       px_i[i] += PXT;
@@ -2162,7 +2200,7 @@
       const int row = row0 + 8 * i;
       const int off = row * 256 + (swz_w(row, c16) << 4);
       uint4 h, l;
-      split8(rd[i][0], rd[i][1], h, l);
+      dy_planes<DSPLIT>(rd[i][0], rd[i][1], h, l);
       *(uint4*)(D + (0 + sub) * SUB + off) = h;
       *(uint4*)(D + (2 + sub) * SUB + off) = l;
       split8(rx[i][0], rx[i][1], h, l);
@@ -3016,17 +3054,26 @@
   conv_x3_kernel<BN, MODE, BMT><<<(unsigned)blocks, NT, std::max(ring, epi), st>>>(p);
 }
 
-template <int BN, int MODE, int STAGES, int OCC, int BMT, int WR = 2, int WC = 2>
+template <int BN, int MODE, int STAGES, int OCC, int BMT, int WR = 2, int WC = 2, bool ASPLIT = false>
 static void launch_x3_buf(const ConvP& p, int64_t blocks, hipStream_t st) {
   const size_t ring = (size_t)STAGES * 2 * (BMT + BN) * 64;
   const size_t epi = (size_t)(WC == 1 ? BMT : BMT / WR) * (BN + 4) * 4;
-  conv_x3_buf_kernel<BN, MODE, STAGES, OCC, BMT, WR, WC><<<(unsigned)blocks, 64 * WR * WC, std::max(ring, epi), st>>>(p);
-}
-
-template <int MODE>
+  conv_x3_buf_kernel<BN, MODE, STAGES, OCC, BMT, WR, WC, false, ASPLIT>
+      <<<(unsigned)blocks, 64 * WR * WC, std::max(ring, epi), st>>>(p);
+}
+
+static bool x3_buf_ok(const Cfg& cf, const ConvP& p) {
+  return cf.loader >= 1 && p.IC % 32 == 0 && p.R * p.S <= 64 && p.Kdim % 32 == 0 && p.src_elems > 0 &&
+         p.src_elems * 4 < (1ll << 31) && p.wt_elems > 0 && p.wt_plane + p.wt_elems < (1ll << 30);
+}
+
+template <int MODE, bool ASPLIT = false>
 static int launch_igemm_x3(const Cfg& cf, ConvP& p, const Geo& g0, void* ws, size_t ws_bytes, hipStream_t st) {
-  const bool buf = cf.loader >= 1 && p.IC % 32 == 0 && p.R * p.S <= 64 && p.Kdim % 32 == 0 && p.src_elems > 0 &&
-                   p.src_elems * 4 < (1ll << 31) && p.wt_elems > 0 && p.wt_plane + p.wt_elems < (1ll << 30);
+  const bool buf = x3_buf_ok(cf, p);
+  if (ASPLIT && !buf && p.Kdim != 0) {
+    set_error("conv dgrad x3 split: this launch has no pre-split form (mx_conv2d_x3_split_supported)");
+    return MX_EUNSUPPORTED;
+  }
   Geo g = g0;
   if (g.bmt == 256 && !buf) {
     g.bmt = 128;
@@ -3047,21 +3094,23 @@
     p.korder = cf.korder;
     if (cf.loader == 2) p.src_elems = 0;
     if (cf.loader == 3) p.wt_elems = 0;
+#define MX_X3B(BN, ST, OCC, BMT, WR, WC) launch_x3_buf<BN, MODE, ST, OCC, BMT, WR, WC, ASPLIT>(p, blocks, st)
     if (g.bmt == 256) {
-      alt ? launch_x3_buf<128, MODE, 2, 1, 256, 4>(p, blocks, st) : launch_x3_buf<128, MODE, 3, 1, 256, 4>(p, blocks, st);
+      alt ? MX_X3B(128, 2, 1, 256, 4, 2) : MX_X3B(128, 3, 1, 256, 4, 2);
     } else if (g.bmt == 64) {
       if (g.bn == 64) {
-        if (altw) launch_x3_buf<64, MODE, 3, 3, 64, 4, 1>(p, blocks, st);
-        else alt ? launch_x3_buf<64, MODE, 4, 2, 64>(p, blocks, st) : launch_x3_buf<64, MODE, 3, 3, 64>(p, blocks, st);
-      } else if (altw) launch_x3_buf<128, MODE, 2, 3, 64, 4, 1>(p, blocks, st);
-      else if (wide64) launch_x3_buf<128, MODE, 3, 2, 64, 4, 1>(p, blocks, st);
-      else alt ? launch_x3_buf<128, MODE, 2, 3, 64>(p, blocks, st) : launch_x3_buf<128, MODE, 3, 2, 64>(p, blocks, st);
+        if (altw) MX_X3B(64, 3, 3, 64, 4, 1);
+        else alt ? MX_X3B(64, 4, 2, 64, 2, 2) : MX_X3B(64, 3, 3, 64, 2, 2);
+      } else if (altw) MX_X3B(128, 2, 3, 64, 4, 1);
+      else if (wide64) MX_X3B(128, 3, 2, 64, 4, 1);
+      else alt ? MX_X3B(128, 2, 3, 64, 2, 2) : MX_X3B(128, 3, 2, 64, 2, 2);
     } else {
-      if (g.bn == 64) alt ? launch_x3_buf<64, MODE, 2, 3, 128>(p, blocks, st) : launch_x3_buf<64, MODE, 3, 2, 128>(p, blocks, st);
-      else if (altw) launch_x3_buf<128, MODE, 3, 1, 128, 4, 1>(p, blocks, st);
-      else if (wide) launch_x3_buf<128, MODE, 2, 2, 128, 4, 1>(p, blocks, st);
-      else alt ? launch_x3_buf<128, MODE, 3, 1, 128>(p, blocks, st) : launch_x3_buf<128, MODE, 2, 2, 128>(p, blocks, st);
-    }
+      if (g.bn == 64) alt ? MX_X3B(64, 2, 3, 128, 2, 2) : MX_X3B(64, 3, 2, 128, 2, 2);
+      else if (altw) MX_X3B(128, 3, 1, 128, 4, 1);
+      else if (wide) MX_X3B(128, 2, 2, 128, 4, 1);
+      else alt ? MX_X3B(128, 3, 1, 128, 2, 2) : MX_X3B(128, 2, 2, 128, 2, 2);
+    }
+#undef MX_X3B
   } else if (g.bmt == 64) {
     if (g.bn == 64) launch_x3<64, MODE, 64>(p, blocks, st);
     else launch_x3<128, MODE, 64>(p, blocks, st);
@@ -3070,7 +3119,7 @@
     else launch_x3<128, MODE, 128>(p, blocks, st);
   }
   MX_LAUNCH_CHECK();
-  record_launch(MODE, g.bmt, g.bn, p.splits, g.tiles, buf, 100 + (buf ? cf.k.stages : 0));
+  record_launch(MODE, g.bmt, g.bn, p.splits, g.tiles, buf, (ASPLIT ? 200 : 100) + (buf ? cf.k.stages : 0));
   return launch_splitk_reduce<float>(p, g, st);
 }
 
@@ -3124,10 +3173,10 @@
   return launch_igemm_x3<0>(cf, p, make_geo_x3(cf, p.M, p.Ncol, p.Kdim), ws, ws_bytes, (hipStream_t)stream);
 }
 
-extern "C" int mx_conv2d_dgrad_x3(const mx_conv_shape* s, const float* dy, const uint16_t* wt, const float* residual,
-                                  float* dx, const float* y, const float* z, const float* mean, const float* invstd,
-                                  int act, float* part, int64_t part_mb, void* ws, size_t ws_bytes, mx_stream_t stream,
-                                  const mx_conv_cfg* cfg) {
+template <bool ASPLIT>
+static int dgrad_x3_impl(const mx_conv_shape* s, const void* dy, const uint16_t* wt, const float* residual, float* dx,
+                         const float* y, const float* z, const float* mean, const float* invstd, int act, float* part,
+                         int64_t part_mb, void* ws, size_t ws_bytes, mx_stream_t stream, const mx_conv_cfg* cfg) {
   Cfg cf;
   int rc = resolve_cfg(cfg, cf);
   if (rc) return rc;
@@ -3149,10 +3198,46 @@
     ConvP p{};
     fill_dgrad_class(p, s, cl[i], dy, wt, residual, dx, bnb ? &b : nullptr);
     p.out_f32 = 1; p.wt_plane = s->C * s->R * s->S * s->K;
-    rc = launch_igemm_x3<1>(cf, p, make_geo_x3(cf, p.M, p.Ncol, p.Kdim), ws, ws_bytes, (hipStream_t)stream);
+    rc = launch_igemm_x3<1, ASPLIT>(cf, p, make_geo_x3(cf, p.M, p.Ncol, p.Kdim), ws, ws_bytes, (hipStream_t)stream);
     if (rc) return rc;
   }
   return MX_OK;
+}
+
+extern "C" int mx_conv2d_dgrad_x3(const mx_conv_shape* s, const float* dy, const uint16_t* wt, const float* residual,
+                                  float* dx, const float* y, const float* z, const float* mean, const float* invstd,
+                                  int act, float* part, int64_t part_mb, void* ws, size_t ws_bytes, mx_stream_t stream,
+                                  const mx_conv_cfg* cfg) {
+  return dgrad_x3_impl<false>(s, dy, wt, residual, dx, y, z, mean, invstd, act, part, part_mb, ws, ws_bytes, stream, cfg);
+}
+
+static bool dgrad_x3_split_ok(const Cfg& cf, const mx_conv_shape* s) {
+  if (s->K % 8 || s->C % 8 || s->stride_h > 2 || s->stride_w > 2) return false;
+  DClass cl[4];
+  const int n = dgrad_launch_classes(s, cl);
+  for (int i = 0; i < n; ++i) {
+    ConvP p{};
+    fill_dgrad_class(p, s, cl[i], nullptr, nullptr, nullptr, nullptr, nullptr);
+    p.wt_plane = s->C * s->R * s->S * s->K;
+    if (p.Kdim != 0 && !x3_buf_ok(cf, p)) return false;
+  }
+  return n > 0;
+}
+
+extern "C" int mx_conv2d_dgrad_x3_split(const mx_conv_shape* s, const uint16_t* dy, const uint16_t* wt,
+                                        const float* residual, float* dx, const float* y, const float* z,
+                                        const float* mean, const float* invstd, int act, float* part, int64_t part_mb,
+                                        void* ws, size_t ws_bytes, mx_stream_t stream, const mx_conv_cfg* cfg) {
+  Cfg cf;
+  int rc = resolve_cfg(cfg, cf);
+  if (!rc) rc = conv_check(s);
+  if (rc) return rc;
+  if (!dgrad_x3_split_ok(cf, s)) {
+    set_error("conv dgrad x3 split: a launch of this shape and cfg has no pre-split form "
+              "(mx_conv2d_x3_split_supported)");
+    return MX_EUNSUPPORTED;
+  }
+  return dgrad_x3_impl<true>(s, dy, wt, residual, dx, y, z, mean, invstd, act, part, part_mb, ws, ws_bytes, stream, cfg);
 }
 
 static bool dgrad_x3_rows_pick(const Cfg& cf, const mx_conv_shape* s, Geo* out) {
@@ -3213,10 +3298,10 @@
   return MX_OK;
 }
 
-extern "C" int mx_conv2d_wgrad_x3(const mx_conv_shape* s, const float* dy, const float* x, float* dw, int64_t Kout,
-                                  int64_t Cin, int layout, void* ws, size_t ws_bytes, mx_stream_t stream,
-                                  const mx_conv_cfg* cfg) {
-  const char* name = "conv wgrad x3";
+template <bool DSPLIT>
+static int wgrad_x3_impl(const mx_conv_shape* s, const void* dy, const float* x, float* dw, int64_t Kout, int64_t Cin,
+                         int layout, void* ws, size_t ws_bytes, mx_stream_t stream, const mx_conv_cfg* cfg) {
+  const char* name = DSPLIT ? "conv wgrad x3 split" : "conv wgrad x3";
   Cfg cf;
   int rc = resolve_cfg(cfg, cf);
   if (!rc) rc = wgrad_check(s, Kout, Cin, layout, name);
@@ -3229,15 +3314,47 @@
   if (rc) return rc;
   const bool wide = wgrad_x3_wide(cf), ww = wgrad_x3_ww(cf);
   if (ww)
-    conv_wgrad_x3ww_kernel<<<(unsigned)(g.tiles * g.splits), 256, 2 * 8 * 32 * 256, st>>>(p);
+    conv_wgrad_x3ww_kernel<DSPLIT><<<(unsigned)(g.tiles * g.splits), 256, 2 * 8 * 32 * 256, st>>>(p);
   else if (wide)
-    conv_wgrad_x3w_kernel<<<(unsigned)(g.tiles * g.splits), 512, 2 * 6 * 32 * 256, st>>>(p);
+    conv_wgrad_x3w_kernel<DSPLIT><<<(unsigned)(g.tiles * g.splits), 512, 2 * 6 * 32 * 256, st>>>(p);
   else
-    conv_wgrad_x3_kernel<<<(unsigned)(g.tiles * g.splits), NT, 2 * 4 * 32 * 256, st>>>(p);
+    conv_wgrad_x3_kernel<DSPLIT><<<(unsigned)(g.tiles * g.splits), NT, 2 * 4 * 32 * 256, st>>>(p);
   MX_LAUNCH_CHECK();
   g_launch_count = 0;
-  record_launch(2, ww ? 256 : 128, (ww || wide) ? 256 : 128, g.splits, g.tiles, true, 100 + (ww ? 5 : wide ? 4 : 3));
+  record_launch(2, ww ? 256 : 128, (ww || wide) ? 256 : 128, g.splits, g.tiles, true,
+                (DSPLIT ? 200 : 100) + (ww ? 5 : wide ? 4 : 3));
   return wgrad_finish(p, g, Kout, st, name);
+}
+
+extern "C" int mx_conv2d_wgrad_x3(const mx_conv_shape* s, const float* dy, const float* x, float* dw, int64_t Kout,
+                                  int64_t Cin, int layout, void* ws, size_t ws_bytes, mx_stream_t stream,
+                                  const mx_conv_cfg* cfg) {
+  return wgrad_x3_impl<false>(s, dy, x, dw, Kout, Cin, layout, ws, ws_bytes, stream, cfg);
+}
+
+extern "C" int mx_conv2d_wgrad_x3_split(const mx_conv_shape* s, const uint16_t* dy, const float* x, float* dw,
+                                        int64_t Kout, int64_t Cin, int layout, void* ws, size_t ws_bytes,
+                                        mx_stream_t stream, const mx_conv_cfg* cfg) {
+  return wgrad_x3_impl<true>(s, dy, x, dw, Kout, Cin, layout, ws, ws_bytes, stream, cfg);
+}
+
+static bool wgrad_x3_split_ok(const Cfg& cf, const mx_conv_shape* s) {
+  if (s->K % 8 || s->C % 8 || s->K * s->R * s->S * s->C >= (1ll << 31)) return false;
+  bool dense;
+  const mx_conv_shape d = wgrad_shape(s, &dense);
+  const WGeo g = wgrad_geo_x3(cf, &d);
+  const int64_t P = d.N * d.Ho * d.Wo;
+  return g.tiles * g.splits < (1ll << 31) && P * d.K * 4 < (1ll << 31) && d.N * d.H * d.W * d.C * 4 < (1ll << 31) &&
+         P + 64 < (1ll << 23) && d.N * d.H * d.W < (1ll << 23) && d.K * 4 < (1ll << 24) && d.C * 4 < (1ll << 24);
+}
+
+extern "C" int mx_conv2d_x3_split_supported(const mx_conv_shape* s, int passes, const mx_conv_cfg* dgrad_cfg,
+                                            const mx_conv_cfg* wgrad_cfg) {
+  Cfg cd, cw;
+  if (!s || !(passes & 3) || (passes & ~3) || conv_check(s)) return 0;
+  if ((passes & 1) && (resolve_cfg(dgrad_cfg, cd) || !dgrad_x3_split_ok(cd, s))) return 0;
+  if ((passes & 2) && (resolve_cfg(wgrad_cfg, cw) || !wgrad_x3_split_ok(cw, s))) return 0;
+  return 1;
 }
 
 extern "C" int mx_conv2d_wgrad_x3_rows(const mx_conv_shape* s, const float* dy, const float* x, float* dw, int64_t Kout,
diff --git a/robust-object-detection_amd/mx_det/_lib.py b/robust-object-detection_amd/mx_det/_lib.py
--- a/robust-object-detection_amd/mx_det/_lib.py
+++ b/robust-object-detection_amd/mx_det/_lib.py
@@ -254,6 +254,12 @@
                                    c_vp, c_i64, c_vp, c_sz, c_vp, c_cfg]),
     "mx_conv2d_wgrad_x3": (c_int, [ctypes.POINTER(ConvShape), c_vp, c_vp, c_vp, c_i64, c_i64, c_int, c_vp, c_sz,
                                    c_vp, c_cfg]),
+    "mx_bn_bwd_apply_split": (c_int, [c_vp, c_vp, c_vp, c_i64, c_i64, c_int, c_vp, c_vp, c_vp, c_vp]),
+    "mx_conv2d_dgrad_x3_split": (c_int, [ctypes.POINTER(ConvShape), c_vp, c_vp, c_vp, c_vp, c_vp, c_vp, c_vp, c_vp,
+                                         c_int, c_vp, c_i64, c_vp, c_sz, c_vp, c_cfg]),
+    "mx_conv2d_wgrad_x3_split": (c_int, [ctypes.POINTER(ConvShape), c_vp, c_vp, c_vp, c_i64, c_i64, c_int, c_vp, c_sz,
+                                         c_vp, c_cfg]),
+    "mx_conv2d_x3_split_supported": (c_int, [ctypes.POINTER(ConvShape), c_int, c_cfg, c_cfg]),
     "mx_rpn_rows_capacity": (c_i64, [c_i64, c_i64, c_int]),
     "mx_rpn_rows_workspace": (c_sz, [c_i64]),
     "mx_rpn_rows_build": (c_int, [c_vp, c_i64, c_i64, c_i64, c_i64, c_int, c_vp, c_i64, c_vp, c_i64, c_vp, c_i64, c_vp,
diff --git a/robust-object-detection_amd/mx_det/conv.py b/robust-object-detection_amd/mx_det/conv.py
--- a/robust-object-detection_amd/mx_det/conv.py
+++ b/robust-object-detection_amd/mx_det/conv.py
@@ -367,10 +367,12 @@
 
 
 def conv_dgrad(dy, wt, x_shape, R, S, stride, pad, residual=None, bnb=None, rows=None, rows_fill=True,
-               rows_inplace=False):
+               rows_inplace=False, split=False):
     N, H, W, C = x_shape
-    K = dy.shape[3]
-    x3 = is_x3(dy)
+    K = dy.shape[-1]
+    x3 = split or is_x3(dy)
+    odt = torch.float32 if split else dy.dtype
+    assert not split or (rows is None and dy.dtype == torch.bfloat16 and dy.dim() == 5 and dy.is_contiguous())
     assert wt.numel() == (2 if x3 else 1) * C * R * S * K, (wt.numel(), C, R, S, K)
     Ho, Wo = out_hw(H, W, R, S, stride, pad)
     sh = _lib.ConvShape(N, H, W, C, K, R, S, Ho, Wo, stride[0], stride[1], pad[0], pad[1])
@@ -404,10 +406,10 @@
                 _timer.stop("x3_dgrad", 2.0 * rows[2] * K * R * S * C, t0, _tag(N, H, W, C, K, R, S, stride),
                             dy.numel() * dy.element_size() + wt.numel() * 2 + rows[2] * C * 4)
             return dx
-    dx = torch.empty((N, H, W, C), dtype=dy.dtype, device=dy.device)
+    dx = torch.empty((N, H, W, C), dtype=odt, device=dy.device)
     t0 = _timer.start() if _timer else None
     if residual is not None:
-        assert residual.dtype == dy.dtype and residual.shape == dx.shape and residual.is_contiguous()
+        assert residual.dtype == odt and residual.shape == dx.shape and residual.is_contiguous()
     part, mb = None, (N * H * W + 63) // 64
     if bnb is not None:
         part = torch.empty((2, mb, C), dtype=torch.float32, device=dy.device)
@@ -418,8 +420,8 @@
             wsb = _lib.load().mx_conv_workspace_x3(ctypes.byref(sh), 1, cfg)
             ws = torch.empty(wsb, dtype=torch.uint8, device=dy.device) if wsb else None
             b = bnb if part is not None else None
-            call("mx_conv2d_dgrad_x3", ctypes.byref(sh), _p(dyc), _p(wt), _p(residual), _p(dx),
-                 _p(b.y) if b else None, _p(b.z) if b else None, _p(b.mean) if b else None,
+            call("mx_conv2d_dgrad_x3_split" if split else "mx_conv2d_dgrad_x3", ctypes.byref(sh), _p(dyc), _p(wt),
+                 _p(residual), _p(dx), _p(b.y) if b else None, _p(b.z) if b else None, _p(b.mean) if b else None,
                  _p(b.invstd) if b else None, int(b.act) if b else 0, _p(part), mb, _p(ws), wsb, _s(), cfg)
             return
         wsb = _lib.load().mx_conv_workspace(ctypes.byref(sh), 1, cfg)
@@ -430,7 +432,7 @@
         else:
             call("mx_conv2d_dgrad_ex", ctypes.byref(sh), _p(dyc), _p(wt), _p(residual), _p(dx), _p(ws), wsb, _s(), cfg)
 
-    key = ("dgrad", dy.dtype, N, H, W, C, K, R, S, tuple(stride), tuple(pad), residual is not None, part is not None)
+    key = ("dgrad", odt, N, H, W, C, K, R, S, tuple(stride), tuple(pad), residual is not None, part is not None)
     _tuned(key, _FD_CANDS_X3 if x3 else _FD_CANDS, run)
     if part is not None:
         bnb.part = part
@@ -500,17 +502,17 @@
     return dedicated_stream(device, "wgrad")
 
 
-def _wgrad_plan(ctx, dy, x, K, R, S, stride, pad, kout=None, cin=None, rows=None):
+def _wgrad_plan(ctx, dy, x, K, R, S, stride, pad, kout=None, cin=None, rows=None, split=False):
     if not ctx.needs_input_grad[1]:
         return None
     dst = grad_dest(ctx)
     side = side_wgrad_enabled(ctx)
     if side and os.environ.get("MX_WGRAD_FORK", "early") != "late":
-        job = wgrad_prepare(dy, x, K, R, S, stride, pad, kout, cin, dst, rows)
+        job = wgrad_prepare(dy, x, K, R, S, stride, pad, kout, cin, dst, rows, split)
         fork = torch.cuda.Event()
         fork.record()
         return job, side, fork
-    return (dy, x, K, R, S, stride, pad, kout, cin, dst, rows), side, None
+    return (dy, x, K, R, S, stride, pad, kout, cin, dst, rows, split), side, None
 
 
 def _wgrad_run(plan):
@@ -532,16 +534,19 @@
                  "t0", "rows")
 
 
-def wgrad_prepare(dy, x, K, R, S, stride, pad, kout=None, cin=None, out=None, rows=None):
+def wgrad_prepare(dy, x, K, R, S, stride, pad, kout=None, cin=None, out=None, rows=None, split=False):
     j = _WgradJob()
     sh = j.sh = shape(x, K, R, S, stride, pad)
     j.kout = kout = kout or K
     j.cin = cin = cin or x.shape[3]
     j.K, j.R, j.S, j.stride = K, R, S, stride
     j.x3 = x3 = is_x3(x)
-    assert dy.dtype == x.dtype, (dy.dtype, x.dtype)
+    if split:
+        assert x3 and rows is None and dy.dtype == torch.bfloat16 and dy.dim() == 5, (dy.dtype, dy.shape)
+    else:
+        assert dy.dtype == x.dtype, (dy.dtype, x.dtype)
     wsfn = "mx_conv_workspace_x3" if x3 else "mx_conv_workspace"
-    j.entry = entry = "mx_conv2d_wgrad_x3" if x3 else "mx_conv2d_wgrad_ex"
+    j.entry = entry = ("mx_conv2d_wgrad_x3_split" if split else "mx_conv2d_wgrad_x3") if x3 else "mx_conv2d_wgrad_ex"
     if out is not None:
         assert out.shape == (kout, cin, R, S) and out.dtype == torch.float32 and out.is_contiguous(), out.shape
         dw = out
@@ -1078,6 +1083,39 @@
     return y
 
 
+def _known_cfg(key, cands):
+    if not _tune_on():
+        return True, None
+    c = _tune_cache.get(key)
+    if c is not None:
+        return True, c
+    if _timer is not None or torch.cuda.is_current_stream_capturing():
+        return True, cands[0]
+    return False, None
+
+
+def x3_split_plan(x, K, R, S, stride, pad, need_dx, need_dw, dgrad_res, dgrad_bnb):
+    if os.environ.get("MX_X3_SPLIT", "1") == "0" or not (need_dx or need_dw):
+        return False
+    N, H, W, C = x.shape
+    sh = shape(x, K, R, S, stride, pad)
+    dcfg = wcfg = None
+    if need_dx:
+        key = ("dgrad", torch.float32, N, H, W, C, K, R, S, tuple(stride), tuple(pad), bool(dgrad_res), bool(dgrad_bnb))
+        known, c = _known_cfg(key, _FD_CANDS_X3)
+        if not known:
+            return False
+        dcfg = _fd_cfg(c)
+    if need_dw:
+        key = ("wgrad", torch.float32, N, H, W, C, K, R, S, tuple(stride), tuple(pad))
+        known, c = _known_cfg(key, _WG_CANDS_X3)
+        if not known:
+            return False
+        wcfg = _wg_cfg(c)
+    return bool(_lib.load().mx_conv2d_x3_split_supported(ctypes.byref(sh), (1 if need_dx else 0) | (2 if need_dw else 0),
+                                                         dcfg, wcfg))
+
+
 class ConvBNAct(torch.autograd.Function):
 
     @staticmethod
@@ -1129,26 +1167,38 @@
                  _p(gamma.detach()), _p(ws), ws.numel(), _p(sums), _p(coef), _s())
             if _timer:
                 _timer.stop("bn_bwd_reduce", M * K * z.element_size() * (3 if act else 2), t0, f"{M}x{K}")
-        dz = torch.empty_like(z)
-        dres = torch.empty_like(z) if has_res else None
-        t0 = _timer.start() if _timer else None
-        call("mx_bn_bwd_apply_ex", _p(gy), _p(y), _p(z), dcode(z), M, K, int(act), _p(coef), _p(dz), _p(dres), _s())
-        if _timer:
-            _timer.stop("bn_bwd_apply", M * K * z.element_size() * (4 + (1 if has_res else 0)), t0, f"{M}x{K}")
-        dx = dw = None
-        wg = _wgrad_plan(ctx, dz, x, K, R, S, stride, pad, cin=wshape[1])
         link = ctx.link
-        if ctx.role == "sink" and dres is not None:
-            link.dres, dres = dres, None
-        if ctx.needs_input_grad[0]:
-            res = None
-            if ctx.role == "src":
-                res, link.dres = link.dres, None
+        need_dx, need_dw = ctx.needs_input_grad[0], ctx.needs_input_grad[1]
+        bnb = chain = None
+        if need_dx:
             feed = ctx.bnb_feed
             chain = ctx.chain
             bnb = feed if (feed is not None and feed.y is not None and tuple(stride) == (1, 1)
                            and feed.y.shape == x.shape and (chain is None or chain.last())) else None
-            dx = conv_dgrad(dz, wt, x.shape, R, S, stride, pad, residual=_chain_res(chain, res), bnb=bnb)
+        split = False
+        if is_x3(z):
+            dgrad_res = need_dx and ((ctx.role == "src" and link.dres is not None)
+                                     or (chain is not None and chain.acc is not None))
+            split = x3_split_plan(x, K, R, S, stride, pad, need_dx, need_dw, dgrad_res, bnb is not None)
+        dres = torch.empty_like(z) if has_res else None
+        t0 = _timer.start() if _timer else None
+        if split:
+            dz = torch.empty((2,) + tuple(z.shape), dtype=torch.bfloat16, device=z.device)
+            call("mx_bn_bwd_apply_split", _p(gy), _p(y), _p(z), M, K, int(act), _p(coef), _p(dz), _p(dres), _s())
+        else:
+            dz = torch.empty_like(z)
+            call("mx_bn_bwd_apply_ex", _p(gy), _p(y), _p(z), dcode(z), M, K, int(act), _p(coef), _p(dz), _p(dres), _s())
+        if _timer:
+            _timer.stop("bn_bwd_apply", M * K * z.element_size() * (4 + (1 if has_res else 0)), t0, f"{M}x{K}")
+        dx = dw = None
+        wg = _wgrad_plan(ctx, dz, x, K, R, S, stride, pad, cin=wshape[1], split=split)
+        if ctx.role == "sink" and dres is not None:
+            link.dres, dres = dres, None
+        if need_dx:
+            res = None
+            if ctx.role == "src":
+                res, link.dres = link.dres, None
+            dx = conv_dgrad(dz, wt, x.shape, R, S, stride, pad, residual=_chain_res(chain, res), bnb=bnb, split=split)
             if chain is not None:
                 dx = chain.hand(dx)
         if wg is not None:
```
